# maotian123/loc_lib

Measured on AMD Instinct MI355X. Metric: scans/sec (64x1800-pt scan vs 10M-pt map) + ICP iter ms, higher is better.
Workload: dtype f64; 1 GPU; BASELINE configs[2]: 256 scans/GPU x 115200 pts (64x1800, cityblock-v1) vs one 10000000-pt map, P2PLANE ICP, reference defaults (alpha=0.1 KD-tree ANN, eps=1e-2, max 20 iters), scans sharded by rank, no collective; includes scan H2D: every step aligns a batch copied host->HBM for it (pinned double buffer, copy stream, overlapped with the previous step); 3 alignment(s) in flight; scans_per_gpu=256, map_points=10000000, pipeline_depth=3, search_mode=tree_faithful_ann, tree_depth=30, tree_bytes=239999992

## Files before the change

include/locgpu.h:

```cpp
#ifndef LOCGPU_H_
#define LOCGPU_H_

#include <stddef.h>
#include <stdint.h>

#ifdef __cplusplus
extern "C" {
#endif

#define LOCGPU_API __attribute__((visibility("default")))

typedef struct locgpu_ctx locgpu_ctx;
typedef struct locgpu_batch locgpu_batch;

typedef enum locgpu_status {
    LOCGPU_OK = 0,
    LOCGPU_ERR_INVALID = -1,
    LOCGPU_ERR_NO_DEVICE = -2,
    LOCGPU_ERR_NO_TARGET = -3,
    LOCGPU_ERR_K_TOO_LARGE = -4,
    LOCGPU_ERR_DEPTH = -5,
    LOCGPU_ERR_OOM = -6
} locgpu_status;

// ... 55 lines not shown
LOCGPU_API int locgpu_icp_build_map_planes(locgpu_ctx* ctx);
LOCGPU_API int locgpu_icp_map_planes_info(const locgpu_ctx* ctx, int64_t out[3]);
LOCGPU_API int locgpu_icp_map_planes_dump(locgpu_ctx* ctx, double* n4, uint8_t* valid, size_t cap, size_t* n_out);

LOCGPU_API int locgpu_knn(locgpu_ctx* ctx, const float* queries, size_t nq, int k, int approximate, float alpha, int search_mode,
                          int32_t* out_idx, uint32_t* visits);

LOCGPU_API int locgpu_bfnn_set_target(locgpu_ctx* ctx, const void* pts, size_t n, size_t stride_bytes);
LOCGPU_API int locgpu_bfnn_knn(locgpu_ctx* ctx, const float* queries, size_t nq, int k, int32_t* out_idx);

LOCGPU_API int locgpu_icp_hb(locgpu_ctx* ctx, const void* src, size_t n, size_t stride_bytes, const double pose[7],
                             const locgpu_icp_opts* opts, double H[36], double B[6], int64_t* effective_num, int* ok);

LOCGPU_API int locgpu_icp_align(locgpu_ctx* ctx, const void* src, size_t n, size_t stride_bytes, const double init_pose[7],
                                const locgpu_icp_opts* opts, double out_pose[7], locgpu_align_stats* stats);

typedef void* (*locgpu_out_cloud_fn)(void* user, size_t n_points);
#define LOCGPU_OUT_FIELDS_DONE ((size_t)1 << (sizeof(size_t) * 8 - 1))
LOCGPU_API int locgpu_icp_scan_match(locgpu_ctx* ctx, const void* src, size_t n, size_t stride_bytes, const double init_pose[7],
                                     const locgpu_icp_opts* opts, double out_pose[7], locgpu_align_stats* stats, void* out_cloud,
                                     size_t out_stride_bytes, locgpu_out_cloud_fn out_fn, void* out_user);
LOCGPU_API int locgpu_ndt_scan_match(locgpu_ctx* ctx, const void* src, size_t n, size_t stride_bytes, const double init_pose[7],
                                     double result_pose[7], locgpu_align_stats* stats, void* out_cloud, size_t out_stride_bytes,
                                     locgpu_out_cloud_fn out_fn, void* out_user);

LOCGPU_API int locgpu_transform_cloud(locgpu_ctx* ctx, const double pose[7], const void* src, size_t n, size_t src_stride_bytes,
                                      void* out, size_t out_stride_bytes);

LOCGPU_API int locgpu_batch_create(locgpu_ctx* ctx, const void* const* srcs, const size_t* counts, size_t stride_bytes, int n_scans,
                                   locgpu_batch** out);
LOCGPU_API void locgpu_batch_destroy(locgpu_batch* b);
LOCGPU_API int locgpu_batch_create_empty(locgpu_ctx* ctx, int n_scans, size_t max_points_per_scan, locgpu_batch** out);
LOCGPU_API int locgpu_batch_upload_async(locgpu_batch* b, const void* const* srcs, const size_t* counts, size_t stride_bytes);
LOCGPU_API int locgpu_batch_upload_wait(locgpu_batch* b);
LOCGPU_API int locgpu_icp_align_batch(locgpu_ctx* ctx, locgpu_batch* b, const double* init_poses, const locgpu_icp_opts* opts,
                                      double* out_poses, locgpu_align_stats* stats);
LOCGPU_API int locgpu_ndt_align_batch(locgpu_ctx* ctx, locgpu_batch* b, const double* init_poses, double* out_poses,
                                      locgpu_align_stats* stats);
LOCGPU_API int locgpu_icp_align_batch_begin(locgpu_ctx* ctx, locgpu_batch* b, const double* init_poses, const locgpu_icp_opts* opts);
LOCGPU_API int locgpu_ndt_align_batch_begin(locgpu_ctx* ctx, locgpu_batch* b, const double* init_poses);
LOCGPU_API int locgpu_align_batch_end(locgpu_ctx* ctx, locgpu_batch* b, double* out_poses, locgpu_align_stats* stats);
LOCGPU_API int locgpu_icp_hb_batch(locgpu_ctx* ctx, locgpu_batch* b, const double* poses, const locgpu_icp_opts* opts, double* hb);
LOCGPU_API int locgpu_gn_update(const double hb[44], int method, int min_effective_pts, double eps, double pose[7], double dx[6],
                                int* applied, int* stop);

typedef struct locgpu_loam locgpu_loam;
typedef struct locgpu_loam_opts {
    locgpu_icp_opts surf;
    locgpu_icp_opts edge;
    int32_t use_surf_points;
    int32_t use_edge_points;
    int32_t max_iteration;
    double eps;
} locgpu_loam_opts;
LOCGPU_API void locgpu_loam_opts_default(locgpu_loam_opts* o);
LOCGPU_API int locgpu_loam_create(int device_id, const locgpu_loam_opts* opts, locgpu_loam** out);
LOCGPU_API int locgpu_loam_create_on(locgpu_ctx* surf_ctx, locgpu_ctx* edge_ctx, const locgpu_loam_opts* opts, locgpu_loam** out);
LOCGPU_API void locgpu_loam_destroy(locgpu_loam* l);
LOCGPU_API const char* locgpu_loam_last_error(const locgpu_loam* l);
LOCGPU_API int locgpu_loam_set_target(locgpu_loam* l, const void* edge_pts, size_t n_edge, const void* surf_pts, size_t n_surf, size_t stride_bytes);
LOCGPU_API int locgpu_loam_hb(locgpu_loam* l, const void* edge, size_t n_edge, const void* surf, size_t n_surf, size_t stride_bytes,
                              const double pose[7], double H[36], double B[6], int64_t eff[2], int32_t ok[2]);
LOCGPU_API int locgpu_loam_scan_match(locgpu_loam* l, const void* edge, size_t n_edge, const void* surf, size_t n_surf, size_t stride_bytes,
                                      const double init_pose[7], double result_pose[7], locgpu_align_stats* stats, void* out_cloud,
                                      size_t out_stride_bytes);
LOCGPU_API int locgpu_loam_align_batch(locgpu_loam* l, int n_scans, const void* const* edge_srcs, const size_t* edge_counts,
                                       const void* const* surf_srcs, const size_t* surf_counts, size_t stride_bytes, const double* init_poses,
                                       double* out_poses, locgpu_align_stats* stats);

typedef struct locgpu_fitness {
    double score;
    int64_t inliers;
    int64_t finite_points;
} locgpu_fitness;
LOCGPU_API int locgpu_icp_fitness(locgpu_ctx* ctx, const void* src, size_t n, size_t stride_bytes, const double* poses, int n_poses,
                                  double max_range, locgpu_fitness* out);
LOCGPU_API int locgpu_icp_fitness_batch(locgpu_ctx* ctx, locgpu_batch* batch, const double* poses, double max_range, locgpu_fitness* out);
LOCGPU_API int locgpu_icp_fitness_resident(locgpu_ctx* ctx, const double pose[7], double max_range, locgpu_fitness* out);

LOCGPU_API int locgpu_batch_create_shared(locgpu_ctx* ctx, const void* src, size_t n, size_t stride_bytes, int n_entries, locgpu_batch** out);

typedef struct locgpu_init_search_opts {
    double max_range;
    double min_inlier_ratio;
} locgpu_init_search_opts;
LOCGPU_API void locgpu_init_search_opts_default(locgpu_init_search_opts* o);
LOCGPU_API int locgpu_icp_init_search(locgpu_ctx* ctx, const void* src, size_t n, size_t stride_bytes, const double* candidates, int m,
                                      const locgpu_icp_opts* opts, const locgpu_init_search_opts* sopts, double* out_poses,
                                      locgpu_fitness* out_fit, locgpu_align_stats* stats, int* best);
LOCGPU_API int locgpu_loam_fitness(locgpu_loam* l, const void* edge, size_t n_edge, const void* surf, size_t n_surf, size_t stride_bytes,
                                   const double* poses, int n_poses, double max_range, locgpu_fitness* out );
LOCGPU_API int locgpu_loam_init_search(locgpu_loam* l, const void* edge, size_t n_edge, const void* surf, size_t n_surf, size_t stride_bytes,
                                       const double* candidates, int m, const locgpu_init_search_opts* sopts, double* out_poses,
                                       locgpu_fitness* out_fit , locgpu_align_stats* stats, int* best);

LOCGPU_API int locgpu_pose_grid(const double centre[7], double xy_half, double xy_step, double yaw_half, double yaw_step, double* out,
                                size_t cap, size_t* n_out);

#define LOCGPU_COMM_ID_BYTES 128
LOCGPU_API int locgpu_comm_unique_id(void* id_out );
LOCGPU_API int locgpu_comm_init(locgpu_ctx* ctx, int rank, int world, const void* id);
LOCGPU_API int locgpu_comm_info(const locgpu_ctx* ctx, int* rank, int* world);
LOCGPU_API int locgpu_batch_create_sharded(locgpu_ctx* ctx, const void* const* srcs, const size_t* counts, size_t stride_bytes, int n_local,
                                           int first_scan, int n_total, locgpu_batch** out);
LOCGPU_API int locgpu_icp_set_target_bcast(locgpu_ctx* ctx, const void* pts, size_t n, size_t stride_bytes, int root);

typedef struct locgpu_pool locgpu_pool;
typedef struct locgpu_pool_opts {
    int32_t slots;
    int32_t prefetch;
    int32_t scans_per_job;
    int32_t chunk;
    int32_t matcher;
    uint64_t max_points;
    locgpu_icp_opts icp;
} locgpu_pool_opts;
LOCGPU_API void locgpu_pool_opts_default(locgpu_pool_opts* o);
LOCGPU_API int locgpu_pool_create(locgpu_ctx* ctx, const locgpu_pool_opts* opts, locgpu_pool** out);
LOCGPU_API void locgpu_pool_destroy(locgpu_pool* pool);
LOCGPU_API int locgpu_pool_submit(locgpu_pool* pool, const void* const* srcs, const size_t* counts, size_t stride_bytes, int n_local, int first_scan,
                                  int n_total, const double* init_poses, int64_t* ticket);
LOCGPU_API int locgpu_pool_wait(locgpu_pool* pool, int64_t ticket, double* out_poses, locgpu_align_stats* stats);
LOCGPU_API int locgpu_pool_step(locgpu_pool* pool, int block);
LOCGPU_API int locgpu_pool_done(const locgpu_pool* pool, int64_t ticket, int* done);
LOCGPU_API int locgpu_pool_info(const locgpu_pool* pool, int64_t out[8]);
LOCGPU_API int locgpu_pool_profile_read(locgpu_pool* pool, double out[2], int reset);

LOCGPU_API int locgpu_ndt_set_target(locgpu_ctx* ctx, const void* pts, size_t n, size_t stride_bytes, const locgpu_ndt_opts* opts);
LOCGPU_API int locgpu_ndt_target_info(const locgpu_ctx* ctx, int64_t out[3]);
LOCGPU_API int locgpu_ndt_dump(locgpu_ctx* ctx, int32_t* keys, double* mu, double* info, size_t cap, size_t* n_out);
LOCGPU_API int locgpu_ndt_align(locgpu_ctx* ctx, const void* src, size_t n, size_t stride_bytes, const double init_pose[7],
                                double out_pose[7], locgpu_align_stats* stats);
LOCGPU_API int locgpu_ndt_hb(locgpu_ctx* ctx, const void* src, size_t n, size_t stride_bytes, const double pose[7], double H[36], double B[6],
                             int64_t* effective_num, int* ok);
LOCGPU_API int locgpu_ndt_hb_batch(locgpu_ctx* ctx, locgpu_batch* b, const double* poses, double* hb);

LOCGPU_API int locgpu_ndt_fitness(locgpu_ctx* ctx, const void* src, size_t n, size_t stride_bytes, const double* poses, int n_poses,
                                  locgpu_fitness* out);
LOCGPU_API int locgpu_ndt_fitness_batch(locgpu_ctx* ctx, locgpu_batch* batch, const double* poses, locgpu_fitness* out);
LOCGPU_API int locgpu_ndt_fitness_resident(locgpu_ctx* ctx, const double pose[7], locgpu_fitness* out);
LOCGPU_API int locgpu_ndt_init_search(locgpu_ctx* ctx, const void* src, size_t n, size_t stride_bytes, const double* candidates, int m,
                                      const locgpu_init_search_opts* sopts, double* out_poses, locgpu_fitness* out_fit,
                                      locgpu_align_stats* stats, int* best);

LOCGPU_API int locgpu_graph_enable(locgpu_ctx* ctx, int on);

LOCGPU_API int locgpu_profile_enable(locgpu_ctx* ctx, int on);
LOCGPU_API int locgpu_profile_read(locgpu_ctx* ctx, double out[6], int reset);
LOCGPU_API int locgpu_visit_count_enable(locgpu_ctx* ctx, int on);
LOCGPU_API int locgpu_visit_count_read(locgpu_ctx* ctx, uint64_t out[4], int reset);

LOCGPU_API int locgpu_search_stats_read(locgpu_ctx* ctx, uint64_t out[4], int reset);
LOCGPU_API int locgpu_debug_batch_nn(locgpu_ctx* ctx, locgpu_batch* batch, int k, int32_t* out);
LOCGPU_API int locgpu_debug_batch_slot(const locgpu_batch* batch);

typedef struct locgpu_cloud locgpu_cloud;
typedef struct locgpu_submap locgpu_submap;
#define LOCGPU_NO_INTENSITY ((size_t)-1)

LOCGPU_API int locgpu_cloud_create(locgpu_ctx* ctx, locgpu_cloud** out);
LOCGPU_API void locgpu_cloud_destroy(locgpu_cloud* c);
LOCGPU_API int locgpu_cloud_upload(locgpu_cloud* c, const void* pts, size_t n, size_t stride_bytes, size_t intensity_offset, int is_dense);
LOCGPU_API int locgpu_cloud_info(const locgpu_cloud* c, size_t* n, int* is_dense);
LOCGPU_API int locgpu_cloud_download(const locgpu_cloud* c, void* out, size_t capacity, size_t stride_bytes, size_t intensity_offset);
LOCGPU_API int locgpu_cloud_copy(const locgpu_cloud* in, locgpu_cloud* out);

LOCGPU_API int locgpu_cloud_remove_nan(const locgpu_cloud* in, locgpu_cloud* out);
LOCGPU_API int locgpu_cloud_voxel_filter(const locgpu_cloud* in, float leaf, locgpu_cloud* out, int* passthrough);
LOCGPU_API int locgpu_cloud_crop_box(const locgpu_cloud* in, const float min_xyz[3], const float max_xyz[3], locgpu_cloud* out);
LOCGPU_API int locgpu_cloud_transform(const locgpu_cloud* in, const double pose[7], locgpu_cloud* out);
LOCGPU_API int locgpu_cloud_append(locgpu_cloud* dst, const locgpu_cloud* src);

LOCGPU_API int locgpu_icp_set_target_cloud(locgpu_ctx* ctx, const locgpu_cloud* target);
LOCGPU_API int locgpu_icp_set_target_cloud_async(locgpu_ctx* ctx, const locgpu_cloud* target);
LOCGPU_API int locgpu_ndt_set_target_cloud(locgpu_ctx* ctx, const locgpu_cloud* target, const locgpu_ndt_opts* opts);
LOCGPU_API int locgpu_icp_align_cloud(locgpu_ctx* ctx, const locgpu_cloud* src, const double init_pose[7], const locgpu_icp_opts* opts,
                                      double out_pose[7], locgpu_align_stats* stats);
LOCGPU_API int locgpu_ndt_align_cloud(locgpu_ctx* ctx, const locgpu_cloud* src, const double init_pose[7], double out_pose[7],
                                      locgpu_align_stats* stats);

LOCGPU_API int locgpu_voxel_filter(locgpu_ctx* ctx, const void* pts, size_t n, size_t stride_bytes, size_t intensity_offset, int is_dense, float leaf,
                                   void* out, size_t* out_n, int* out_is_dense);
LOCGPU_API int locgpu_crop_box(locgpu_ctx* ctx, const void* pts, size_t n, size_t stride_bytes, size_t intensity_offset, int is_dense,
                               const float min_xyz[3], const float max_xyz[3], void* out, size_t* out_n, int* out_is_dense);
LOCGPU_API int locgpu_remove_nan(locgpu_ctx* ctx, const void* pts, size_t n, size_t stride_bytes, size_t intensity_offset, int is_dense, void* out,
                                 size_t* out_n, int* out_is_dense);

LOCGPU_API int locgpu_batch_preprocess(locgpu_batch* src, float leaf, locgpu_batch* dst, int32_t* out_counts ,
                                       int32_t* out_status );
LOCGPU_API int locgpu_batch_upload_clouds(locgpu_batch* b, const locgpu_cloud* const* clouds, int n);
LOCGPU_API int locgpu_batch_download_scan(locgpu_batch* b, int scan, void* out, size_t capacity, size_t stride_bytes, size_t* n);

LOCGPU_API int locgpu_cloud_loam_extract(const locgpu_cloud* in, const uint8_t* ring, int num_scan, locgpu_cloud* edge, locgpu_cloud* surf);
LOCGPU_API int locgpu_loam_extract(locgpu_ctx* ctx, const void* pts, size_t n, size_t stride_bytes, size_t intensity_offset, int intensity_is_u8,
                                   size_t ring_offset, int num_scan, void* edge_out, size_t* n_edge, void* surf_out, size_t* n_surf,
                                   size_t out_stride_bytes, size_t out_intensity_offset);

LOCGPU_API int locgpu_batch_loam_extract(locgpu_batch* src, const uint8_t* const* rings ,
                                         int num_scan, locgpu_batch* edge, locgpu_batch* surf, int32_t* out_edge_counts,
                                         int32_t* out_surf_counts, int32_t* out_status );
LOCGPU_API int locgpu_loam_align_batches(locgpu_loam* l, locgpu_batch* edge, locgpu_batch* surf, const double* init_poses, double* out_poses,
                                         locgpu_align_stats* stats);

typedef struct locgpu_sensor locgpu_sensor;
typedef struct locgpu_sensor_model {
    int32_t n_rings, n_cols;
    float range_scale, min_range;
    int32_t az_per_ring, reserved;
    const float* cos_el;
    const float* sin_el;
    const float* cos_az;
    const float* sin_az;
} locgpu_sensor_model;
LOCGPU_API int locgpu_sensor_create(locgpu_ctx* ctx, const locgpu_sensor_model* model, locgpu_sensor** out);
LOCGPU_API void locgpu_sensor_destroy(locgpu_sensor* s);
LOCGPU_API int locgpu_batch_upload_ranges(locgpu_batch* b, const locgpu_sensor* s, const uint16_t* const* images ,
                                          int32_t* out_counts );
LOCGPU_API int locgpu_batch_download_rings(locgpu_batch* b, int scan, uint8_t* out, size_t capacity, size_t* n);
LOCGPU_API int locgpu_batch_loam_extract_resident(locgpu_batch* src, int num_scan, locgpu_batch* edge, locgpu_batch* surf,
                                                  int32_t* out_edge_counts, int32_t* out_surf_counts, int32_t* out_status );
LOCGPU_API int locgpu_cloud_upload_ranges(locgpu_cloud* c, const locgpu_sensor* s, const uint16_t* image, uint8_t* ring_out ,
                                          size_t* n);

LOCGPU_API int locgpu_range_ingest_times(locgpu_ctx* ctx, double out_ms[2]);

LOCGPU_API int locgpu_submap_create(locgpu_ctx* ctx, int num_kfs, float leaf, locgpu_submap** out);
LOCGPU_API void locgpu_submap_destroy(locgpu_submap* m);
LOCGPU_API int locgpu_submap_add_keyframe(locgpu_submap* m, const locgpu_cloud* scan, const double pose[7]);
LOCGPU_API int locgpu_submap_cloud(locgpu_submap* m, locgpu_cloud** map);
LOCGPU_API int locgpu_submap_last_keyframe(locgpu_submap* m, locgpu_cloud** kf);
LOCGPU_API int locgpu_submap_info(const locgpu_submap* m, int* n_keyframes, size_t* map_points);

LOCGPU_API int locgpu_loam_set_target_cloud(locgpu_loam* l, const locgpu_cloud* edge_map, const locgpu_cloud* surf_map);
LOCGPU_API int locgpu_loam_set_target_cloud_async(locgpu_loam* l, const locgpu_cloud* edge_map, const locgpu_cloud* surf_map);
LOCGPU_API int locgpu_loam_scan_match_cloud(locgpu_loam* l, const locgpu_cloud* edge, const locgpu_cloud* surf, const double init_pose[7],
                                            double result_pose[7], locgpu_align_stats* stats, locgpu_cloud* out);
LOCGPU_API int locgpu_loam_fitness_resident(locgpu_loam* l, const double pose[7], double max_range, locgpu_fitness out[2]);
LOCGPU_API int locgpu_loam_fitness_cloud(locgpu_loam* l, const locgpu_cloud* edge, const locgpu_cloud* surf, const double* poses, int n_poses,
                                         double max_range, locgpu_fitness* out );
LOCGPU_API int locgpu_loam_init_search_cloud(locgpu_loam* l, const locgpu_cloud* edge, const locgpu_cloud* surf, const double* candidates, int m,
                                             const locgpu_init_search_opts* sopts, double* out_poses, locgpu_fitness* out_fit ,
                                             locgpu_align_stats* stats, int* best);

typedef struct locgpu_loam_submap locgpu_loam_submap;
LOCGPU_API int locgpu_loam_submap_create(locgpu_ctx* ctx, int num_kfs, float leaf, locgpu_loam_submap** out);
LOCGPU_API void locgpu_loam_submap_destroy(locgpu_loam_submap* m);
LOCGPU_API int locgpu_loam_submap_add_keyframe(locgpu_loam_submap* m, const locgpu_cloud* edge, const locgpu_cloud* surf, const double pose[7]);
LOCGPU_API int locgpu_loam_submap_clouds(locgpu_loam_submap* m, locgpu_cloud** edge_map, locgpu_cloud** surf_map);
LOCGPU_API int locgpu_loam_submap_info(const locgpu_loam_submap* m, int* n_keyframes, size_t* edge_points, size_t* surf_points);

LOCGPU_API int locgpu_clouds_merge(locgpu_ctx* ctx, const locgpu_cloud* const* clouds, const double* poses , int n, float leaf,
                                   locgpu_cloud* out, int* passthrough );
LOCGPU_API int locgpu_batch_merge(locgpu_batch* b, const double* poses , const uint8_t* use , float leaf,
                                  locgpu_cloud* out, int* passthrough );
LOCGPU_API int locgpu_batch_export_cloud(locgpu_batch* b, int scan, locgpu_cloud* cloud);

#ifdef __cplusplus
}
#endif
#endif
```

loc_lib_amd/api.py:

```python
import ctypes
import os
import subprocess

import numpy as np

_HERE = os.path.dirname(os.path.abspath(__file__))
LIB_PATH = os.environ.get("LOCGPU_LIB") or os.path.join(_HERE, "liblocgpu.so")
CSRC = os.path.join(_HERE, "csrc")

P2P, P2LINE, P2PLANE = 0, 1, 2
P2PLANE_MAP = 5
SEARCH_TREE_FAITHFUL, SEARCH_GRID_EXACT = 0, 1
CENTER, NEARBY6 = 0, 1
DIRECT_NDT, INCREMENTAL_NDT = 1, 2

ABI_SYMBOLS = [
    "locgpu_icp_opts_default", "locgpu_ndt_opts_default", "locgpu_create", "locgpu_destroy", "locgpu_last_error",
    "locgpu_device_count", "locgpu_icp_set_target", "locgpu_icp_set_target_async", "locgpu_icp_target_info", "locgpu_knn", "locgpu_icp_hb", "locgpu_icp_align",
    "locgpu_transform_cloud", "locgpu_batch_create", "locgpu_batch_destroy", "locgpu_icp_align_batch", "locgpu_ndt_align_batch",
    "locgpu_icp_hb_batch", "locgpu_gn_update", "locgpu_ndt_set_target", "locgpu_ndt_target_info", "locgpu_ndt_dump",
    "locgpu_ndt_align", "locgpu_profile_enable", "locgpu_profile_read", "locgpu_visit_count_enable", "locgpu_visit_count_read",
    "locgpu_search_stats_read", "locgpu_debug_batch_nn", "locgpu_debug_batch_slot", "locgpu_graph_enable",
    "locgpu_cloud_create", "locgpu_cloud_destroy", "locgpu_cloud_upload", "locgpu_cloud_info", "locgpu_cloud_download", "locgpu_cloud_copy",
    "locgpu_cloud_remove_nan", "locgpu_cloud_voxel_filter", "locgpu_cloud_crop_box", "locgpu_cloud_transform", "locgpu_cloud_append",
    "locgpu_icp_set_target_cloud", "locgpu_icp_set_target_cloud_async", "locgpu_ndt_set_target_cloud", "locgpu_icp_align_cloud", "locgpu_ndt_align_cloud",
    "locgpu_voxel_filter", "locgpu_crop_box", "locgpu_remove_nan",
    "locgpu_submap_create", "locgpu_submap_destroy", "locgpu_submap_add_keyframe", "locgpu_submap_cloud", "locgpu_submap_last_keyframe",
    "locgpu_submap_info", "locgpu_cloud_loam_extract", "locgpu_loam_extract",
    "locgpu_batch_create_empty", "locgpu_batch_upload_async", "locgpu_batch_upload_wait",
    "locgpu_bfnn_set_target", "locgpu_bfnn_knn",
    "locgpu_icp_align_batch_begin", "locgpu_ndt_align_batch_begin", "locgpu_align_batch_end",
    "locgpu_comm_unique_id", "locgpu_comm_init", "locgpu_comm_info", "locgpu_batch_create_sharded", "locgpu_icp_set_target_bcast",
    "locgpu_pool_opts_default", "locgpu_pool_create", "locgpu_pool_destroy", "locgpu_pool_submit", "locgpu_pool_wait", "locgpu_pool_info",
    "locgpu_pool_profile_read", "locgpu_pool_step", "locgpu_pool_done",
    "locgpu_icp_scan_match", "locgpu_ndt_scan_match",
    "locgpu_icp_fitness", "locgpu_icp_fitness_batch", "locgpu_icp_fitness_resident", "locgpu_batch_create_shared",
    "locgpu_init_search_opts_default", "locgpu_icp_init_search", "locgpu_pose_grid",
    "locgpu_ndt_fitness", "locgpu_ndt_fitness_batch", "locgpu_ndt_fitness_resident", "locgpu_ndt_init_search", "locgpu_ndt_hb", "locgpu_ndt_hb_batch",
    "locgpu_icp_build_map_planes", "locgpu_icp_map_planes_info", "locgpu_icp_map_planes_dump",
    "locgpu_loam_opts_default", "locgpu_loam_create", "locgpu_loam_destroy", "locgpu_loam_last_error", "locgpu_loam_set_target",
    "locgpu_loam_hb", "locgpu_loam_scan_match", "locgpu_loam_align_batch",
    "locgpu_loam_set_target_cloud", "locgpu_loam_set_target_cloud_async", "locgpu_loam_scan_match_cloud", "locgpu_loam_fitness_resident",
    "locgpu_loam_submap_create", "locgpu_loam_submap_destroy", "locgpu_loam_submap_add_keyframe", "locgpu_loam_submap_clouds", "locgpu_loam_submap_info",
    "locgpu_loam_create_on", "locgpu_loam_fitness", "locgpu_loam_fitness_cloud", "locgpu_loam_init_search", "locgpu_loam_init_search_cloud",
    "locgpu_batch_preprocess", "locgpu_batch_upload_clouds", "locgpu_batch_download_scan",
    "locgpu_batch_loam_extract", "locgpu_loam_align_batches",
    "locgpu_clouds_merge", "locgpu_batch_merge", "locgpu_batch_export_cloud",
    "locgpu_sensor_create", "locgpu_sensor_destroy", "locgpu_batch_upload_ranges", "locgpu_batch_download_rings",
    "locgpu_batch_loam_extract_resident", "locgpu_cloud_upload_ranges", "locgpu_range_ingest_times",
]
COMM_ID_BYTES = 128
NO_INTENSITY = ctypes.c_size_t(-1).value


class LocGpuError(RuntimeError):
    def __init__(self, code, msg):
        super().__init__("locgpu error %d: %s" % (code, msg))
        self.code = code


class IcpOpts(ctypes.Structure):
    _fields_ = [("method", ctypes.c_int32), ("max_iteration", ctypes.c_int32), ("max_nn_distance", ctypes.c_double),
                ("max_plane_distance", ctypes.c_double), ("max_line_distance", ctypes.c_double), ("min_effective_pts", ctypes.c_int32),
                ("eps", ctypes.c_double), ("approximate", ctypes.c_int32), ("ann_alpha", ctypes.c_float), ("search_mode", ctypes.c_int32)]


class NdtOpts(ctypes.Structure):
    _fields_ = [("max_iteration", ctypes.c_int32), ("voxel_size", ctypes.c_double), ("min_effective_pts", ctypes.c_int32),
                ("min_pts_in_voxel", ctypes.c_int32), ("eps", ctypes.c_double), ("res_outlier_th", ctypes.c_double),
                ("nearby_type", ctypes.c_int32), ("method", ctypes.c_int32), ("capacity", ctypes.c_int64)]


class LoamOpts(ctypes.Structure):
    _fields_ = [("surf", IcpOpts), ("edge", IcpOpts), ("use_surf_points", ctypes.c_int32), ("use_edge_points", ctypes.c_int32),
                ("max_iteration", ctypes.c_int32), ("eps", ctypes.c_double)]


class PoolOpts(ctypes.Structure):
    _fields_ = [("slots", ctypes.c_int32), ("prefetch", ctypes.c_int32), ("scans_per_job", ctypes.c_int32), ("chunk", ctypes.c_int32), ("matcher", ctypes.c_int32),
                ("max_points", ctypes.c_uint64), ("icp", IcpOpts)]


class Fitness(ctypes.Structure):
    _fields_ = [("score", ctypes.c_double), ("inliers", ctypes.c_int64), ("finite_points", ctypes.c_int64)]


class InitSearchOpts(ctypes.Structure):
    _fields_ = [("max_range", ctypes.c_double), ("min_inlier_ratio", ctypes.c_double)]


class SensorModelC(ctypes.Structure):
    _fields_ = [("n_rings", ctypes.c_int32), ("n_cols", ctypes.c_int32), ("range_scale", ctypes.c_float), ("min_range", ctypes.c_float),
                ("az_per_ring", ctypes.c_int32), ("reserved", ctypes.c_int32), ("cos_el", ctypes.c_void_p), ("sin_el", ctypes.c_void_p),
                ("cos_az", ctypes.c_void_p), ("sin_az", ctypes.c_void_p)]


class AlignStats(ctypes.Structure):
    _fields_ = [("iterations", ctypes.c_int32), ("converged", ctypes.c_int32), ("status", ctypes.c_int32), ("reserved", ctypes.c_int32),
                ("last_effective_num", ctypes.c_int64), ("last_dx_norm", ctypes.c_double)]


def build(force=False):
    args = ["make", "-C", CSRC, "-j4"]
    if force:
        args.append("-B")
    subprocess.check_call(args, stdout=subprocess.DEVNULL)
    return LIB_PATH


_lib = None


def lib():
    global _lib
    if _lib is None:
        if not os.path.exists(LIB_PATH):
            raise LocGpuError(-2, "liblocgpu.so is not built (run `python -c 'import __graft_entry__ as g; g.build()'`); no CPU fallback exists")
        L = ctypes.CDLL(LIB_PATH)
        vp, sz, i32, dbl, f32 = ctypes.c_void_p, ctypes.c_size_t, ctypes.c_int, ctypes.c_double, ctypes.c_float
        sig = {
            "locgpu_icp_opts_default": (None, [vp]), "locgpu_ndt_opts_default": (None, [vp]),
            "locgpu_create": (i32, [i32, vp]), "locgpu_destroy": (None, [vp]), "locgpu_last_error": (ctypes.c_char_p, [vp]),
            "locgpu_device_count": (i32, []),
            "locgpu_icp_set_target": (i32, [vp, vp, sz, sz]), "locgpu_icp_set_target_async": (i32, [vp, vp, sz, sz]), "locgpu_icp_target_info": (i32, [vp, vp]),
            "locgpu_knn": (i32, [vp, vp, sz, i32, i32, f32, i32, vp, vp]),
            "locgpu_icp_hb": (i32, [vp, vp, sz, sz, vp, vp, vp, vp, vp, vp]),
            "locgpu_icp_align": (i32, [vp, vp, sz, sz, vp, vp, vp, vp]),
            "locgpu_transform_cloud": (i32, [vp, vp, vp, sz, sz, vp, sz]),
            "locgpu_batch_create": (i32, [vp, vp, vp, sz, i32, vp]), "locgpu_batch_destroy": (None, [vp]),
            "locgpu_icp_align_batch": (i32, [vp, vp, vp, vp, vp, vp]), "locgpu_ndt_align_batch": (i32, [vp, vp, vp, vp, vp]),
            "locgpu_icp_align_batch_begin": (i32, [vp, vp, vp, vp]), "locgpu_ndt_align_batch_begin": (i32, [vp, vp, vp]),
            "locgpu_align_batch_end": (i32, [vp, vp, vp, vp]),
            "locgpu_icp_hb_batch": (i32, [vp, vp, vp, vp, vp]),
            "locgpu_gn_update": (i32, [vp, i32, i32, dbl, vp, vp, vp, vp]),
            "locgpu_ndt_set_target": (i32, [vp, vp, sz, sz, vp]), "locgpu_ndt_target_info": (i32, [vp, vp]),
            "locgpu_ndt_dump": (i32, [vp, vp, vp, vp, sz, vp]), "locgpu_ndt_align": (i32, [vp, vp, sz, sz, vp, vp, vp]),
            "locgpu_profile_enable": (i32, [vp, i32]), "locgpu_profile_read": (i32, [vp, vp, i32]),
            "locgpu_visit_count_enable": (i32, [vp, i32]), "locgpu_visit_count_read": (i32, [vp, vp, i32]),
            "locgpu_search_stats_read": (i32, [vp, vp, i32]), "locgpu_debug_batch_nn": (i32, [vp, vp, i32, vp]), "locgpu_debug_batch_slot": (i32, [vp]), "locgpu_graph_enable": (i32, [vp, i32]),
            "locgpu_cloud_create": (i32, [vp, vp]), "locgpu_cloud_destroy": (None, [vp]),
            "locgpu_cloud_upload": (i32, [vp, vp, sz, sz, sz, i32]), "locgpu_cloud_info": (i32, [vp, vp, vp]),
            "locgpu_cloud_download": (i32, [vp, vp, sz, sz, sz]), "locgpu_cloud_copy": (i32, [vp, vp]),
            "locgpu_cloud_remove_nan": (i32, [vp, vp]), "locgpu_cloud_voxel_filter": (i32, [vp, f32, vp, vp]),
            "locgpu_cloud_crop_box": (i32, [vp, vp, vp, vp]), "locgpu_cloud_transform": (i32, [vp, vp, vp]),
            "locgpu_cloud_append": (i32, [vp, vp]),
            "locgpu_icp_set_target_cloud": (i32, [vp, vp]), "locgpu_icp_set_target_cloud_async": (i32, [vp, vp]), "locgpu_ndt_set_target_cloud": (i32, [vp, vp, vp]),
            "locgpu_icp_align_cloud": (i32, [vp, vp, vp, vp, vp, vp]), "locgpu_ndt_align_cloud": (i32, [vp, vp, vp, vp, vp]),
            "locgpu_voxel_filter": (i32, [vp, vp, sz, sz, sz, i32, f32, vp, vp, vp]),
            "locgpu_crop_box": (i32, [vp, vp, sz, sz, sz, i32, vp, vp, vp, vp, vp]),
            "locgpu_remove_nan": (i32, [vp, vp, sz, sz, sz, i32, vp, vp, vp]),
            "locgpu_submap_create": (i32, [vp, i32, f32, vp]), "locgpu_submap_destroy": (None, [vp]),
            "locgpu_submap_add_keyframe": (i32, [vp, vp, vp]), "locgpu_submap_cloud": (i32, [vp, vp]),
            "locgpu_submap_last_keyframe": (i32, [vp, vp]), "locgpu_submap_info": (i32, [vp, vp, vp]),
            "locgpu_cloud_loam_extract": (i32, [vp, vp, i32, vp, vp]),
            "locgpu_loam_extract": (i32, [vp, vp, sz, sz, sz, i32, sz, i32, vp, vp, vp, vp, sz, sz]),
            "locgpu_batch_create_empty": (i32, [vp, i32, sz, vp]), "locgpu_batch_upload_async": (i32, [vp, vp, vp, sz]),
            "locgpu_batch_upload_wait": (i32, [vp]),
            "locgpu_comm_unique_id": (i32, [vp]), "locgpu_comm_init": (i32, [vp, i32, i32, vp]), "locgpu_comm_info": (i32, [vp, vp, vp]),
            "locgpu_batch_create_sharded": (i32, [vp, vp, vp, sz, i32, i32, i32, vp]),
            "locgpu_icp_set_target_bcast": (i32, [vp, vp, sz, sz, i32]),
            "locgpu_bfnn_set_target": (i32, [vp, vp, sz, sz]), "locgpu_bfnn_knn": (i32, [vp, vp, sz, i32, vp]),
            "locgpu_pool_opts_default": (None, [vp]), "locgpu_pool_create": (i32, [vp, vp, vp]), "locgpu_pool_destroy": (None, [vp]),
            "locgpu_pool_submit": (i32, [vp, vp, vp, sz, i32, i32, i32, vp, vp]), "locgpu_pool_wait": (i32, [vp, ctypes.c_int64, vp, vp]),
            "locgpu_pool_info": (i32, [vp, vp]), "locgpu_pool_profile_read": (i32, [vp, vp, i32]),
            "locgpu_pool_step": (i32, [vp, i32]), "locgpu_pool_done": (i32, [vp, ctypes.c_int64, vp]),
            "locgpu_icp_scan_match": (i32, [vp, vp, sz, sz, vp, vp, vp, vp, vp, sz, vp, vp]),
            "locgpu_ndt_scan_match": (i32, [vp, vp, sz, sz, vp, vp, vp, vp, sz, vp, vp]),
            "locgpu_icp_fitness": (i32, [vp, vp, sz, sz, vp, i32, dbl, vp]), "locgpu_icp_fitness_batch": (i32, [vp, vp, vp, dbl, vp]),
            "locgpu_icp_fitness_resident": (i32, [vp, vp, dbl, vp]), "locgpu_batch_create_shared": (i32, [vp, vp, sz, sz, i32, vp]),
            "locgpu_init_search_opts_default": (None, [vp]),
            "locgpu_icp_init_search": (i32, [vp, vp, sz, sz, vp, i32, vp, vp, vp, vp, vp, vp]),
            "locgpu_pose_grid": (i32, [vp, dbl, dbl, dbl, dbl, vp, sz, vp]),
            "locgpu_ndt_fitness": (i32, [vp, vp, sz, sz, vp, i32, vp]), "locgpu_ndt_fitness_batch": (i32, [vp, vp, vp, vp]),
            "locgpu_ndt_fitness_resident": (i32, [vp, vp, vp]),
            "locgpu_ndt_hb": (i32, [vp, vp, sz, sz, vp, vp, vp, vp, vp]), "locgpu_ndt_hb_batch": (i32, [vp, vp, vp, vp]),
            "locgpu_ndt_init_search": (i32, [vp, vp, sz, sz, vp, i32, vp, vp, vp, vp, vp]),
            "locgpu_icp_build_map_planes": (i32, [vp]), "locgpu_icp_map_planes_info": (i32, [vp, vp]),
            "locgpu_icp_map_planes_dump": (i32, [vp, vp, vp, sz, vp]),
            "locgpu_loam_opts_default": (None, [vp]), "locgpu_loam_create": (i32, [i32, vp, vp]), "locgpu_loam_destroy": (None, [vp]),
            "locgpu_loam_last_error": (ctypes.c_char_p, [vp]), "locgpu_loam_set_target": (i32, [vp, vp, sz, vp, sz, sz]),
            "locgpu_loam_hb": (i32, [vp, vp, sz, vp, sz, sz, vp, vp, vp, vp, vp]),
            "locgpu_loam_scan_match": (i32, [vp, vp, sz, vp, sz, sz, vp, vp, vp, vp, sz]),
            "locgpu_loam_align_batch": (i32, [vp, i32, vp, vp, vp, vp, sz, vp, vp, vp]),
            "locgpu_loam_set_target_cloud": (i32, [vp, vp, vp]), "locgpu_loam_set_target_cloud_async": (i32, [vp, vp, vp]),
            "locgpu_loam_scan_match_cloud": (i32, [vp, vp, vp, vp, vp, vp, vp]), "locgpu_loam_fitness_resident": (i32, [vp, vp, dbl, vp]),
            "locgpu_loam_submap_create": (i32, [vp, i32, f32, vp]), "locgpu_loam_submap_destroy": (None, [vp]),
            "locgpu_loam_submap_add_keyframe": (i32, [vp, vp, vp, vp]), "locgpu_loam_submap_clouds": (i32, [vp, vp, vp]),
            "locgpu_loam_submap_info": (i32, [vp, vp, vp, vp]),
            "locgpu_loam_create_on": (i32, [vp, vp, vp, vp]),
            "locgpu_loam_fitness": (i32, [vp, vp, sz, vp, sz, sz, vp, i32, dbl, vp]),
            "locgpu_loam_fitness_cloud": (i32, [vp, vp, vp, vp, i32, dbl, vp]),
            "locgpu_loam_init_search": (i32, [vp, vp, sz, vp, sz, sz, vp, i32, vp, vp, vp, vp, vp]),
            "locgpu_loam_init_search_cloud": (i32, [vp, vp, vp, vp, i32, vp, vp, vp, vp, vp]),
            "locgpu_batch_preprocess": (i32, [vp, f32, vp, vp, vp]), "locgpu_batch_upload_clouds": (i32, [vp, vp, i32]),
            "locgpu_batch_download_scan": (i32, [vp, i32, vp, sz, sz, vp]),
            "locgpu_batch_loam_extract": (i32, [vp, vp, i32, vp, vp, vp, vp, vp]), "locgpu_loam_align_batches": (i32, [vp, vp, vp, vp, vp, vp]),
            "locgpu_clouds_merge": (i32, [vp, vp, vp, i32, f32, vp, vp]), "locgpu_batch_merge": (i32, [vp, vp, vp, f32, vp, vp]),
            "locgpu_batch_export_cloud": (i32, [vp, i32, vp]),
            "locgpu_sensor_create": (i32, [vp, vp, vp]), "locgpu_sensor_destroy": (None, [vp]),
            "locgpu_batch_upload_ranges": (i32, [vp, vp, vp, vp]), "locgpu_batch_download_rings": (i32, [vp, i32, vp, sz, vp]),
            "locgpu_batch_loam_extract_resident": (i32, [vp, i32, vp, vp, vp, vp, vp]),
            "locgpu_cloud_upload_ranges": (i32, [vp, vp, vp, vp, vp]), "locgpu_range_ingest_times": (i32, [vp, vp]),
        }
        for name, (res, args) in sig.items():
            fn = getattr(L, name)
            fn.restype = res
            fn.argtypes = args
        _lib = L
    return _lib


def device_count():
    return int(lib().locgpu_device_count())


def comm_unique_id():
    buf = (ctypes.c_char * COMM_ID_BYTES)()
    rc = lib().locgpu_comm_unique_id(buf)
    if rc != 0:
        raise LocGpuError(rc, "locgpu_comm_unique_id failed")
    return bytes(buf)


def _cloud(a):
    a = np.ascontiguousarray(a, dtype=np.float32)
    if a.ndim != 2 or a.shape[1] < 3:
        raise ValueError("cloud must be [n, >=3] float32")
    return a


def _pose(p):
    p = np.ascontiguousarray(p, dtype=np.float64)
    if p.shape[-1] != 7:
        raise ValueError("pose must have 7 doubles (quaternion xyzw + translation)")
    return p


def icp_opts(method=P2P, **kw):
    o = IcpOpts()
    lib().locgpu_icp_opts_default(ctypes.byref(o))
    o.method = method
    for k, v in kw.items():
        if not hasattr(o, k):
            raise TypeError("unknown ICP option %r" % k)
        setattr(o, k, v)
    return o


def ndt_opts(**kw):
    o = NdtOpts()
    lib().locgpu_ndt_opts_default(ctypes.byref(o))
    for k, v in kw.items():
        if not hasattr(o, k):
            raise TypeError("unknown NDT option %r" % k)
        setattr(o, k, v)
    return o


def init_search_opts(**kw):
    o = InitSearchOpts()
    lib().locgpu_init_search_opts_default(ctypes.byref(o))
    for k, v in kw.items():
        if not hasattr(o, k):
            raise TypeError("unknown initial-pose search option %r" % k)
        setattr(o, k, v)
    return o


def loam_opts(**kw):
    o = LoamOpts()
    lib().locgpu_loam_opts_default(ctypes.byref(o))
    for k, v in kw.items():
        if not hasattr(o, k):
            raise TypeError("unknown LOAM option %r" % k)
        setattr(o, k, v)
    return o


def pose_grid(centre, xy_half, xy_step, yaw_half, yaw_step, cap=None):
    c = _pose(centre)
    n = ctypes.c_size_t(0)
    rc = lib().locgpu_pose_grid(c.ctypes.data, xy_half, xy_step, yaw_half, yaw_step, None, 0, ctypes.byref(n))
    if rc != 0:
        raise LocGpuError(rc, "locgpu_pose_grid: bad arguments")
    k = n.value if cap is None else min(int(cap), n.value)
    out = np.zeros((k, 7))
    rc = lib().locgpu_pose_grid(c.ctypes.data, xy_half, xy_step, yaw_half, yaw_step, out.ctypes.data if k else None, k, ctypes.byref(n))
    if rc != 0:
        raise LocGpuError(rc, "locgpu_pose_grid: bad arguments")
    return out, int(n.value)


# ... 224 lines not shown
        return out, [_stats_dict(s) for s in st]

    def icp_hb_batch(self, batch, poses, opts):
        batch.upload_wait()
        p = _pose(poses).reshape(batch.n_scans, 7)
        hb = np.zeros((batch.n_scans, 44))
        self._check(lib().locgpu_icp_hb_batch(self._h, batch._h, p.ctypes.data, ctypes.byref(opts), hb.ctypes.data))
        return hb

    def icp_fitness(self, src, poses, max_range=1.0, raw=False):
        s = _cloud(src)
        p = _pose(poses)
        one = p.ndim == 1
        p = p.reshape(-1, 7)
        out = (Fitness * p.shape[0])()
        self._check(lib().locgpu_icp_fitness(self._h, s.ctypes.data, s.shape[0], s.strides[0], p.ctypes.data, p.shape[0], max_range, out))
        if raw:
            return out
        return _fitness_dict(out[0]) if one else [_fitness_dict(f) for f in out]

    def icp_fitness_batch(self, batch, poses, max_range=1.0, raw=False):
        batch.upload_wait()
        p = _pose(poses).reshape(batch.n_scans, 7)
        out = (Fitness * batch.n_scans)()
        self._check(lib().locgpu_icp_fitness_batch(self._h, batch._h, p.ctypes.data, max_range, out))
        return out if raw else [_fitness_dict(f) for f in out]

    def icp_fitness_resident(self, pose, max_range=1.0):
        out = Fitness()
        self._check(lib().locgpu_icp_fitness_resident(self._h, _pose(pose).ctypes.data, max_range, ctypes.byref(out)))
        return _fitness_dict(out)

    def batch_shared(self, scan, n_entries):
        return Batch(self, None, n_scans=n_entries, shared=scan)

    def icp_init_search(self, src, candidates, opts, sopts=None, raw=False):
        s = _cloud(src)
        c = _pose(candidates).reshape(-1, 7)
        m = c.shape[0]
        out = np.zeros((m, 7))
        fit = (Fitness * max(m, 1))()
        st = (AlignStats * max(m, 1))()
        best = ctypes.c_int(-2)
        self._check(lib().locgpu_icp_init_search(self._h, s.ctypes.data, s.shape[0], s.strides[0], c.ctypes.data, m, ctypes.byref(opts),
                                                 ctypes.byref(sopts) if sopts is not None else None, out.ctypes.data, fit, st, ctypes.byref(best)))
        return out, (fit if raw else [_fitness_dict(f) for f in fit]), [_stats_dict(x) for x in st], int(best.value)

    def ndt_set_target(self, cloud, opts=None):
        c = _cloud(cloud)
        self._check(lib().locgpu_ndt_set_target(self._h, c.ctypes.data, c.shape[0], c.strides[0], ctypes.byref(opts) if opts else None))

    def ndt_target_info(self):
        out = np.zeros(3, dtype=np.int64)
        self._check(lib().locgpu_ndt_target_info(self._h, out.ctypes.data))
        return dict(num_voxels=int(out[0]), capacity=int(out[1]), bytes=int(out[2]))

    def ndt_dump(self):
        n = self.ndt_target_info()["num_voxels"]
        keys = np.zeros((max(n, 1), 3), dtype=np.int32)
        mu = np.zeros((max(n, 1), 3))
        info = np.zeros((max(n, 1), 9))
        n_out = ctypes.c_size_t(0)
        self._check(lib().locgpu_ndt_dump(self._h, keys.ctypes.data, mu.ctypes.data, info.ctypes.data, n, ctypes.byref(n_out)))
        return keys[:n], mu[:n], info[:n].reshape(n, 3, 3)

    def ndt_align(self, src, init_pose):
        s = _cloud(src)
        out = np.zeros(7)
        st = AlignStats()
        self._check(lib().locgpu_ndt_align(self._h, s.ctypes.data, s.shape[0], s.strides[0], _pose(init_pose).ctypes.data, out.ctypes.data,
                                           ctypes.byref(st)))
        return out, _stats_dict(st)

    def ndt_hb(self, src, pose):
        s = _cloud(src)
        H, B = np.zeros(36), np.zeros(6)
        eff, ok = ctypes.c_int64(0), ctypes.c_int(0)
        self._check(lib().locgpu_ndt_hb(self._h, s.ctypes.data, s.shape[0], s.strides[0], _pose(pose).ctypes.data, H.ctypes.data, B.ctypes.data,
                                        ctypes.byref(eff), ctypes.byref(ok)))
        return bool(ok.value), H.reshape(6, 6), B, int(eff.value)

    def ndt_hb_batch(self, batch, poses):
        batch.upload_wait()
        p = _pose(poses).reshape(batch.n_scans, 7)
        hb = np.zeros((batch.n_scans, 44))
        self._check(lib().locgpu_ndt_hb_batch(self._h, batch._h, p.ctypes.data, hb.ctypes.data))
        return hb

    def ndt_fitness(self, src, poses, raw=False):
        s = _cloud(src)
        p = _pose(poses)
        one = p.ndim == 1
        p = p.reshape(-1, 7)
        out = (Fitness * max(p.shape[0], 1))()
        self._check(lib().locgpu_ndt_fitness(self._h, s.ctypes.data, s.shape[0], s.strides[0], p.ctypes.data, p.shape[0], out))
        if raw:
            return out
        return _fitness_dict(out[0]) if one else [_fitness_dict(f) for f in out]

    def ndt_fitness_batch(self, batch, poses, raw=False):
        batch.upload_wait()
        p = _pose(poses).reshape(batch.n_scans, 7)
        out = (Fitness * batch.n_scans)()
        self._check(lib().locgpu_ndt_fitness_batch(self._h, batch._h, p.ctypes.data, out))
        return out if raw else [_fitness_dict(f) for f in out]

    def ndt_fitness_resident(self, pose):
        out = Fitness()
        self._check(lib().locgpu_ndt_fitness_resident(self._h, _pose(pose).ctypes.data, ctypes.byref(out)))
        return _fitness_dict(out)

    def ndt_init_search(self, src, candidates, sopts=None, raw=False):
        s = _cloud(src)
        c = _pose(candidates).reshape(-1, 7)
        m = c.shape[0]
        out = np.zeros((m, 7))
        fit = (Fitness * max(m, 1))()
        st = (AlignStats * max(m, 1))()
        best = ctypes.c_int(-2)
        self._check(lib().locgpu_ndt_init_search(self._h, s.ctypes.data, s.shape[0], s.strides[0], c.ctypes.data, m,
                                                 ctypes.byref(sopts) if sopts is not None else None, out.ctypes.data, fit, st, ctypes.byref(best)))
        return out, (fit if raw else [_fitness_dict(f) for f in fit]), [_stats_dict(x) for x in st], int(best.value)

    def graph_enable(self, on=True):
        self._check(lib().locgpu_graph_enable(self._h, int(on)))

    def profile_enable(self, on=True):
        self._check(lib().locgpu_profile_enable(self._h, int(on)))

    def profile_read(self, reset=True):
        out = np.zeros(6)
        self._check(lib().locgpu_profile_read(self._h, out.ctypes.data, int(reset)))
        return dict(search_ms=out[0], accum_ms=out[1], solve_ms=out[2], search_n=int(out[3]), accum_n=int(out[4]), solve_n=int(out[5]))

    def range_ingest_times(self):
        out = np.zeros(2)
        self._check(lib().locgpu_range_ingest_times(self._h, out.ctypes.data))
        return float(out[0]), float(out[1])

    def visit_count_enable(self, on=True):
        self._check(lib().locgpu_visit_count_enable(self._h, int(on)))

    def visit_count_read(self, reset=True):
        out = np.zeros(4, dtype=np.uint64)
        self._check(lib().locgpu_visit_count_read(self._h, out.ctypes.data, int(reset)))
        return dict(nodes=int(out[0]), leaves=int(out[1]), queries=int(out[2]), distinct_slots=int(out[3]))


    def debug_batch_nn(self, batch, k=5):
        out = np.empty((batch.n_local, batch.max_points, k), dtype=np.int32)
        self._check(lib().locgpu_debug_batch_nn(self._h, batch._h, int(k), out.ctypes.data))
        return out

    def search_stats_read(self, reset=True):
        out = np.zeros(4, dtype=np.uint64)
        self._check(lib().locgpu_search_stats_read(self._h, out.ctypes.data, int(reset)))
        return dict(searched=int(out[0]), redone=int(out[1]), walked=int(out[2]), replayed=int(out[3]))


def _xyzi(a):
    a = np.ascontiguousarray(a, dtype=np.float32)
    if a.ndim != 2 or a.shape[1] != 4:
        raise ValueError("cloud must be [n, 4] float32 (x, y, z, intensity)")
    return a


class Cloud:

    def __init__(self, ctx, points=None, is_dense=True, _borrowed=None):
        self.ctx = ctx
        self._owned = _borrowed is None
        if _borrowed is not None:
            self._h = _borrowed
        else:
            self._h = ctypes.c_void_p()
            ctx._check(lib().locgpu_cloud_create(ctx._h, ctypes.byref(self._h)))
            if points is not None:
                self.upload(points, is_dense)

    def upload(self, points, is_dense=True):
        a = _xyzi(points)
        self.ctx._check(lib().locgpu_cloud_upload(self._h, a.ctypes.data, a.shape[0], 16, 12, int(is_dense)))
        return self

    @property
    def info(self):
        n, d = ctypes.c_size_t(0), ctypes.c_int(0)
        self.ctx._check(lib().locgpu_cloud_info(self._h, ctypes.byref(n), ctypes.byref(d)))
        return int(n.value), bool(d.value)

    def __len__(self):
        return self.info[0]

    @property
    def is_dense(self):
        return self.info[1]

    def download(self):
        n = len(self)
        out = np.zeros((n, 4), np.float32)
        self.ctx._check(lib().locgpu_cloud_download(self._h, out.ctypes.data, n, 16, 12))
        return out

    def _out(self, out):
        return out if out is not None else Cloud(self.ctx)

    def copy(self, out=None):
        out = self._out(out)
        self.ctx._check(lib().locgpu_cloud_copy(self._h, out._h))
        return out

    def remove_nan(self, out=None):
        out = self._out(out)
        self.ctx._check(lib().locgpu_cloud_remove_nan(self._h, out._h))
        return out

    def voxel_filter(self, leaf, out=None, with_passthrough=False):
        out = self._out(out)
        pt = ctypes.c_int(0)
        self.ctx._check(lib().locgpu_cloud_voxel_filter(self._h, float(leaf), out._h, ctypes.byref(pt)))
        return (out, bool(pt.value)) if with_passthrough else out

    def crop_box(self, mn, mx, out=None):
        out = self._out(out)
        mn, mx = np.ascontiguousarray(mn, np.float32), np.ascontiguousarray(mx, np.float32)
        self.ctx._check(lib().locgpu_cloud_crop_box(self._h, mn.ctypes.data, mx.ctypes.data, out._h))
        return out

    def transform(self, pose, out=None):
        out = self._out(out)
        self.ctx._check(lib().locgpu_cloud_transform(self._h, _pose(pose).ctypes.data, out._h))
        return out

    def append(self, other):
        self.ctx._check(lib().locgpu_cloud_append(self._h, other._h))
        return self

    def upload_ranges(self, sensor, image, with_rings=True):
        img = sensor.model.image(image)
        rings = np.zeros(sensor.model.cells, np.uint8) if with_rings else None
        n = ctypes.c_size_t(0)
        self.ctx._check(lib().locgpu_cloud_upload_ranges(self._h, sensor._h, img.ctypes.data, rings.ctypes.data if with_rings else None, ctypes.byref(n)))
        return np.ascontiguousarray(rings[:int(n.value)]) if with_rings else None

    def loam_extract(self, ring, num_scan=16):
        ring = np.ascontiguousarray(ring, dtype=np.uint8)
        if len(ring) != len(self):
            raise ValueError("one ring byte per point")
        edge, surf = Cloud(self.ctx), Cloud(self.ctx)
        self.ctx._check(lib().locgpu_cloud_loam_extract(self._h, ring.ctypes.data, int(num_scan), edge._h, surf._h))
        return edge, surf

    def close(self):
        if self._owned and getattr(self, "_h", None) and getattr(self.ctx, "_h", None):
            lib().locgpu_cloud_destroy(self._h)
        self._h = None

    def __del__(self):
        self.close()


class SensorModel:

    def __init__(self, n_rings, n_cols, range_scale, min_range, cos_el, sin_el, cos_az, sin_az):
        self.n_rings, self.n_cols = int(n_rings), int(n_cols)
        self.range_scale, self.min_range = np.float32(range_scale), np.float32(min_range)
        self.cos_el, self.sin_el, self.cos_az, self.sin_az = (np.ascontiguousarray(t, dtype=np.float32) for t in (cos_el, sin_el, cos_az, sin_az))
        self.az_per_ring = int(self.cos_az.ndim == 2)
        want_az = (self.n_rings, self.n_cols) if self.az_per_ring else (self.n_cols,)
        if self.cos_el.shape != (self.n_rings,) or self.sin_el.shape != (self.n_rings,) or self.cos_az.shape != want_az or self.sin_az.shape != want_az:
            raise ValueError("sensor tables do not match n_rings / n_cols")

    @property
    def cells(self):
        return self.n_rings * self.n_cols

    def c_struct(self):
        return SensorModelC(self.n_rings, self.n_cols, float(self.range_scale), float(self.min_range), self.az_per_ring, 0, self.cos_el.ctypes.data,
                            self.sin_el.ctypes.data, self.cos_az.ctypes.data, self.sin_az.ctypes.data)

    def image(self, a):
        a = np.ascontiguousarray(a, dtype=np.uint16)
        if a.size != self.cells:
            raise ValueError("a range image of this sensor has %d x %d cells" % (self.n_rings, self.n_cols))
        return a


class Sensor:

    def __init__(self, ctx, model):
        self.ctx, self.model = ctx, model
        self._h = ctypes.c_void_p()
        m = model.c_struct()
        ctx._check(lib().locgpu_sensor_create(ctx._h, ctypes.byref(m), ctypes.byref(self._h)))

    def close(self):
        if getattr(self, "_h", None) and getattr(self.ctx, "_h", None):
            lib().locgpu_sensor_destroy(self._h)
        self._h = None

    def __del__(self):
        self.close()


class Submap:

# ... 469 lines not shown
```

loc_lib_amd/csrc/context.hpp:

```cpp
#pragma once
#include <hip/hip_runtime.h>

#include <string>
#include <vector>

#include "../../include/locgpu.h"
#include "batch_upload.hpp"
#include "device_buffer.hpp"
#include "device_math.hpp"
#include "grid_kernels.hpp"
#include "icp_kernels.hpp"

#include "host_worker.hpp"

struct NdtTable;
namespace locgpu {
struct IncNdtState;
struct FilterScratch;
struct LoamScratch;
struct BatchFilterScratch;
struct BatchLoamScratch;
struct MergeScratch;
struct RangeIngestScratch;
}
struct locgpu_sensor;

namespace locgpu {
struct PendingTarget;
struct AlignSpec {
    GnParams prm{};
    float alpha = 1.0f;
    bool grid = false;
    bool ndt() const { return method_is_ndt(prm.method); }
    int k() const { return method_k(prm.method); }
    bool operator==(const AlignSpec& o) const { return prm == o.prm && alpha == o.alpha && grid == o.grid; }
};
constexpr int kNdtOptDirect = 1, kNdtOptIncremental = 2;
constexpr int kNearbyCenter = 0, kNearby6 = 1;
constexpr int ndt_n_nearby(int nearby_type) { return nearby_type == kNearbyCenter ? 1 : 7; }
struct StageEvents {
    std::vector<Event> ev;
    size_t used = 0;
    int mode = 0;
    void mark(hipStream_t s, bool search_edge = false);
    void collect(locgpu_ctx* ctx, bool ndt);
};
}

struct locgpu_ctx {
    int device = 0;
    hipStream_t stream = nullptr;
    static constexpr int kSlots = 3;
    hipStream_t slot_stream[kSlots] = {};
    int next_slot = 0;
    int slot_load[kSlots] = {};
    hipStream_t copy_stream = nullptr;
    locgpu::Event foreign_ev;
    hipStream_t comm_stream = nullptr;
    locgpu::Uploader* up = nullptr;
    locgpu::PendingTarget* target_scratch = nullptr;
    locgpu::PendingTarget* pending_target = nullptr;
    std::string err;

    locgpu::DevBuf<uint2> d_tree;
    size_t tree_slots = 0, num_leaves = 0, num_nodes = 0, num_points = 0;
    int depth = 0;
    bool tree_bounded = true;
    unsigned long long target_epoch = 0;

    locgpu::DevBuf<uint32_t> d_leaf_slots;

    locgpu::DevBuf<double> d_planes;
    size_t planes_rows = 0;
    bool planes_ready = false;
    long long planes_valid = 0;
    locgpu::DevBuf<unsigned long long> d_planes_count;
    locgpu_batch* planes_ws = nullptr;

    locgpu::GridView grid;
    locgpu::GridBuffers grid_buf;

    locgpu::DevBuf<float4> d_bfnn;
    size_t bfnn_n = 0;

    NdtTable* ndt = nullptr;
    locgpu::IncNdtState* inc = nullptr;
    locgpu_ndt_opts ndt_opts;

    locgpu::FilterScratch* filt = nullptr;
    locgpu::LoamScratch* loam = nullptr;
    locgpu::BatchFilterScratch* bfilt = nullptr;
    locgpu::BatchLoamScratch* bloam = nullptr;
    locgpu::MergeScratch* merge = nullptr;
    locgpu::RangeIngestScratch* ringest = nullptr;
    std::vector<locgpu_sensor*> sensors;

    locgpu_batch* single = nullptr;
    size_t single_cap = 0;
    locgpu_batch* search = nullptr;
    locgpu::HostWorker* worker = nullptr;

    void* comm = nullptr;
    int comm_rank = 0, comm_world = 1;

    int profile = 0;
    double prof_ms[3] = {0, 0, 0};
    long long prof_n[3] = {0, 0, 0};
    bool use_graph = false;
    bool count_visits = false;
    locgpu::DevBuf<unsigned long long> d_visits;
    locgpu::DevBuf<uint32_t> d_touched;
    size_t touched_words = 0;
    locgpu::DevBuf<unsigned long long> d_search_stats;
};

struct locgpu_batch {
    locgpu_ctx* ctx = nullptr;
    int slot = 0;
    hipStream_t stream = nullptr;
    bool pinned = false;
    bool leased = false;
    locgpu::Event chunk_ev;
    int n_scans = 0, max_n = 0, blocks_per_scan = 0;
    int n_total = 0, first = 0;
    bool sharded = false;
    locgpu::DevBuf<double> d_acc;
    size_t pitch = 0;
    locgpu::DevBuf<float4> d_src;
    locgpu::DevBuf<int> d_counts;
    locgpu::DevBuf<unsigned char> d_rings;
    bool rings_valid = false;
    locgpu::DevBuf<locgpu::PoseState> d_state;
    locgpu::DevBuf<uint32_t> d_nn;
    bool shared_src = false;
    locgpu::DevBuf<int> d_src_of;
    int cap_scans = 0, split_scans = 0;
    size_t cap_points = 0;
    const float4* d_src_ext = nullptr;
    bool counters_clean = false;
    int last_iterations = -1;
    locgpu::DevBuf<double> d_partials;
    locgpu::DevBuf<double> d_hb;
    locgpu::DevBuf<uint32_t> d_redo_list;
    locgpu::DevBuf<unsigned int> d_redo_count;
    locgpu::DevBuf<uint32_t> d_redo_list2;
    locgpu::DevBuf<uint32_t> d_grid_qkey;
    locgpu::DevBuf<uint2> d_grid_sorted;
    locgpu::DevBuf<uint32_t> d_grid_tile_count;
    locgpu::DevBuf<unsigned char> d_grid_scan_temp;
    hipGraphExec_t graph_exec = nullptr;
    hipGraphExec_t graph_exec_next = nullptr;
    locgpu::AlignSpec graph_spec;
    const void* graph_target = nullptr;
    unsigned long long graph_epoch = 0;
    locgpu::PinnedBuf<float4> h_src;
    locgpu::Event xyz_ev[8];
    locgpu::PinnedBuf<locgpu::PoseState> h_state;
    locgpu::PinnedBuf<unsigned long long> h_post;
    static constexpr int kPostWord = 16;
    unsigned int post_call = 0;
    bool paced_tail = false;
    locgpu::Event tail_ev;
    locgpu::PinnedBuf<double> h_hb;
    locgpu::PinnedBuf<int> h_active;
    locgpu::DevBuf<int> d_active;
    std::vector<int> counts;
    locgpu::BatchUploadState upl;
    locgpu::StageEvents stage_ev;
    locgpu::Event ev_ready, ev_reduced;
    struct Pending {
        bool active = false;
        locgpu::AlignSpec spec;
        bool graph = false;
        bool paced = false;
        int launched = 0;
        std::vector<double> init_poses;
    } pending;
};

namespace locgpu {

int fail(locgpu_ctx* ctx, int code, const std::string& msg);
bool hip_ok(locgpu_ctx* ctx, hipError_t e, const char* what);

void ndt_free(locgpu_ctx* ctx);
int alloc_batch(locgpu_ctx* ctx, int n_scans, size_t max_n, locgpu_batch** out, int first = 0, int n_total = -1, bool shared_src = false);
void free_batch(locgpu_batch* b);
int check_icp(locgpu_ctx* ctx, const locgpu_icp_opts* o, AlignSpec& spec);
int check_ndt(locgpu_ctx* ctx, AlignSpec& spec);
int target_join(locgpu_ctx* ctx, bool install = true);
void free_target_scratch(locgpu_ctx* ctx);
int icp_set_target_from_cloud(locgpu_ctx* ctx, const locgpu_cloud* target, bool async);
int ensure_grid(locgpu_ctx* ctx);
void free_grid(locgpu_ctx* ctx);
bool comm_all_reduce_f64(locgpu_ctx* ctx, double* buf, size_t count, hipStream_t s);
bool comm_broadcast(locgpu_ctx* ctx, void* buf, size_t bytes, int root, hipStream_t s);
bool comm_all_reduce_min_int(locgpu_ctx* ctx, int* buf, hipStream_t s);
void comm_destroy(locgpu_ctx* ctx);

}

#define LOCGPU_HIP(ctx, expr)                                                    \
    do {                                                                         \
        if (!locgpu::hip_ok((ctx), (expr), #expr)) return LOCGPU_ERR_NO_DEVICE;  \
    } while (0)
```

loc_lib_amd/csrc/gn_driver.hip:

```cpp
#include <algorithm>
#include <chrono>
#include <cmath>
#include <cstdlib>
#include <cstring>
#include <string>
#include <thread>

#include "batch_upload.hpp"
#include "env.hpp"
#include "gn_driver.hpp"
#include "ndt_inc.hpp"
#include "ndt_kernels.hpp"
#include "stream_lease.hpp"

namespace locgpu {

namespace {
inline int next_chunk(const locgpu_batch* b) { return b->n_total == 1 ? 2 : kNextChunk; }
inline int first_chunk_len(const locgpu_batch* b) {
    if (b->n_total != 1 || b->sharded || b->last_iterations < 0) return kFirstChunk;
    return std::min(kLongFirstChunk, std::max(3, b->last_iterations + 1));
}

}

SearchArgs make_search_args(const locgpu_ctx* ctx, const locgpu_batch* b, const float4* src, const PoseState* st, int k, float alpha_eff, bool skip_nonfinite) {
    SearchArgs sa{ctx->d_tree, ctx->tree_slots * sizeof(uint64_t), ctx->depth, src, b->d_counts, st, b->d_nn, b->pitch, b->max_n, b->n_scans, k, alpha_eff,
                  skip_nonfinite ? 1 : 0, nullptr, b->d_redo_list, b->d_redo_count, b->d_redo_list2, b->d_redo_count + 1, ctx->d_search_stats};
    if (!ctx->tree_bounded) sa.redo_list = nullptr;
    return sa;
}

void init_state(PoseState& ps, const double pose[7]) {
    std::memset(&ps, 0, sizeof(ps));
    for (int i = 0; i < 4; ++i) ps.q[i] = pose[i];
    for (int i = 0; i < 3; ++i) ps.t[i] = pose[4 + i];
    quat_to_R(ps.q, ps.R);
}

static void init_states(locgpu_batch* b, const double* poses) {
    for (int s = 0; s < b->n_total; ++s) init_state(b->h_state[s], poses + 7 * (size_t)s);
}

void write_scan_result(const PoseState& ps, const double* init, double* out_pose, locgpu_align_stats* stats) {
    if (ps.status == 1) {
        for (int j = 0; j < 7; ++j) out_pose[j] = init[j];
    } else {
        for (int j = 0; j < 4; ++j) out_pose[j] = ps.q[j];
        for (int j = 0; j < 3; ++j) out_pose[4 + j] = ps.t[j];
    }
    if (!stats) return;
    stats->iterations = ps.iterations; stats->converged = ps.converged; stats->status = ps.status; stats->reserved = 0;
    stats->last_effective_num = ps.last_eff; stats->last_dx_norm = ps.last_dx_norm;
}

bool shard_decoupled(const locgpu_ctx* ctx, bool scan_sharded) {
    static const int env = env_int("LOCGPU_SHARD_DECOUPLED", -1);
    return ctx->comm && scan_sharded && (env >= 0 ? env != 0 : ctx->comm_world > 1);
}

void StageEvents::mark(hipStream_t s, bool search_edge) {
    if (!mode || (mode == 2 && !search_edge)) return;
    if (ev.size() <= used) {
        Event e;
        if (e.ensure(hipEventDefault) != hipSuccess) return;
        ev.push_back(std::move(e));
    }
    (void)hipEventRecord(ev[used++], s);
}

void StageEvents::collect(locgpu_ctx* ctx, bool ndt) {
    const size_t per = mode == 2 ? 2 : 4;
    for (size_t i = 0; i + per - 1 < used; i += per)
        for (size_t j = 0; j + 1 < per; ++j) {
            if (ndt && j == 0) continue;
            float ms = 0.f;
            if (hipEventElapsedTime(&ms, ev[i + j], ev[i + j + 1]) == hipSuccess) { ctx->prof_ms[j] += ms; ctx->prof_n[j] += 1; }
        }
    used = 0;
}

int launch_local_stage(locgpu_ctx* ctx, locgpu_batch* b, const LocalStage& w, hipStream_t s) {
    StageEvents& ev = b->stage_ev;
    int n_partial_blocks = b->blocks_per_scan;
    ev.mark(s, true);
    if (b->n_scans == 0 || (w.active && w.n_active == 0)) {
        ev.mark(s, true);
    } else if (!w.spec.ndt()) {
        const GnParams& prm = w.spec.prm;
        SearchArgs sa = make_search_args(ctx, b, w.src, w.state, w.spec.k(), w.spec.alpha, skips_nonfinite(prm.method));
        const bool grid_mode = w.spec.grid && ctx->tree_bounded;
        if (grid_mode && !w.grid) { fail(ctx, LOCGPU_ERR_INVALID, "grid search: work list missing (ensure_grid_lists was not called)"); return -1; }
        sa.visit_totals = w.visits;
        sa.active = w.active; sa.n_active = w.n_active;
        sa.src_of = w.src_of;
        if (sa.visit_totals && !w.capturing) {
            const size_t words = (ctx->tree_slots + 2 + 31) / 32;
            if (words > ctx->touched_words) {
                ctx->touched_words = 0;
                if (ctx->d_touched.alloc(words) == hipSuccess && hipMemsetAsync(ctx->d_touched, 0, words * sizeof(uint32_t), s) == hipSuccess)
                    ctx->touched_words = words;
            }
            sa.touched = ctx->touched_words ? ctx->d_touched.get() : nullptr;
        }
        const bool ok_search = (grid_mode && !sa.visit_totals) ? launch_icp_search_grid(ctx->grid, sa, *w.grid, s) : launch_icp_search(sa, s);
        if (!ok_search) { fail(ctx, LOCGPU_ERR_DEPTH, std::string(w.who) + ": unsupported k/depth"); return -1; }
        if (sa.touched) launch_count_touched(sa.touched, (ctx->tree_slots + 2 + 31) / 32, sa.visit_totals, s);
        ev.mark(s, true);
        AccumArgs aa{ctx->d_tree, w.src, b->d_counts, w.state, b->d_nn, b->pitch, b->max_n, b->n_scans, icp_gate(prm), b->d_partials};
        aa.planes = ctx->d_planes;
        aa.active = w.active; aa.n_active = w.n_active;
        aa.src_of = w.src_of;
        aa.split_scans = w.split_scans;
        n_partial_blocks = launch_icp_accum(prm.method, aa, s);
    } else {
        ev.mark(s, true);
        if (w.spec.prm.method == kMethodNdtInc)
            launch_inc_accum(ctx->inc, ctx->ndt_opts.res_outlier_th, ndt_n_nearby(ctx->ndt_opts.nearby_type), w.src, b->d_counts, w.state, b->max_n, b->n_scans, b->d_partials, s,
                             w.active, w.n_active, w.src_of);
        else
            n_partial_blocks = launch_ndt_accum(ctx->ndt, w.src, b->d_counts, w.state, b->max_n, b->n_scans, b->d_partials, s, w.active, w.n_active, w.split_scans, w.src_of);
    }
    ev.mark(s);
    return n_partial_blocks;
}

struct IterLauncher {
    locgpu_ctx* ctx;
    locgpu_batch* b;
    const AlignSpec& spec;
    bool capturing = false;
    int slot = 0;
    bool replicated_on_comm_stream = false;
    const int* active = nullptr;
    int n_active = 0;
    const GnPost* post = nullptr;
    bool launch(int do_update);
};

bool IterLauncher::launch(int do_update) {
    hipStream_t s = b->stream;
    const GnParams& prm = spec.prm;
    const bool ndt = spec.ndt();
    StageEvents& ev = b->stage_ev;
    ev.mode = capturing ? 0 : ctx->profile;
    const GridSearchScratch gsc{b->d_grid_qkey, b->d_grid_sorted, b->d_grid_tile_count, b->d_grid_scan_temp};
    const LocalStage w{batch_src(b), b->d_state + b->first, active, n_active, b->d_src_of, b->sharded ? b->n_total : b->split_scans, spec,
                       ctx->count_visits ? ctx->d_visits : nullptr, b->d_grid_qkey ? &gsc : nullptr, capturing, "search"};
    const int n_partial_blocks = launch_local_stage(ctx, b, w, s);
    if (n_partial_blocks < 0) return false;
    if (b->sharded) {
        double* acc = b->d_acc + (size_t)(slot % kFirstChunk) * b->n_total * kAccW;
        slot++;
        launch_sum_partials(b->d_partials, n_partial_blocks, b->d_state, b->first, b->n_scans, b->n_total, acc, s);
        if (do_update && shard_decoupled(ctx, b->n_scans != b->n_total)) {
            hipStream_t cs = ctx->comm_stream;
            if (b->n_scans > 0)
                launch_gn_solve(acc + (size_t)b->first * kAccW, 1, b->d_state + b->first, b->n_scans, prm, do_update, b->d_hb + (size_t)b->first * 44,
                                ndt ? nullptr : b->d_redo_count, s);
            if (!hip_ok(ctx, hipEventRecord(b->ev_ready, s), "sharded: hipEventRecord") || !hip_ok(ctx, hipStreamWaitEvent(cs, b->ev_ready, 0), "sharded: hipStreamWaitEvent")) return false;
            if (!comm_all_reduce_f64(ctx, acc, (size_t)b->n_total * kAccW, cs)) return false;
            const int after = b->first + b->n_scans;
            if (b->first > 0) launch_gn_solve(acc, 1, b->d_state, b->first, prm, do_update, b->d_hb, nullptr, cs);
            if (after < b->n_total)
                launch_gn_solve(acc + (size_t)after * kAccW, 1, b->d_state + after, b->n_total - after, prm, do_update, b->d_hb + (size_t)after * 44, nullptr, cs);
            replicated_on_comm_stream = true;
            ev.mark(s);
            return hip_ok(ctx, hipGetLastError(), "kernel launch");
        }
        if (ctx->comm) {
            static const int force = env_int("LOCGPU_COMM_DIRECT", -1);
            const bool direct = force >= 0 ? force != 0 : ctx->comm_world == 1;
            hipStream_t cs = direct ? s : ctx->comm_stream;
            if (!direct && (!hip_ok(ctx, hipEventRecord(b->ev_ready, s), "sharded: hipEventRecord") || !hip_ok(ctx, hipStreamWaitEvent(cs, b->ev_ready, 0), "sharded: hipStreamWaitEvent"))) return false;
            if (!comm_all_reduce_f64(ctx, acc, (size_t)b->n_total * kAccW, cs)) return false;
            if (!direct && (!hip_ok(ctx, hipEventRecord(b->ev_reduced, cs), "sharded: hipEventRecord") || !hip_ok(ctx, hipStreamWaitEvent(s, b->ev_reduced, 0), "sharded: hipStreamWaitEvent"))) return false;
        }
        launch_gn_solve(acc, 1, b->d_state, b->n_total, prm, do_update, b->d_hb, ndt ? nullptr : b->d_redo_count, s);
    } else {
        launch_gn_solve(b->d_partials, n_partial_blocks, b->d_state, b->n_scans, prm, do_update, b->d_hb, ndt ? nullptr : b->d_redo_count, s, nullptr, post);
    }
    ev.mark(s);
    return hip_ok(ctx, hipGetLastError(), "kernel launch");
}

static int batch_ready(locgpu_ctx* ctx, locgpu_batch* b) {
    const int rc = upload_join_batch(b);
    if (rc != LOCGPU_OK) return rc;
    LOCGPU_HIP(ctx, upload_order_after(b, b->stream));
    return LOCGPU_OK;
}

int ensure_grid_lists(locgpu_ctx* ctx, locgpu_batch* b, const AlignSpec& spec) {
    if (!spec.grid) return LOCGPU_OK;
    if (!b->d_grid_qkey) {
        LOCGPU_HIP(ctx, b->d_grid_qkey.alloc(b->pitch));
        LOCGPU_HIP(ctx, b->d_grid_sorted.alloc(b->pitch));
    }
    const size_t tocc = ctx->grid.n_tocc, scan = std::max<size_t>(ctx->grid.scan_temp_bytes, 1);
    if (b->d_grid_tile_count.cap() < tocc + 1) {
        LOCGPU_HIP(ctx, hipStreamSynchronize(b->stream));
        LOCGPU_HIP(ctx, b->d_grid_tile_count.alloc(tocc + 1));
    }
    if (b->d_grid_scan_temp.cap() < scan) {
        LOCGPU_HIP(ctx, hipStreamSynchronize(b->stream));
        LOCGPU_HIP(ctx, b->d_grid_scan_temp.alloc(scan));
    }
    return LOCGPU_OK;
}

static int capture_chunk(locgpu_ctx* ctx, locgpu_batch* b, const AlignSpec& spec, int iters, bool with_h2d, hipGraphExec_t* out) {
    hipStream_t s = b->stream;
    hipGraph_t graph = nullptr;
    LOCGPU_HIP(ctx, hipStreamBeginCapture(s, hipStreamCaptureModeThreadLocal));
    bool ok = !with_h2d || hip_ok(ctx, hipMemcpyAsync(b->d_state, b->h_state, b->n_total * sizeof(PoseState), hipMemcpyHostToDevice, s), "capture H2D");
    IterLauncher it{ctx, b, spec};
    it.capturing = true;
    for (int i = 0; ok && i < iters; ++i) ok = it.launch(1);
    ok = ok && hip_ok(ctx, hipMemcpyAsync(b->h_state, b->d_state, b->n_total * sizeof(PoseState), hipMemcpyDeviceToHost, s), "capture D2H");
    const hipError_t e = hipStreamEndCapture(s, &graph);
    if (!ok || !hip_ok(ctx, e, "hipStreamEndCapture")) { if (graph) (void)hipGraphDestroy(graph); return LOCGPU_ERR_NO_DEVICE; }
    const bool inst = hip_ok(ctx, hipGraphInstantiate(out, graph, nullptr, nullptr, 0), "hipGraphInstantiate");
    (void)hipGraphDestroy(graph);
    if (!inst) { *out = nullptr; return LOCGPU_ERR_NO_DEVICE; }
    return LOCGPU_OK;
}

static int ensure_graphs(locgpu_ctx* ctx, locgpu_batch* b, const AlignSpec& spec) {
    const void* target = !spec.ndt() ? (const void*)ctx->d_tree : (spec.prm.method == kMethodNdtInc ? inc_ndt_table_ptr(ctx->inc) : (const void*)ctx->ndt->d_rec);
    if (b->graph_exec && b->graph_spec == spec && b->graph_target == target && b->graph_epoch == ctx->target_epoch) return LOCGPU_OK;
    const int first = std::min(kFirstChunk, spec.prm.max_iteration);
    if (b->graph_exec) { (void)hipGraphExecDestroy(b->graph_exec); b->graph_exec = nullptr; }
    if (b->graph_exec_next) { (void)hipGraphExecDestroy(b->graph_exec_next); b->graph_exec_next = nullptr; }
    int rc = capture_chunk(ctx, b, spec, first, true, &b->graph_exec);
    if (rc == LOCGPU_OK && spec.prm.max_iteration > first) rc = capture_chunk(ctx, b, spec, next_chunk(b), false, &b->graph_exec_next);
    if (rc != LOCGPU_OK) return rc;
    b->graph_spec = spec; b->graph_target = target;
    b->graph_epoch = ctx->target_epoch;
    return LOCGPU_OK;
}

static int enqueue_chunk(locgpu_ctx* ctx, locgpu_batch* b, bool first_chunk) {
    locgpu_batch::Pending& P = b->pending;
    const GnParams& prm = P.spec.prm;
    hipStream_t s = b->stream;
    if (P.graph) {
        LOCGPU_HIP(ctx, hipGraphLaunch(first_chunk ? b->graph_exec : b->graph_exec_next, s));
        P.launched += first_chunk ? std::min(kFirstChunk, prm.max_iteration) : next_chunk(b);
        LOCGPU_HIP(ctx, hipEventRecord(b->chunk_ev, s));
        return LOCGPU_OK;
    }
    if (first_chunk) LOCGPU_HIP(ctx, hipMemcpyAsync(b->d_state, b->h_state, b->n_total * sizeof(PoseState), hipMemcpyHostToDevice, s));
    IterLauncher it{ctx, b, P.spec};
    if (!first_chunk && !P.spec.ndt() && b->n_scans > 1) {
        int na = 0;
        for (int i = 0; i < b->n_scans; ++i)
            if (!b->h_state[b->first + i].done) b->h_active[na++] = i;
        if (na > 0 && na < b->n_scans) {
            LOCGPU_HIP(ctx, hipMemcpyAsync(b->d_active, b->h_active, (size_t)na * sizeof(int), hipMemcpyHostToDevice, s));
            it.active = b->d_active;
            it.n_active = na;
        }
    }
    const int todo = std::min(first_chunk ? first_chunk_len(b) : next_chunk(b), prm.max_iteration - P.launched);
    for (int c = 0; c < todo; ++c)
        if (!it.launch(1)) return LOCGPU_ERR_NO_DEVICE;
// ... 315 lines not shown
```

loc_lib_amd/csrc/icp_fit.hip:

```cpp
#include "env.hpp"
#include "icp_kernels.hpp"
#include "launch.hpp"

#include <cstdlib>

namespace locgpu {

template <int ROWS>
__device__ __forceinline__ void add_rows(double (&acc)[28], const double (&J)[ROWS][6], const double (&e)[ROWS]) {
#pragma clang fp contract(fast)
    int o = 0;
#pragma unroll
    for (int i = 0; i < 6; ++i)
#pragma unroll
        for (int j = i; j < 6; ++j) {
            double s = J[0][i] * J[0][j];
#pragma unroll
            for (int r = 1; r < ROWS; ++r) s += J[r][i] * J[r][j];
            acc[o++] += s;
        }
#pragma unroll
    for (int i = 0; i < 6; ++i) {
        double s = -J[0][i] * e[0];
#pragma unroll
        for (int r = 1; r < ROWS; ++r) s += -J[r][i] * e[r];
        acc[21 + i] += s;
    }
}

constexpr int kAccPad = kBlock + 2;
struct RowAccum {
    int ent, slice, ra, rb;
    double sum;
    bool used;
    __device__ __forceinline__ void init() {
        index(threadIdx.x);
        sum = 0.0;
        used = false;
    }
    __device__ __forceinline__ void index(int tid) {
        ent = tid & 31;
        slice = tid >> 5;
        ra = 7; rb = 7;
        int o = 0;
#pragma unroll
        for (int i = 0; i < 6; ++i)
#pragma unroll
            for (int j = i; j < 6; ++j) {
                if (o == ent) { ra = i; rb = j; }
                ++o;
            }
        if (ent >= 21 && ent < 27) { ra = ent - 21; rb = 6; }
    }
    template <int ROWS>
    __device__ __forceinline__ void add(double (&s_row)[8][kAccPad], const double (&J)[ROWS][6], const double (&neg_e)[ROWS], double fitted) {
#pragma clang fp contract(fast)
        const int tid = threadIdx.x;
#pragma unroll
        for (int r = 0; r < ROWS; ++r) {
            if (used) __syncthreads();
            used = true;
#pragma unroll
            for (int c = 0; c < 6; ++c) s_row[c][tid] = J[r][c];
            s_row[6][tid] = neg_e[r];
            s_row[7][tid] = r == 0 ? fitted : 0.0;
            __syncthreads();
            if (ent < 28) {
#pragma unroll 8
                for (int k = 0; k < 32; ++k) {
                    const int col = k * (kBlock / 32) + slice;
                    sum += s_row[ra][col] * s_row[rb][col];
                }
            }
        }
    }
    __device__ __forceinline__ void store(double (&s_slice)[kBlock / 32][32], double* __restrict__ dst) {
        s_slice[slice][ent] = sum;
        __syncthreads();
        if (threadIdx.x < 28) {
            double t = s_slice[0][threadIdx.x];
#pragma unroll
            for (int w = 1; w < kBlock / 32; ++w) t += s_slice[w][threadIdx.x];
            dst[threadIdx.x] = t;
        }
    }
};

__device__ __forceinline__ void R_hat(const double* R, const D3& q, double (&Rh)[3][3]) {
#pragma unroll
    for (int r = 0; r < 3; ++r) {
        Rh[r][0] = R[3 * r + 1] * q.z - R[3 * r + 2] * q.y;
        Rh[r][1] = R[3 * r + 2] * q.x - R[3 * r + 0] * q.z;
        Rh[r][2] = R[3 * r + 0] * q.y - R[3 * r + 1] * q.x;
    }
}

__device__ __forceinline__ void plane_row(const D3& n3, const double* R, const D3& q, double (&J)[6]) {
    double nR[3];
#pragma unroll
    for (int c = 0; c < 3; ++c) nR[c] = -n3.x * R[c] + (-n3.y * R[3 + c] + -n3.z * R[6 + c]);
    J[0] = nR[1] * q.z - nR[2] * q.y;
    J[1] = nR[2] * q.x - nR[0] * q.z;
    J[2] = nR[0] * q.y - nR[1] * q.x;
    J[3] = n3.x; J[4] = n3.y; J[5] = n3.z;
}

__device__ __forceinline__ void sort5(uint32_t (&s)[5]) {
    auto cx = [&](int a, int b) {
        const uint32_t lo = min(s[a], s[b]), hi = max(s[a], s[b]);
        s[a] = lo; s[b] = hi;
    };
    cx(0, 1); cx(3, 4); cx(2, 4); cx(2, 3); cx(1, 4); cx(0, 3); cx(0, 2); cx(1, 3); cx(1, 2);
}

template <int FIT>
__device__ __forceinline__ bool fit_plane(const uint2* __restrict__ tree, const uint32_t (&slot)[5], double (&n4)[4]) {
    D3 nb[5];
#pragma unroll
    for (int j = 0; j < 5; ++j) nb[j] = leaf_point(tree, slot[j]);
    if constexpr (FIT == 1) {
        if (!plane_null_vector_secular(nb, n4)) plane_null_vector(nb, n4);
    } else {
        plane_null_vector(nb, n4);
    }
    const D3 n3{n4[0], n4[1], n4[2]};
    bool fit = true;
#pragma unroll
    for (int j = 0; j < 5; ++j) {
        const double err = dot3(n3, nb[j]) + n4[3];
        if (err * err > 1e-2) fit = false;
    }
    return fit;
}

__device__ __forceinline__ void plane_point_row(const double (&n4)[4], const float4& p, const PoseState& ps, double max_plane_distance,
                                                double (&J)[6], double& neg_e) {
    const D3 n3{n4[0], n4[1], n4[2]};
    const D3 q{(double)p.x, (double)p.y, (double)p.z};
    const D3 qs = se3_apply(ps.q, ps.t, q);
    const double dis = dot3(n3, qs) + n4[3];
    if (!(fabs(dis) > max_plane_distance)) {
        plane_row(n3, ps.R, q, J);
        neg_e = -dis;
    }
}

template <int FIT>
__device__ __forceinline__ void plane_accum_per_point(const uint2* __restrict__ tree, const float4* __restrict__ src,
                                                                 const int* __restrict__ counts, const PoseState* __restrict__ st,
                                                                 const uint32_t* __restrict__ nn, size_t nn_pitch, int max_n,
                                                                 double max_plane_distance, double* __restrict__ partials, int kPlanePts,
                                                                 const int* __restrict__ active, const int* __restrict__ src_of) {
    __shared__ double s_row[8][kAccPad];
    __shared__ double s_slice[kBlock / 32][32];
    const int scan = active ? active[blockIdx.y] : (int)blockIdx.y;
    if (st[scan].done) return;
    RowAccum ra;
    ra.init();
    const int tid = threadIdx.x;
#pragma unroll 1
    for (int pp = 0; pp < kPlanePts; ++pp) {
        const int i = (blockIdx.x * kPlanePts + pp) * kBlock + tid;
        double J[1][6] = {{0.0, 0.0, 0.0, 0.0, 0.0, 0.0}};
        double neg_e[1] = {0.0};
        double fitted = 0.0;
        if (i < counts[scan]) {
            const size_t gi = (size_t)scan * max_n + i;
            uint32_t slot[5];
#pragma unroll
            for (int j = 0; j < 5; ++j) slot[j] = __builtin_nontemporal_load(&nn[(size_t)j * nn_pitch + gi]);
            const float4 p = src[src_index(src_of, scan, max_n, i)];
            if (slot[4] != kInvalidSlot) {
                sort5(slot);
                double n4[4];
                if (fit_plane<FIT>(tree, slot, n4)) {
                    fitted = 1.0;
                    plane_point_row(n4, p, st[scan], max_plane_distance, J[0], neg_e[0]);
                }
            }
        }
        ra.add<1>(s_row, J, neg_e, fitted);
    }
    ra.store(s_slice, partials + ((size_t)scan * gridDim.x + blockIdx.x) * kAccW);
}

constexpr int kDedupPP = 4;
constexpr int kDedupPts = kDedupPP * kBlock;
constexpr uint16_t kLeadFits = 0x8000;
static_assert(8 * kAccPad <= 4 * kDedupPts && kDedupPts <= kLeadFits, "s_row inside the plane table; a leader's point in 15 bits");
template <int FIT>
__device__ __forceinline__ void plane_accum_per_run(const uint2* __restrict__ tree, const float4* __restrict__ src,
                                                                 const int* __restrict__ counts, const PoseState* __restrict__ st,
                                                                 const uint32_t* __restrict__ nn, size_t nn_pitch, int max_n,
                                                                 double max_plane_distance, double* __restrict__ partials, int kPlanePts,
                                                                 const int* __restrict__ active, const int* __restrict__ src_of) {
    __shared__ double s_plane[kDedupPts][4];
    __shared__ double s_slice[kBlock / 32][32];
    __shared__ uint16_t s_lead[kDedupPts];
    __shared__ uint16_t s_rank[kDedupPP][kBlock];
    __shared__ int s_wcnt[kDedupPP][kBlock / 64];
    double (&s_row)[8][kAccPad] = *reinterpret_cast<double (*)[8][kAccPad]>(&s_plane[0][0]);
    const int scan = active ? active[blockIdx.y] : (int)blockIdx.y;
    if (st[scan].done) return;
    const int lane = threadIdx.x & 63;
    const int wave = __builtin_amdgcn_readfirstlane(threadIdx.x >> 6);
    const int n = counts[scan];
    const size_t region = (size_t)scan * max_n;
    const int first = blockIdx.x * kPlanePts * kBlock;
    RowAccum ra;
    ra.init();
    int tid = threadIdx.x;
    asm volatile("" : "+v"(tid));
    int rank[kDedupPP];
    bool leader[kDedupPP];
#pragma unroll
    for (int h = 0; h < kDedupPP; ++h) {
        const int i = first + h * kBlock + tid;
        uint32_t slot[5];
        bool has = false;
        if (h < kPlanePts && i < n) {
#pragma unroll
            for (int j = 0; j < 5; ++j) slot[j] = nn[(size_t)j * nn_pitch + region + i];
            has = slot[4] != kInvalidSlot;
        }
        if (has) {
            sort5(slot);
        } else {
#pragma unroll
            for (int j = 0; j < 5; ++j) slot[j] = kInvalidSlot;
        }
        bool differs = lane == 0;
#pragma unroll
        for (int j = 0; j < 5; ++j) differs |= (uint32_t)__shfl_up((int)slot[j], 1, 64) != slot[j];
        leader[h] = has && differs;
        const unsigned long long mask = __ballot(leader[h]);
        const int below = (int)__builtin_amdgcn_mbcnt_hi((uint32_t)(mask >> 32), __builtin_amdgcn_mbcnt_lo((uint32_t)mask, 0u));
        rank[h] = has ? below + (leader[h] ? 1 : 0) : 0;
        if (lane == 0) s_wcnt[h][wave] = __popcll(mask);
    }
    __syncthreads();
    int n_lead = 0, before[kDedupPP];
#pragma unroll
    for (int h = 0; h < kDedupPP; ++h) {
        before[h] = n_lead;
#pragma unroll
        for (int w = 0; w < kBlock / 64; ++w) {
            const int c = s_wcnt[h][w];
            before[h] += w < wave ? c : 0;
            n_lead += c;
        }
    }
    n_lead = __builtin_amdgcn_readfirstlane(n_lead);
#pragma unroll
    for (int h = 0; h < kDedupPP; ++h) {
        if (rank[h] > 0) rank[h] += before[h];
        if (leader[h]) s_lead[rank[h] - 1] = (uint16_t)(h * kBlock + tid);
        s_rank[h][tid] = (uint16_t)rank[h];
    }
    __syncthreads();
#pragma unroll 1
    for (int base = 0; base < n_lead; base += kBlock) {
        if (base + wave * 64 < n_lead) {
            const int j = base + tid;
            if (j < n_lead) {
                const uint16_t pt = s_lead[j];
                const size_t gi = region + first + pt;
                uint32_t slot[5];
#pragma unroll
                for (int k = 0; k < 5; ++k) slot[k] = __builtin_nontemporal_load(&nn[(size_t)k * nn_pitch + gi]);
                sort5(slot);
                double n4[4];
                if (fit_plane<FIT>(tree, slot, n4)) s_lead[j] = pt | kLeadFits;
#pragma unroll
                for (int c = 0; c < 4; ++c) s_plane[j][c] = n4[c];
            }
        }
    }
    __syncthreads();
    tid = threadIdx.x;
    asm volatile("" : "+v"(tid));
    ra.index(tid);
    double n4[kDedupPP][4];
    float4 p[kDedupPP];
    bool fits[kDedupPP];
#pragma unroll
    for (int h = 0; h < kDedupPP; ++h) {
        rank[h] = s_rank[h][tid];
        fits[h] = false;
        if (rank[h] > 0) {
            fits[h] = (s_lead[rank[h] - 1] & kLeadFits) != 0;
#pragma unroll
            for (int c = 0; c < 4; ++c) n4[h][c] = s_plane[rank[h] - 1][c];
            p[h] = src[src_index(src_of, scan, max_n, first + h * kBlock + tid)];
        }
    }
    __syncthreads();
#pragma unroll
    for (int h = 0; h < kDedupPP; ++h) {
        if (h < kPlanePts) {
            double J[1][6] = {{0.0, 0.0, 0.0, 0.0, 0.0, 0.0}};
            double neg_e[1] = {0.0};
            double fitted = 0.0;
            if (fits[h]) {
                fitted = 1.0;
                plane_point_row(n4[h], p[h], st[scan], max_plane_distance, J[0], neg_e[0]);
            }
            ra.add<1>(s_row, J, neg_e, fitted);
        }
    }
    ra.store(s_slice, partials + ((size_t)scan * gridDim.x + blockIdx.x) * kAccW);
}

template <int FIT, bool DEDUP>
__global__ __launch_bounds__(kBlock) __attribute__((amdgpu_waves_per_eu(4, 4))) void icp_plane_accum_kernel(const uint2* __restrict__ tree, const float4* __restrict__ src,
                                                                 const int* __restrict__ counts, const PoseState* __restrict__ st,
                                                                 const uint32_t* __restrict__ nn, size_t nn_pitch, int max_n,
                                                                 double max_plane_distance, double* __restrict__ partials, int kPlanePts,
                                                                 const int* __restrict__ active, const int* __restrict__ src_of) {
    if constexpr (DEDUP)
        plane_accum_per_run<FIT>(tree, src, counts, st, nn, nn_pitch, max_n, max_plane_distance, partials, kPlanePts, active, src_of);
    else
        plane_accum_per_point<FIT>(tree, src, counts, st, nn, nn_pitch, max_n, max_plane_distance, partials, kPlanePts, active, src_of);
}

__global__ __launch_bounds__(kBlock) void icp_point_accum_kernel(const uint2* __restrict__ tree, const float4* __restrict__ src,
                                                                 const int* __restrict__ counts, const PoseState* __restrict__ st,
                                                                 const uint32_t* __restrict__ nn, size_t nn_pitch, int max_n,
                                                                 double max_nn_distance, double* __restrict__ partials, int pts,
                                                                 const int* __restrict__ active, const int* __restrict__ src_of) {
    const int scan = active ? active[blockIdx.y] : (int)blockIdx.y;
    if (st[scan].done) return;
    double acc[28];
#pragma unroll
    for (int v = 0; v < 28; ++v) acc[v] = 0.0;
#pragma unroll 1
    for (int pp = 0; pp < pts; ++pp) {
    const int i = (blockIdx.x * pts + pp) * kBlock + threadIdx.x;
    if (i < counts[scan]) {
        const size_t gi = (size_t)scan * max_n + i;
        const uint32_t s0 = nn[gi];
        if (s0 != kInvalidSlot) {
            const float4 p = src[src_index(src_of, scan, max_n, i)];
            const D3 q{(double)p.x, (double)p.y, (double)p.z};
            const D3 qs = se3_apply(st[scan].q, st[scan].t, q);
            const D3 e3 = leaf_point(tree, s0) - qs;
            const double dis2 = dot3(e3, e3);
            if (!(dis2 > max_nn_distance)) {
                acc[27] += 1.0;
                double Rh[3][3];
                R_hat(st[scan].R, q, Rh);
                double J[3][6];
#pragma unroll
                for (int r = 0; r < 3; ++r)
#pragma unroll
                    for (int c = 0; c < 3; ++c) { J[r][c] = Rh[r][c] / 16; J[r][3 + c] = (r == c) ? -1.0 : 0.0; }
                const double e[3] = {e3.x, e3.y, e3.z};
                add_rows<3>(acc, J, e);
            }
        }
    }
    }
    block_reduce_store<28, kAccW>(acc, partials + ((size_t)scan * gridDim.x + blockIdx.x) * kAccW);
}

__global__ __launch_bounds__(kBlock) void icp_mapplane_accum_kernel(const double4* __restrict__ planes, const float4* __restrict__ src,
                                                                    const int* __restrict__ counts, const PoseState* __restrict__ st,
                                                                    const uint32_t* __restrict__ nn, int max_n, double max_plane_distance,
                                                                    double* __restrict__ partials, int pts, const int* __restrict__ active,
                                                                    const int* __restrict__ src_of) {
    const int scan = active ? active[blockIdx.y] : (int)blockIdx.y;
    if (st[scan].done) return;
    double acc[28];
#pragma unroll
    for (int v = 0; v < 28; ++v) acc[v] = 0.0;
    const int n = counts[scan];
    const size_t region = src_index(src_of, scan, max_n, 0);
#pragma unroll 1
    for (int pp = 0; pp < pts; ++pp) {
        const int i = (blockIdx.x * pts + pp) * kBlock + threadIdx.x;
        if (i < n) {
            const uint32_t s0 = __builtin_nontemporal_load(&nn[(size_t)scan * max_n + i]);
            const float4 p = src[region + i];
            if (s0 != kInvalidSlot) {
                const double4 n4 = planes[s0 >> 1];
                if (n4.x == n4.x) {
                    acc[27] += 1.0;
                    const D3 n3{n4.x, n4.y, n4.z};
                    const D3 q{(double)p.x, (double)p.y, (double)p.z};
                    const D3 qs = se3_apply(st[scan].q, st[scan].t, q);
                    const double dis = dot3(n3, qs) + n4.w;
                    if (!(fabs(dis) > max_plane_distance)) {
                        double J[1][6];
                        plane_row(n3, st[scan].R, q, J[0]);
                        const double e[1] = {dis};
                        add_rows<1>(acc, J, e);
                    }
                }
            }
        }
    }
    block_reduce_store<28, kAccW>(acc, partials + ((size_t)scan * gridDim.x + blockIdx.x) * kAccW);
}

__global__ __launch_bounds__(kBlock) __attribute__((amdgpu_waves_per_eu(5, 5))) void icp_line_accum_kernel(const uint2* __restrict__ tree, const float4* __restrict__ src,
                                                                const int* __restrict__ counts, const PoseState* __restrict__ st,
                                                                const uint32_t* __restrict__ nn, size_t nn_pitch, int max_n,
                                                                double max_line_distance, double* __restrict__ partials, int pts,
                                                                const int* __restrict__ active, const int* __restrict__ src_of) {
    __shared__ double s_row[8][kAccPad];
    __shared__ double s_slice[kBlock / 32][32];
    const int scan = active ? active[blockIdx.y] : (int)blockIdx.y;
    if (st[scan].done) return;
    RowAccum ra;
    ra.init();
#pragma unroll 1
    for (int pp = 0; pp < pts; ++pp) {
    const int i = (blockIdx.x * pts + pp) * kBlock + threadIdx.x;
    double J[3][6], neg_e[3] = {0.0, 0.0, 0.0};
    double fitted = 0.0;
#pragma unroll
    for (int r = 0; r < 3; ++r)
#pragma unroll
        for (int c = 0; c < 6; ++c) J[r][c] = 0.0;
    if (i < counts[scan]) {
        const size_t gi = (size_t)scan * max_n + i;
        uint32_t slot[5];
#pragma unroll
        for (int j = 0; j < 5; ++j) slot[j] = nn[(size_t)j * nn_pitch + gi];
        const float4 p = src[src_index(src_of, scan, max_n, i)];
        if (slot[4] != kInvalidSlot) {
            const D3 q{(double)p.x, (double)p.y, (double)p.z};
            const D3 qs = se3_apply(st[scan].q, st[scan].t, q);
            D3 nb[5];
#pragma unroll
            for (int j = 0; j < 5; ++j) nb[j] = leaf_point(tree, slot[j]);
            D3 sum{0.0, 0.0, 0.0};
#pragma unroll
            for (int j = 0; j < 5; ++j) sum = sum + nb[j];
            const D3 p0{sum.x / 5.0, sum.y / 5.0, sum.z / 5.0};
            D3 dl[5];
#pragma unroll
            for (int j = 0; j < 5; ++j) dl[j] = nb[j] - p0;
            const D3 d = line_direction(dl);
            bool fit = true;
#pragma unroll
            for (int j = 0; j < 5; ++j) {
                const D3 c = cross3(d, nb[j] - p0);
                if (dot3(c, c) > max_line_distance) fit = false;
            }
            if (fit) {
                fitted = 1.0;
                const D3 e3 = cross3(d, qs - p0);
                if (!(sqrt(dot3(e3, e3)) > max_line_distance)) {
                    const double hd[3][3] = {{0.0, -d.z, d.y}, {d.z, 0.0, -d.x}, {-d.y, d.x, 0.0}};
                    const double hq[3][3] = {{0.0, -q.z, q.y}, {q.z, 0.0, -q.x}, {-q.y, q.x, 0.0}};
                    const double* R = st[scan].R;
                    double hR[3][3], A[3][3];
#pragma unroll
                    for (int r = 0; r < 3; ++r)
#pragma unroll
                        for (int c = 0; c < 3; ++c) {
                            double s = hd[r][0] * R[c];
                            s += hd[r][1] * R[3 + c];
                            s += hd[r][2] * R[6 + c];
                            hR[r][c] = s;
                        }
#pragma unroll
                    for (int r = 0; r < 3; ++r)
#pragma unroll
                        for (int c = 0; c < 3; ++c) {
                            double s = hR[r][0] * hq[0][c];
                            s += hR[r][1] * hq[1][c];
// ... 82 lines not shown
    ps.iterations += 1;
    if (ok) {
        if (prm.method == LOCGPU_P2P)
            for (int i = 0; i < 6; ++i) dx[i] = dx[i] / 16;
        se3_apply_update(ps.q, ps.t, dx);
        quat_to_R(ps.q, ps.R);
        const double nrm = sqrt((dx[0] * dx[0] + (dx[2] * dx[2] + dx[4] * dx[4])) + (dx[1] * dx[1] + (dx[3] * dx[3] + dx[5] * dx[5])));
        ps.last_dx_norm = nrm;
        if (nrm < prm.eps) { ps.converged = 1; ps.done = 1; }
    }
    if (ps.iterations >= prm.max_iteration) ps.done = 1;
}

__global__ __launch_bounds__(kBlock) void gn_solve_kernel(const double* __restrict__ partials, int blocks_per_scan, PoseState* __restrict__ st,
                                                          GnParams prm, int do_update, double* __restrict__ hb_out, unsigned int* __restrict__ list_counts,
                                                          const int* __restrict__ scans, GnPost post) {
    __shared__ double s_sum[kBlock / kAccW][kAccW];
    const int scan = scans ? scans[blockIdx.x] : (int)blockIdx.x;
    if (list_counts && blockIdx.x == 0 && threadIdx.x < 4) list_counts[threadIdx.x] = 0u;
    if (st[scan].done) return;
    const double col_total = reduce_partials(partials + (size_t)scan * blocks_per_scan * kAccW, blocks_per_scan, true, s_sum);
    if (threadIdx.x < kAccW) s_sum[0][threadIdx.x] = col_total;
    __syncthreads();
    if (threadIdx.x != 0) return;
    double tot[28];
    for (int v = 0; v < 28; ++v) tot[v] = s_sum[0][v];
    PoseState& ps = st[scan];
    gn_update(tot, ps, prm, do_update, hb_out ? hb_out + 44 * (size_t)scan : nullptr);
    if (post.word) {
        const unsigned long long tag = ((unsigned long long)post.call << 32) | ((unsigned long long)(unsigned int)ps.iterations << 1) | (ps.done ? 1ull : 0ull);
        if (ps.done) {
            GnPostRecord r;
            for (int i = 0; i < 4; ++i) r.w[i] = __double_as_longlong(ps.q[i]);
            for (int i = 0; i < 3; ++i) r.w[4 + i] = __double_as_longlong(ps.t[i]);
            r.w[7] = __double_as_longlong(ps.last_dx_norm);
            r.w[8] = (unsigned long long)ps.last_eff;
            r.w[9] = ((unsigned long long)(unsigned int)ps.converged << 32) | (unsigned int)ps.status;
            typedef unsigned long long u64x2 __attribute__((ext_vector_type(2)));
            volatile u64x2* to = reinterpret_cast<volatile u64x2*>(post.record);
            for (int i = 0; i < GnPostRecord::kWords / 2; ++i) to[i] = u64x2{r.w[2 * i], r.w[2 * i + 1]};
            *reinterpret_cast<volatile u64x2*>(post.word) = u64x2{tag, gn_post_sum(tag, r)};
        } else {
            __hip_atomic_store(post.word, tag, __ATOMIC_RELAXED, __HIP_MEMORY_SCOPE_SYSTEM);
        }
    }
}

__global__ __launch_bounds__(kBlock) void loam_solve_kernel(LoamSolveArgs a) {
    __shared__ double s_sum[kBlock / kAccW][kAccW];
    __shared__ double s_tot[2][kAccW];
    const int scan = a.scans ? a.scans[blockIdx.x] : (int)blockIdx.x;
    if (blockIdx.x == 0 && threadIdx.x < 4) {
        if (a.list_counts[0]) a.list_counts[0][threadIdx.x] = 0u;
        if (a.list_counts[1]) a.list_counts[1][threadIdx.x] = 0u;
    }
    if (a.st[scan].done) return;
#pragma unroll
    for (int c = 0; c < 2; ++c) {
        double t = 0.0;
        if (a.partials[c]) t = reduce_partials(a.partials[c] + (size_t)scan * a.blocks_per_scan[c] * kAccW, a.blocks_per_scan[c], true, s_sum);
        if (threadIdx.x < kAccW) s_tot[c][threadIdx.x] = t;
    }
    __syncthreads();
    if (threadIdx.x != 0) return;
    PoseState& ps = a.st[scan];
    double H[36], B[6], dx[6];
    long long eff[2] = {0, 0};
    bool ok[2] = {true, true};
#pragma unroll
    for (int c = 0; c < 2; ++c) {
        if (!a.partials[c]) continue;
        int o = 0;
        for (int i = 0; i < 6; ++i)
            for (int j = i; j < 6; ++j) { H[6 * i + j] = s_tot[c][o]; H[6 * j + i] = s_tot[c][o]; ++o; }
        for (int i = 0; i < 6; ++i) B[i] = s_tot[c][21 + i];
        eff[c] = (long long)s_tot[c][27];
        const double det_c = lu6_det_solve_reg(H, B, dx);
        ok[c] = (eff[c] >= a.min_effective_pts[c]) && !(det_c == 0.0);
    }
    {
        int o = 0;
        for (int i = 0; i < 6; ++i)
            for (int j = i; j < 6; ++j) { const double v = s_tot[0][o] + s_tot[1][o]; H[6 * i + j] = v; H[6 * j + i] = v; ++o; }
        for (int i = 0; i < 6; ++i) { B[i] = s_tot[0][21 + i] + s_tot[1][21 + i]; dx[i] = 0.0; }
    }
    if (a.hb_out) {
        double* hb = a.hb_out + (size_t)kLoamHbW * scan;
        for (int i = 0; i < 36; ++i) hb[i] = H[i];
        for (int i = 0; i < 6; ++i) hb[36 + i] = B[i];
        hb[42] = (double)eff[0]; hb[43] = (double)eff[1];
        hb[44] = ok[0] ? 1.0 : 0.0; hb[45] = ok[1] ? 1.0 : 0.0;
    }
    ps.last_eff = eff[0] + eff[1];
    if (!a.do_update) return;
    ps.iterations += 1;
    if (!ok[0] || !ok[1]) {
        ps.status = !ok[0] ? 3 : 4;
        ps.done = 1;
        return;
    }
    const double det = lu6_det_solve_reg(H, B, dx);
    if (!(det == 0.0)) {
        se3_apply_update(ps.q, ps.t, dx);
        quat_to_R(ps.q, ps.R);
        const double nrm = sqrt((dx[0] * dx[0] + (dx[2] * dx[2] + dx[4] * dx[4])) + (dx[1] * dx[1] + (dx[3] * dx[3] + dx[5] * dx[5])));
        ps.last_dx_norm = nrm;
        if (nrm < a.eps) { ps.converged = 1; ps.done = 1; }
    }
    if (ps.iterations >= a.max_iteration) ps.done = 1;
}

__global__ __launch_bounds__(kBlock) void sum_partials_kernel(const double* __restrict__ partials, int blocks_per_scan, const PoseState* __restrict__ st_all,
                                                              int first, int n_local, double* __restrict__ acc, const unsigned char* __restrict__ owned) {
    __shared__ double s_sum[kBlock / kAccW][kAccW];
    const int g = blockIdx.x;
    const int scan = g - first;
    const bool mine = scan >= 0 && scan < n_local && !st_all[g].done && (!owned || owned[g]);
    const double t = reduce_partials(partials + (size_t)(mine ? scan : 0) * blocks_per_scan * kAccW, blocks_per_scan, mine, s_sum);
    if (threadIdx.x < kAccW) acc[(size_t)g * kAccW + threadIdx.x] = threadIdx.x < 28 ? t : 0.0;
}

__global__ __launch_bounds__(kBlock) void transform_cloud_kernel(const float4* __restrict__ src, size_t n, M12f m, float* __restrict__ dst_xyz) {
    const size_t i = (size_t)blockIdx.x * kBlock + threadIdx.x;
    if (i >= n) return;
    const float4 p = src[i];
    const float* m12 = m.v;
    dst_xyz[3 * i + 0] = ((m12[0] * p.x + m12[1] * p.y) + m12[2] * p.z) + m12[3];
    dst_xyz[3 * i + 1] = ((m12[4] * p.x + m12[5] * p.y) + m12[6] * p.z) + m12[7];
    dst_xyz[3 * i + 2] = ((m12[8] * p.x + m12[9] * p.y) + m12[10] * p.z) + m12[11];
}

int plane_fit_mode() {
    static const int mode = [] { const char* e = getenv("LOCGPU_PLANE_FIT"); return e && *e ? atoi(e) : 1; }();
    return mode;
}
static bool plane_dedup() {
    static const bool on = env_int("LOCGPU_PLANE_DEDUP", 1) != 0;
    return on;
}

int icp_accum_split(int method, int max_n, int n_scans) {
    static_assert(kDedupPP >= 4, "the plane table of plane_accum_per_run has room for the largest plane rung below");
    const long total_blocks = (long)((max_n + kBlock - 1) / kBlock) * n_scans;
    return total_blocks >= 8192 ? (method == LOCGPU_P2PLANE ? 4 : 8) : (total_blocks >= 4096 ? 4 : (total_blocks >= 2048 ? 2 : 1));
}

int launch_icp_accum(int method, const AccumArgs& a, hipStream_t s) {
    const int blocks = (a.max_n + kBlock - 1) / kBlock;
    int pts = icp_accum_split(method, a.max_n, a.n_scans);
    if (a.split_scans > 0) pts = icp_accum_split(method, a.max_n, a.split_scans);
    const dim3 grid((blocks + pts - 1) / pts, a.active ? a.n_active : a.n_scans);
    if (method == LOCGPU_P2PLANE) {
        const bool secular = plane_fit_mode() == 1;
        auto kernel = plane_dedup() && pts <= kDedupPP ? (secular ? icp_plane_accum_kernel<1, true> : icp_plane_accum_kernel<0, true>)
                                    : (secular ? icp_plane_accum_kernel<1, false> : icp_plane_accum_kernel<0, false>);
        hipLaunchKernelGGL(kernel, grid, dim3(kBlock), 0, s, a.tree, a.src, a.counts, a.st, a.nn, a.nn_pitch, a.max_n, a.gate, a.partials, pts, a.active, a.src_of);
    } else if (method == LOCGPU_P2PLANE_MAP)
        hipLaunchKernelGGL(icp_mapplane_accum_kernel, grid, dim3(kBlock), 0, s, reinterpret_cast<const double4*>(a.planes), a.src, a.counts, a.st, a.nn, a.max_n, a.gate, a.partials, pts, a.active, a.src_of);
    else if (method == LOCGPU_P2LINE)
        hipLaunchKernelGGL(icp_line_accum_kernel, grid, dim3(kBlock), 0, s, a.tree, a.src, a.counts, a.st, a.nn, a.nn_pitch, a.max_n, a.gate, a.partials, pts, a.active, a.src_of);
    else
        hipLaunchKernelGGL(icp_point_accum_kernel, grid, dim3(kBlock), 0, s, a.tree, a.src, a.counts, a.st, a.nn, a.nn_pitch, a.max_n, a.gate, a.partials, pts, a.active, a.src_of);
    return (int)grid.x;
}

void launch_gn_solve(const double* partials, int blocks_per_scan, PoseState* st, int n_scans, const GnParams& prm, int do_update, double* hb_out,
                     unsigned int* list_counts, hipStream_t s, const int* scans, const GnPost* post) {
    hipLaunchKernelGGL(gn_solve_kernel, dim3(n_scans), dim3(kBlock), 0, s, partials, blocks_per_scan, st, prm, do_update, hb_out, list_counts, scans, post ? *post : GnPost{});
}

void launch_loam_solve(const LoamSolveArgs& a, int n_scans, hipStream_t s) {
    hipLaunchKernelGGL(loam_solve_kernel, dim3(n_scans), dim3(kBlock), 0, s, a);
}

void launch_sum_partials(const double* partials, int blocks_per_scan, const PoseState* st_all, int first, int n_local, int n_total, double* acc,
                         hipStream_t s, const unsigned char* owned) {
    hipLaunchKernelGGL(sum_partials_kernel, dim3(n_total), dim3(kBlock), 0, s, partials, blocks_per_scan, st_all, first, n_local, acc, owned);
}

void launch_transform_cloud(const float4* src, size_t n, const M12f& m12, float* dst_xyz, hipStream_t s) {
    hipLaunchKernelGGL(transform_cloud_kernel, dim3((unsigned)((n + kBlock - 1) / kBlock)), dim3(kBlock), 0, s, src, n, m12, dst_xyz);
}

}
```

loc_lib_amd/csrc/icp_kernels.hpp:

```cpp
#pragma once
#include <hip/hip_runtime.h>
#include <stdint.h>

#include "../../include/locgpu.h"
#include "device_math.hpp"

namespace locgpu {

constexpr int kBlock = 256;
constexpr int kAccW = 32;
constexpr uint32_t kInvalidSlot = 0xFFFFFFFFu;
constexpr int kSearchStatSlots = 16 + 2 * 64;

struct GnParams {
    int method;
    int max_iteration;
    int min_effective_pts;
    double eps;
    double max_nn_distance, max_plane_distance, max_line_distance;
    bool operator==(const GnParams& o) const {
        return method == o.method && max_iteration == o.max_iteration && min_effective_pts == o.min_effective_pts && eps == o.eps &&
               max_nn_distance == o.max_nn_distance && max_plane_distance == o.max_plane_distance && max_line_distance == o.max_line_distance;
    }
};
constexpr int kMethodNdtDirect = 3, kMethodNdtInc = 4;
constexpr bool method_is_ndt(int method) { return method == kMethodNdtDirect || method == kMethodNdtInc; }
static_assert(!method_is_ndt(LOCGPU_P2P) && !method_is_ndt(LOCGPU_P2LINE) && !method_is_ndt(LOCGPU_P2PLANE) && !method_is_ndt(LOCGPU_P2PLANE_MAP),
              "an NDT method value collides with a locgpu_icp_method");
constexpr int method_k(int method) { return method_is_ndt(method) ? 0 : ((method == LOCGPU_P2P || method == LOCGPU_P2PLANE_MAP) ? 1 : 5); }

__device__ __forceinline__ float as_f32(uint32_t u) { return __uint_as_float(u); }

__device__ __forceinline__ size_t src_index(const int* __restrict__ src_of, int scan, int max_n, int i) {
    return (size_t)(src_of ? src_of[scan] : scan) * max_n + i;
}

template <int NV, int W>
__device__ __forceinline__ void block_reduce_store(double (&acc)[NV], double* __restrict__ dst) {
    static_assert(NV <= W, "a value per LDS column");
    __shared__ double s_part[kBlock / 64][W];
    const int lane = threadIdx.x & 63, wave = threadIdx.x >> 6;
#pragma unroll
    for (int v = 0; v < NV; ++v) {
        const double s = wave_sum(acc[v]);
        if (lane == 0) s_part[wave][v] = s;
    }
    __syncthreads();
    if (threadIdx.x < NV) {
        double s = s_part[0][threadIdx.x];
#pragma unroll
        for (int w = 1; w < kBlock / 64; ++w) s += s_part[w][threadIdx.x];
        dst[threadIdx.x] = s;
    }
}

__device__ __forceinline__ void wave_append(uint32_t* __restrict__ list, unsigned int* __restrict__ count, bool pred, uint32_t value) {
    const unsigned long long mask = __ballot(pred);
    if (!mask) return;
    const int lane = (int)__lane_id();
    const int leader = __ffsll((long long)mask) - 1;
    unsigned int base = 0;
    if (lane == leader) base = atomicAdd(count, (unsigned int)__popcll(mask));
    base = (unsigned int)__shfl((int)base, leader, 64);
    if (pred) list[base + (unsigned int)__popcll(mask & ((1ull << lane) - 1ull))] = value;
}

template <int KMAX>
struct KnnHeap {
    float d[KMAX + 1];
    uint32_t id[KMAX + 1];
    int n;

    __device__ __forceinline__ float getd(int i) const {
        float r = d[0];
#pragma unroll
        for (int j = 1; j <= KMAX; ++j) {
            const float t = d[j];
            r = (i == j) ? t : r;
        }
        return r;
    }
    __device__ __forceinline__ uint32_t geti(int i) const {
        uint32_t r = id[0];
#pragma unroll
        for (int j = 1; j <= KMAX; ++j) {
            const uint32_t t = id[j];
            r = (i == j) ? t : r;
        }
        return r;
    }
    __device__ __forceinline__ void set(int i, float v, uint32_t w) {
#pragma unroll
        for (int j = 0; j <= KMAX; ++j) {
            const float od = d[j];
            const uint32_t oi = id[j];
            d[j] = (i == j) ? v : od;
            id[j] = (i == j) ? w : oi;
        }
    }
    __device__ __forceinline__ float top() const { return d[0]; }

    __device__ __forceinline__ void sift_up(int hole, float val, uint32_t w) {
        while (hole > 0) {
            const int parent = (hole - 1) / 2;
            const float pd = getd(parent);
            if (!(pd < val)) break;
            set(hole, pd, geti(parent));
            hole = parent;
        }
        set(hole, val, w);
    }
    __device__ __forceinline__ void push(float val, uint32_t w) {
        const int hole = n;
        n++;
        sift_up(hole, val, w);
    }
    __device__ __forceinline__ void pop() {
        const float value = getd(n - 1);
        const uint32_t vid = geti(n - 1);
        const int len = n - 1;
        int hole = 0, second = 0;
        while (second < (len - 1) / 2) {
            second = 2 * (second + 1);
            if (getd(second) < getd(second - 1)) second--;
            set(hole, getd(second), geti(second));
            hole = second;
        }
        if ((len & 1) == 0 && second == (len - 2) / 2) {
            second = 2 * (second + 1);
            set(hole, getd(second - 1), geti(second - 1));
            hole = second - 1;
        }
        sift_up(hole, value, vid);
        n--;
    }
};

template <>
struct KnnHeap<1> {
    float d[1];
    uint32_t id[1];
    int n;
    __device__ __forceinline__ float top() const { return d[0]; }
    __device__ __forceinline__ uint32_t geti(int) const { return id[0]; }
    __device__ __forceinline__ void push(float val, uint32_t w) {
        if (n == 0 || val < d[0]) { d[0] = val; id[0] = w; }
        n++;
    }
    __device__ __forceinline__ void pop() { n--; }
};

template <int KMAX, int D, bool COUNT>
__device__ __forceinline__ void tree_knn(const uint2* __restrict__ tree, float qx, float qy, float qz, int k, float alpha_eff,
                                         uint32_t (*s_far)[kBlock], float (*s_d2)[kBlock], int tid, KnnHeap<KMAX>& heap,
                                         uint32_t& nvis, uint32_t& lvis) {
    heap.n = 0;
    int sp = 0;
    uint32_t cur = 0;
    for (;;) {
        for (;;) {
            uint4 w;
            __builtin_memcpy(&w, tree + cur, 16);
            if (COUNT) nvis++;
            const uint32_t meta = w.y;
            const uint32_t tag = meta >> 30;
            if (tag == 3u) {
                if (COUNT) lvis++;
                const float dx = qx - as_f32(w.x), dy = qy - as_f32(w.z), dz = qz - as_f32(w.w);
                const float dis2 = dx * dx + (dy * dy + dz * dz);
                if (heap.n < k) {
                    heap.push(dis2, cur);
                } else if (dis2 < heap.top()) {
                    heap.push(dis2, cur);
                    heap.pop();
                }
                break;
            }
            const float th = as_f32(w.x);
            const float qa = tag == 0u ? qx : (tag == 1u ? qy : qz);
            const float dd = qa - th;
            const float d2 = dd * dd;
            const uint32_t right = meta & 0x3FFFFFFFu;
            const bool go_left = qa < th;
            const uint32_t far_slot = go_left ? right : cur + 1u;
            if (heap.n < k || d2 < heap.top() * alpha_eff) {
                s_far[sp][tid] = far_slot;
                s_d2[sp][tid] = d2;
                sp = sp + 1 < D ? sp + 1 : D - 1;
            }
            cur = go_left ? cur + 1u : right;
        }
        bool found = false;
        while (sp > 0) {
            sp--;
            const float d2 = s_d2[sp][tid];
            if (heap.n < k || d2 < heap.top() * alpha_eff) {
                cur = s_far[sp][tid];
                found = true;
                break;
            }
        }
        if (!found) break;
    }
}

template <int KMAX, int D, bool COUNT, int BLK = kBlock>
// ... 81 lines not shown
```

loc_lib_amd/csrc/icp_search.hip:

```cpp
#include "env.hpp"
#include "icp_kernels.hpp"
#include "launch.hpp"
#include "search_walk.hpp"

#include <algorithm>
#include <iterator>
#include <type_traits>
#include <utility>

namespace locgpu {

template <int KMAX, int D, bool COUNT>
__global__ __launch_bounds__(kBlock) void icp_search_kernel(const uint2* __restrict__ tree, const float4* __restrict__ src,
                                                            const int* __restrict__ counts, const PoseState* __restrict__ st,
                                                            uint32_t* __restrict__ nn, size_t nn_pitch, int max_n, int k, float alpha_eff,
                                                            int skip_nonfinite, unsigned long long* __restrict__ visit_totals, uint32_t* __restrict__ touched,
                                                            const int* __restrict__ active, const int* __restrict__ src_of) {
    __shared__ uint32_t s_far[D][kBlock];
    __shared__ float s_d2[D][kBlock];
    const int scan = active ? active[blockIdx.y] : (int)blockIdx.y;
    if (st[scan].done) return;
    const int tid = threadIdx.x;
    const int i = blockIdx.x * kBlock + tid;
    if (i >= counts[scan]) return;
    const size_t gi = (size_t)scan * max_n + i;
    const float4 p = src[src_index(src_of, scan, max_n, i)];
    uint32_t out[KMAX];
    int cnt = 0;
    uint32_t nvis = 0, lvis = 0;
    const bool finite = !skip_nonfinite || (isfinite(p.x) && isfinite(p.y) && isfinite(p.z));
    if (finite) {
        const D3 qs = se3_apply(st[scan].q, st[scan].t, D3{(double)p.x, (double)p.y, (double)p.z});
        KnnHeap<KMAX> heap;
        tree_knn_flat<KMAX, D, COUNT>(tree, (float)qs.x, (float)qs.y, (float)qs.z, k, alpha_eff, s_far, s_d2, tid, heap, nvis, lvis, touched);
        heap_to_sorted<KMAX>(heap, out, cnt);
    } else {
#pragma unroll
        for (int j = 0; j < KMAX; ++j) out[j] = kInvalidSlot;
    }
#pragma unroll
    for (int j = 0; j < KMAX; ++j)
        if (j < k) nn[(size_t)j * nn_pitch + gi] = out[j];
    if (COUNT) {
        atomicAdd(&visit_totals[0], (unsigned long long)nvis);
        atomicAdd(&visit_totals[1], (unsigned long long)lvis);
        atomicAdd(&visit_totals[2], 1ull);
    }
}

typedef float f32x4_nt __attribute__((ext_vector_type(4)));
__device__ __forceinline__ float4 load_once(const float4* __restrict__ p) {
    const f32x4_nt v = __builtin_nontemporal_load(reinterpret_cast<const f32x4_nt*>(p));
    return float4{v.x, v.y, v.z, v.w};
}

template <class T>
__device__ __forceinline__ float4 list_point(const float4* __restrict__ src, const int* __restrict__ src_of, int max_n, T gi, int& scan) {
    scan = (int)(gi / (T)max_n);
    return src_of ? src[(size_t)src_of[scan] * max_n + (gi - (T)scan * (T)max_n)] : src[gi];
}

template <int K, int ROWB, bool STAMP = false, int WIN = 0>
__device__ __forceinline__ void walk_query(__amdgpu_buffer_rsrc_t rsrc, const uint2* __restrict__ tree, Walk<K>& w, bool valid, float alpha_eff, int T, uint32_t dummy,
                                           uint32_t col_addr, int cap) {
#pragma unroll
    for (int j = 0; j < K; ++j) { w.d[j] = __builtin_inff(); w.id[j] = kInvalidSlot; }
    w.slow = 0;
    const bool sane = fabsf(w.qx) < 1e18f && fabsf(w.qy) < 1e18f && fabsf(w.qz) < 1e18f;
    if (valid && sane) {
        walk_descend<K, ROWB, WIN>(rsrc, tree, w, T, col_addr);
    } else {
        w.cur = dummy; w.avail = 0; w.c3n = 0; w.slow = valid ? 1u : 0u;
    }
#ifndef LOCGPU_K1_C
#define LOCGPU_K1_C 2
#endif
    walk_rounds_capped<K, ROWB, LOCGPU_K1_C, STAMP>(rsrc, w, alpha_eff, dummy, col_addr, cap);
#pragma unroll
    for (int j = 0; j + 1 < K; ++j) w.slow |= w.d[j] == w.d[j + 1] ? 1u : 0u;
}

template <int K>
__device__ __forceinline__ bool walk_exact_in_wave(const uint2* __restrict__ tree, bool slow, float qx, float qy, float qz, float alpha_eff, uint2* lds,
                                                   uint32_t* __restrict__ nn, size_t nn_pitch, size_t gi, unsigned long long* __restrict__ search_stats) {
    const unsigned long long slow_mask = __ballot(slow);
    if (slow_mask == 0ull || __popcll(slow_mask) > 2) return slow_mask == 0ull;
    if (slow) {
        uint32_t(*s_far)[2] = reinterpret_cast<uint32_t(*)[2]>(lds);
        float(*s_d2)[2] = reinterpret_cast<float(*)[2]>(reinterpret_cast<char*>(lds) + 64 * 2 * sizeof(uint32_t));
        const int col = __popcll(slow_mask & ((1ull << (threadIdx.x & 63)) - 1ull));
        KnnHeap<K> heap;
        uint32_t nvis = 0, lvis = 0, out[K];
        int cnt;
        tree_knn_flat<K, 64, false, 2>(tree, qx, qy, qz, K, alpha_eff, s_far, s_d2, col, heap, nvis, lvis);
        heap_to_sorted<K>(heap, out, cnt);
#pragma unroll
        for (int j = 0; j < K; ++j) nn[(size_t)j * nn_pitch + gi] = out[j];
        if (search_stats) atomicAdd(&search_stats[1], 1ull);
    }
    return true;
}

template <int K, int DF, int LANES = 64, bool STAMP = false, int WIN = 0>
__global__ __launch_bounds__(64) void icp_search_walk_kernel(const uint2* __restrict__ tree, const float4* __restrict__ src,
                                                             const int* __restrict__ counts, const PoseState* __restrict__ st,
                                                             uint32_t* __restrict__ nn, size_t nn_pitch, int max_n, float alpha_eff, int T,
                                                             unsigned int tree_bytes, uint32_t dummy, int skip_nonfinite, uint32_t* __restrict__ redo_list,
                                                             unsigned int* __restrict__ redo_count, uint32_t* __restrict__ deep_list,
                                                             unsigned int* __restrict__ deep_count, unsigned long long* __restrict__ search_stats,
                                                             const int* __restrict__ active, const int* __restrict__ src_of) {
    extern __shared__ uint2 s_dyn[];
    constexpr int ROWB = LANES * 8;
    static_assert(DF * ROWB >= 64 * 2 * 8, "exact stack columns do not fit");
    if ((uint32_t)(size_t)s_dyn != 0u) __builtin_trap();
    const int scan = active ? active[blockIdx.y] : (int)blockIdx.y;
    const int tid = threadIdx.x;
    if (st[scan].done) return;
    const int i = blockIdx.x * LANES + tid;
    if (tid >= LANES || i >= counts[scan]) return;
    const size_t gi = (size_t)scan * max_n + i;
    const float4 p = load_once(&src[src_index(src_of, scan, max_n, i)]);
    const bool finite = !skip_nonfinite || (isfinite(p.x) && isfinite(p.y) && isfinite(p.z));
    if (search_stats && finite) atomicAdd(&search_stats[0], 1ull);
    const D3 qs = se3_apply(st[scan].q, st[scan].t, D3{(double)p.x, (double)p.y, (double)p.z});
    const __amdgpu_buffer_rsrc_t rsrc = __builtin_amdgcn_make_buffer_rsrc((void*)tree, 0, (int)tree_bytes, 0x00020000);
    Walk<K> w;
    w.qx = (float)qs.x; w.qy = (float)qs.y; w.qz = (float)qs.z;
    static_assert(WIN <= DF - 2, "the window lies in the rows above the two candidate rows");
    walk_query<K, ROWB, STAMP, WIN>(rsrc, tree, w, finite, alpha_eff, T, dummy, (uint32_t)(size_t)(&s_dyn[tid]), DF);
    if (STAMP && search_stats) {
        atomicAdd(&search_stats[4], (unsigned long long)w.rounds);
        if ((tid & 63) == 0) { atomicAdd(&search_stats[9], (unsigned long long)w.wave_rounds); atomicAdd(&search_stats[12], 1ull); }
        atomicAdd(&search_stats[13], (unsigned long long)w.wave_rounds);
        redo_list[nn_pitch + gi] = w.rounds;
    }
    const bool deep = w.c3n == 1u;
    const bool slow = !deep && w.slow != 0u;
    if (!deep && !slow) {
#pragma unroll
        for (int j = 0; j < K; ++j) __builtin_nontemporal_store(w.id[j], &nn[(size_t)j * nn_pitch + gi]);
    }
    wave_append(deep_list, deep_count, deep, (uint32_t)gi);
    if (LANES == 16) {
        bool pending = slow;
        for (;;) {
            const unsigned long long m = __ballot(pending);
            if (m == 0ull) break;
            const bool mine = pending && __popcll(m & ((1ull << (threadIdx.x & 63)) - 1ull)) < 2;
            (void)walk_exact_in_wave<K>(tree, mine, w.qx, w.qy, w.qz, alpha_eff, s_dyn, nn, nn_pitch, gi, search_stats);
            pending = pending && !mine;
        }
    } else if (!walk_exact_in_wave<K>(tree, slow, w.qx, w.qy, w.qz, alpha_eff, s_dyn, nn, nn_pitch, gi, search_stats)) {
        wave_append(redo_list, redo_count, slow, (uint32_t)gi);
    }
}

template <int K, int D, int LANES = 64>
__global__ __launch_bounds__(64) void icp_search_walk_list_kernel(const uint2* __restrict__ tree, const float4* __restrict__ src,
                                                                  const PoseState* __restrict__ st, uint32_t* __restrict__ nn, size_t nn_pitch, int max_n,
                                                                  float alpha_eff, unsigned int tree_bytes, uint32_t dummy, const uint32_t* __restrict__ list,
                                                                  const unsigned int* __restrict__ n_list, uint32_t* __restrict__ redo_list,
                                                                  unsigned int* __restrict__ redo_count, unsigned long long* __restrict__ search_stats,
                                                                  const int* __restrict__ src_of) {
    extern __shared__ uint2 s_dyn[];
    constexpr int ROWB = LANES * 8;
    static_assert((D + 2) * ROWB >= 64 * 2 * 8, "exact stack columns do not fit");
    if ((uint32_t)(size_t)s_dyn != 0u) __builtin_trap();
    const unsigned int n = *n_list;
    const int tid = threadIdx.x;
    if (blockIdx.x == 0 && tid == 0 && search_stats) atomicAdd(&search_stats[2], (unsigned long long)n);
    if (tid >= LANES) return;
    const __amdgpu_buffer_rsrc_t rsrc = __builtin_amdgcn_make_buffer_rsrc((void*)tree, 0, (int)tree_bytes, 0x00020000);
    const unsigned int per_wave = min((unsigned int)LANES, max(1u, (n + gridDim.x - 1) / gridDim.x));
    for (unsigned int r0 = blockIdx.x * per_wave; r0 < n; r0 += gridDim.x * per_wave) {
        const unsigned int r = r0 + (unsigned int)tid;
        const bool valid = (unsigned int)tid < per_wave && r < n;
        const uint32_t gi = valid ? list[r] : 0u;
        Walk<K> w;
        w.qx = w.qy = w.qz = 0.f;
        if (valid) {
            int scan;
            const float4 p = list_point(src, src_of, max_n, gi, scan);
            const D3 qs = se3_apply(st[scan].q, st[scan].t, D3{(double)p.x, (double)p.y, (double)p.z});
            w.qx = (float)qs.x; w.qy = (float)qs.y; w.qz = (float)qs.z;
        }
        walk_query<K, ROWB>(rsrc, tree, w, valid, alpha_eff, 0, dummy, (uint32_t)(size_t)(&s_dyn[tid]), 0x7fffffff);
        const bool slow = valid && w.slow != 0u;
        if (valid && !slow) {
#pragma unroll
            for (int j = 0; j < K; ++j) nn[(size_t)j * nn_pitch + gi] = w.id[j];
        }
        if (!walk_exact_in_wave<K>(tree, slow, w.qx, w.qy, w.qz, alpha_eff, s_dyn, nn, nn_pitch, gi, search_stats))
            wave_append(redo_list, redo_count, slow, gi);
    }
}

constexpr int kRedoWaves = 2048;
constexpr int kDeepLanes = 64, kDeepWaves = 2048;
template <int KMAX, int D>
__global__ __launch_bounds__(64) void icp_search_redo_kernel(const uint2* __restrict__ tree, const float4* __restrict__ src,
                                                             const PoseState* __restrict__ st, uint32_t* __restrict__ nn, size_t nn_pitch,
                                                             int max_n, int k, float alpha_eff, const uint32_t* __restrict__ redo_list,
                                                             const unsigned int* __restrict__ redo_count, unsigned long long* __restrict__ search_stats,
                                                             const int* __restrict__ src_of) {
    __shared__ uint32_t s_far[D][64];
    __shared__ float s_d2[D][64];
    const unsigned int n = *redo_count;
    const int tid = threadIdx.x;
    if (blockIdx.x == 0 && tid == 0 && search_stats) atomicAdd(&search_stats[1], (unsigned long long)n);
    const unsigned int per_wave = min(64u, (n + gridDim.x - 1) / gridDim.x);
    if ((unsigned)tid >= per_wave) return;
    for (unsigned int r = blockIdx.x * per_wave + tid; r < n; r += gridDim.x * per_wave) {
        const size_t gi = redo_list[r];
        int scan;
        const float4 p = list_point(src, src_of, max_n, gi, scan);
        const D3 qs = se3_apply(st[scan].q, st[scan].t, D3{(double)p.x, (double)p.y, (double)p.z});
        KnnHeap<KMAX> heap;
        uint32_t nvis = 0, lvis = 0, out[KMAX];
        int cnt;
        tree_knn_flat<KMAX, D, false, 64>(tree, (float)qs.x, (float)qs.y, (float)qs.z, k, alpha_eff, s_far, s_d2, tid, heap, nvis, lvis);
        heap_to_sorted<KMAX>(heap, out, cnt);
#pragma unroll
        for (int j = 0; j < KMAX; ++j)
            if (j < k) nn[(size_t)j * nn_pitch + gi] = out[j];
    }
}

template <int KMAX, int D>
__global__ __launch_bounds__(kBlock) void knn_query_kernel(const uint2* __restrict__ tree, const float* __restrict__ queries, size_t nq,
                                                           int k, float alpha_eff, int32_t* __restrict__ out_idx,
                                                           uint32_t* __restrict__ visits) {
    __shared__ uint32_t s_far[D][kBlock];
    __shared__ float s_d2[D][kBlock];
    const int tid = threadIdx.x;
    const size_t i = (size_t)blockIdx.x * kBlock + tid;
    if (i >= nq) return;
    KnnHeap<KMAX> heap;
    uint32_t nvis = 0, lvis = 0;
    tree_knn<KMAX, D, true>(tree, queries[3 * i], queries[3 * i + 1], queries[3 * i + 2], k, alpha_eff, s_far, s_d2, tid, heap, nvis, lvis);
    uint32_t out[KMAX];
    int cnt;
    heap_to_sorted<KMAX>(heap, out, cnt);
#pragma unroll
    for (int j = 0; j < KMAX; ++j)
        if (j < k) out_idx[i * k + j] = (out[j] == kInvalidSlot) ? -1 : (int32_t)(tree[out[j]].y & 0x3FFFFFFFu);
    if (visits) { visits[2 * i] = nvis; visits[2 * i + 1] = lvis; }
}

__global__ __launch_bounds__(kBlock) void count_touched_kernel(uint32_t* __restrict__ touched, size_t n_words, unsigned long long* __restrict__ totals) {
    unsigned long long c = 0;
    for (size_t i = (size_t)blockIdx.x * kBlock + threadIdx.x; i < n_words; i += (size_t)gridDim.x * kBlock) {
        c += (unsigned long long)__popc(touched[i]);
        touched[i] = 0u;
    }
    for (int off = 32; off > 0; off >>= 1) c += __shfl_xor(c, off, 64);
    if ((threadIdx.x & 63) == 0 && c) atomicAdd(&totals[3], c);
}

__global__ __launch_bounds__(kBlock) void nn_to_index_kernel(const uint2* __restrict__ tree, uint32_t tree_slots, const uint32_t* __restrict__ nn, size_t nn_pitch,
                                                             const int* __restrict__ counts, int max_n, size_t n_queries, int k, int32_t* __restrict__ out) {
    const size_t gi = (size_t)blockIdx.x * kBlock + threadIdx.x;
    if (gi >= n_queries) return;
    const bool live = (int)(gi % (size_t)max_n) < counts[gi / (size_t)max_n];
    for (int j = 0; j < k; ++j) {
        const uint32_t slot = live ? nn[(size_t)j * nn_pitch + gi] : kInvalidSlot;
        out[gi * k + j] = (slot == kInvalidSlot || slot >= tree_slots) ? -1 : (int32_t)(tree[slot].y & 0x3FFFFFFFu);
    }
}


template <class F>
static bool with_depth(int depth, F&& f) {
    if (depth <= 32) f(std::integral_constant<int, 32>{});
    else if (depth <= 40) f(std::integral_constant<int, 40>{});
    else if (depth <= 64) f(std::integral_constant<int, 64>{});
    else return false;
    return true;
}
template <bool UP_TO, class F>
static bool with_k(int k, F&& f) {
    if (k == 1) return f(std::integral_constant<int, 1>{});
    if (UP_TO ? k <= 5 : k == 5) return f(std::integral_constant<int, 5>{});
    if constexpr (UP_TO)
        if (k <= 8) return f(std::integral_constant<int, 8>{});
    return false;
}

bool stamp_build() {
    static const bool on = env_int("LOCGPU_STAMP", 0) != 0;
    return on;
}

void launch_nn_to_index(const uint2* tree, size_t tree_slots, const uint32_t* nn, size_t nn_pitch, const int* counts, int max_n, size_t n_queries, int k,
                        int32_t* out, hipStream_t s) {
    if (n_queries == 0 || max_n <= 0) return;
    hipLaunchKernelGGL(nn_to_index_kernel, dim3((unsigned)((n_queries + kBlock - 1) / kBlock)), dim3(kBlock), 0, s, tree, (uint32_t)tree_slots, nn, nn_pitch, counts, max_n,
                       n_queries, k, out);
}

void launch_count_touched(uint32_t* touched, size_t n_words, unsigned long long* totals, hipStream_t s) {
    hipLaunchKernelGGL(count_touched_kernel, dim3(1024), dim3(kBlock), 0, s, touched, n_words, totals);
}

template <int KMAX, int D, bool COUNT>
static void launch_exact(const SearchArgs& a, hipStream_t s) {
    dim3 grid((a.max_n + kBlock - 1) / kBlock, a.active ? a.n_active : a.n_scans);
    hipLaunchKernelGGL((icp_search_kernel<KMAX, D, COUNT>), grid, dim3(kBlock), 0, s, a.tree, a.src, a.counts, a.st, a.nn, a.nn_pitch, a.max_n,
                       a.k, a.alpha_eff, a.skip_nonfinite, a.visit_totals, COUNT ? a.touched : nullptr, a.active, a.src_of);
}

struct WalkShape { int df, win; };
constexpr WalkShape kWalkShapes[] = {{10, 8}, {12, 0}, {15, 0}, {24, 0}};
template <class F, size_t... I>
static bool all_walk_shapes(F&& f, std::index_sequence<I...>) {
    return (f(std::integral_constant<int, kWalkShapes[I].df>{}, std::integral_constant<int, kWalkShapes[I].win>{}) && ...);
}
template <class F>
static bool all_walk_shapes(F&& f) { return all_walk_shapes(f, std::make_index_sequence<std::size(kWalkShapes)>{}); }

static int fast_stack_depth() {
    static const int v = [] {
        const int e = env_int("LOCGPU_FAST_STACK", kWalkShapes[0].df);
        for (const WalkShape& w : kWalkShapes)
            if (w.df == e) return e;
        return kWalkShapes[0].df;
    }();
    return v;
}
constexpr int kWindowStored = 13;

template <auto Kernel>
static bool no_static_lds() {
    hipFuncAttributes attr{};
    return hipFuncGetAttributes(&attr, reinterpret_cast<const void*>(Kernel)) == hipSuccess && attr.sharedSizeBytes == 0;
}
template <int K>
static bool walk_kernels_ok() {
    bool ok = all_walk_shapes([](auto DF, auto WIN) {
        return no_static_lds<icp_search_walk_kernel<K, DF(), 64, false, WIN()>>() && no_static_lds<icp_search_walk_kernel<K, DF(), 64, true, WIN()>>();
    });
    for (int depth : {32, 40, 64})
        with_depth(depth, [&](auto D) { ok = ok && no_static_lds<icp_search_walk_kernel<K, D() + 2, 16>>() && no_static_lds<icp_search_walk_list_kernel<K, D(), kDeepLanes>>(); });
    return ok;
}
bool search_kernels_lds_ok() {
    static const bool ok = walk_kernels_ok<1>() && walk_kernels_ok<5>();
    return ok;
}

template <int K, int D>
static void launch_redo(const SearchArgs& a, hipStream_t s) {
    hipLaunchKernelGGL((icp_search_redo_kernel<K, D>), dim3(kRedoWaves), dim3(64), 0, s, a.tree, a.src, a.st, a.nn, a.nn_pitch, a.max_n, a.k,
                       a.alpha_eff, a.redo_list, a.redo_count, a.search_stats, a.src_of);
}
template <int K, int D>
static void launch_walk_list(const SearchArgs& a, const uint32_t* list, const unsigned int* n_list, hipStream_t s) {
    hipLaunchKernelGGL((icp_search_walk_list_kernel<K, D, kDeepLanes>), dim3(kDeepWaves), dim3(64), (D + 2) * kDeepLanes * 8, s, a.tree, a.src, a.st, a.nn, a.nn_pitch, a.max_n,
                       a.alpha_eff, (unsigned int)a.tree_bytes + 16u, (uint32_t)(a.tree_bytes / 8), list, n_list, a.redo_list, a.redo_count, a.search_stats, a.src_of);
}

template <int K, int D, int DF, int WIN>
static void launch_walk(const SearchArgs& a, hipStream_t s) {
    const bool stamp = stamp_build();
    const uint32_t dummy = (uint32_t)(a.tree_bytes / 8);
    const unsigned int rsrc_bytes = (unsigned int)a.tree_bytes + 16u;
    const int n_launch = a.active ? a.n_active : a.n_scans;
    if (!stamp && (size_t)((a.max_n + 63) / 64) * n_launch <= 2048) {
        dim3 g1((a.max_n + 15) / 16, n_launch);
        hipLaunchKernelGGL((icp_search_walk_kernel<K, D + 2, 16>), g1, dim3(64), (D + 2) * 16 * 8, s, a.tree, a.src, a.counts, a.st, a.nn, a.nn_pitch, a.max_n,
                           a.alpha_eff, 0, rsrc_bytes, dummy, a.skip_nonfinite, a.redo_list, a.redo_count, a.redo_list2, a.redo_count2, a.search_stats, a.active, a.src_of);
        return;
    }
    const int stored = WIN ? kWindowStored : DF - 2;
    const int Tw = a.depth > stored ? a.depth - stored : 0;
    dim3 g2((a.max_n + 63) / 64, n_launch);
    static const bool lds_knob = env_flag("LOCGPU_K1_LDS_BYTES");
    unsigned lds_bytes = DF * 64 * 8;
    if (lds_knob) lds_bytes = (unsigned)std::max(env_int("LOCGPU_K1_LDS_BYTES", 0), DF * 64 * 8);
    if (stamp)
        hipLaunchKernelGGL((icp_search_walk_kernel<K, DF, 64, true, WIN>), g2, dim3(64), DF * 64 * 8, s, a.tree, a.src, a.counts, a.st, a.nn, a.nn_pitch, a.max_n,
                           a.alpha_eff, Tw, rsrc_bytes, dummy, a.skip_nonfinite, a.redo_list, a.redo_count, a.redo_list2, a.redo_count2, a.search_stats, a.active, a.src_of);
    else
        hipLaunchKernelGGL((icp_search_walk_kernel<K, DF, 64, false, WIN>), g2, dim3(64), lds_bytes, s, a.tree, a.src, a.counts, a.st, a.nn, a.nn_pitch, a.max_n,
                           a.alpha_eff, Tw, rsrc_bytes, dummy, a.skip_nonfinite, a.redo_list, a.redo_count, a.redo_list2, a.redo_count2, a.search_stats, a.active, a.src_of);
    launch_walk_list<K, D>(a, a.redo_list2, a.redo_count2, s);
    launch_redo<K, D>(a, s);
}

bool launch_icp_search(const SearchArgs& a, hipStream_t s) {
    const bool exact_only = a.visit_totals != nullptr || !a.redo_list || !a.redo_list2;
    return with_k<false>(a.k, [&](auto Kc) {
        return with_depth(a.depth, [&](auto Dc) {
            constexpr int K = decltype(Kc)::value, D = decltype(Dc)::value;
            if (exact_only) return a.visit_totals ? launch_exact<K, D, true>(a, s) : launch_exact<K, D, false>(a, s);
            all_walk_shapes([&](auto DF, auto WIN) {
                if (DF() != fast_stack_depth()) return true;
                launch_walk<K, D, DF(), WIN()>(a, s);
                return false;
            });
        });
    });
}

bool launch_icp_search_redo(const SearchArgs& a, hipStream_t s) {
    return with_k<false>(a.k, [&](auto Kc) {
        return with_depth(a.depth, [&](auto Dc) { launch_redo<decltype(Kc)::value, decltype(Dc)::value>(a, s); });
    });
}

bool launch_icp_search_list(const SearchArgs& a, const uint32_t* list, const unsigned int* n_list, hipStream_t s) {
    return with_k<false>(a.k, [&](auto Kc) {
        return with_depth(a.depth, [&](auto Dc) {
            constexpr int K = decltype(Kc)::value, D = decltype(Dc)::value;
            launch_walk_list<K, D>(a, list, n_list, s);
            launch_redo<K, D>(a, s);
        });
    });
}

bool launch_knn_query(const uint2* tree, int depth, const float* q, size_t nq, int k, float alpha_eff, int32_t* out, uint32_t* visits,
                      hipStream_t s) {
    return with_k<true>(k, [&](auto Kc) {
        return with_depth(depth, [&](auto Dc) {
            hipLaunchKernelGGL((knn_query_kernel<decltype(Kc)::value, decltype(Dc)::value>), dim3((unsigned)((nq + kBlock - 1) / kBlock)), dim3(kBlock), 0, s, tree, q, nq, k,
                               alpha_eff, out, visits);
        });
    });
}

}
```

loc_lib_amd/csrc/launch.hpp:

```cpp
#pragma once
#include "gn_post.hpp"
#include <hip/hip_runtime.h>
#include <stdint.h>

#include "device_math.hpp"

namespace locgpu {

struct GnParams;

struct SearchArgs {
    const uint2* tree;
    size_t tree_bytes;
    int depth;
    const float4* src;
    const int* counts;
    const PoseState* st;
    uint32_t* nn;
    size_t nn_pitch;
    int max_n, n_scans, k;
    float alpha_eff;
    int skip_nonfinite;
    unsigned long long* visit_totals;
    uint32_t* redo_list;
    unsigned int* redo_count;
    uint32_t* redo_list2;
    unsigned int* redo_count2;
    unsigned long long* search_stats;
    const int* active = nullptr;
    int n_active = 0;
    const int* src_of = nullptr;
    uint32_t* touched = nullptr;
};

struct AccumArgs {
    const uint2* tree;
    const float4* src;
    const int* counts;
    const PoseState* st;
    const uint32_t* nn;
    size_t nn_pitch;
    int max_n, n_scans;
    double gate;
    double* partials;
    const int* active = nullptr;
    int n_active = 0;
    const int* src_of = nullptr;
    int split_scans = 0;
    const double* planes = nullptr;
};

bool launch_icp_search(const SearchArgs& a, hipStream_t s);
bool launch_icp_search_redo(const SearchArgs& a, hipStream_t s);
bool launch_icp_search_list(const SearchArgs& a, const uint32_t* list, const unsigned int* n_list, hipStream_t s);
bool launch_knn_query(const uint2* tree, int depth, const float* q, size_t nq, int k, float alpha_eff, int32_t* out, uint32_t* visits,
                      hipStream_t s);
int launch_icp_accum(int method, const AccumArgs& a, hipStream_t s);
void launch_gn_solve(const double* partials, int blocks_per_scan, PoseState* st, int n_scans, const GnParams& prm, int do_update, double* hb_out,
                     unsigned int* list_counts, hipStream_t s, const int* scans = nullptr, const GnPost* post = nullptr);
constexpr int kLoamHbW = 46;
struct LoamSolveArgs {
    const double* partials[2];
    int blocks_per_scan[2];
    int min_effective_pts[2];
    unsigned int* list_counts[2];
    int max_iteration;
    double eps;
    PoseState* st;
    int do_update;
    double* hb_out;
    const int* scans;
};
void launch_loam_solve(const LoamSolveArgs& a, int n_scans, hipStream_t s);
int icp_accum_split(int method, int max_n, int n_scans);
void launch_sum_partials(const double* partials, int blocks_per_scan, const PoseState* st_all, int first, int n_local, int n_total, double* acc,
                         hipStream_t s, const unsigned char* owned = nullptr);
constexpr int kFitW = 4;
struct FitnessArgs {
    const uint2* tree;
    const float4* src;
    const int* counts;
    const PoseState* st;
    const uint32_t* nn;
    int max_n, n_scans;
    float gate2;
    double* partials;
    double* out;
    unsigned int* list_counts;
    const int* src_of = nullptr;
};
int icp_fitness_rows(int max_n);
void launch_icp_fitness(const FitnessArgs& a, hipStream_t s);
int launch_icp_fitness_accum(const FitnessArgs& a, hipStream_t s);
void launch_loam_fitness_sum(const double* const partials[2], const int rows[2], int n_cands, double* out, unsigned int* const list_counts[2], hipStream_t s);
void launch_fitness_sum(const double* partials, int rows, int n_scans, double* out, unsigned int* list_counts, hipStream_t s);
struct M12f { float v[12]; };
void launch_transform_cloud(const float4* src, size_t n, const M12f& m12, float* dst_xyz, hipStream_t s);
void launch_loam_join_transform(const float4* edge, size_t n_edge, const float4* surf, size_t n_surf, const M12f& m12, float4* out, hipStream_t s);
void launch_map_plane_queries(const uint2* tree, const uint32_t* leaf_slots, size_t first, int n, float4* src, int* counts, hipStream_t s);
void launch_map_plane_fit(const uint2* tree, const uint32_t* leaf_slots, size_t first, int n, const uint32_t* nn, size_t nn_pitch, double* planes,
                          unsigned long long* n_valid, hipStream_t s);
void launch_map_plane_dump(const uint2* tree, const uint32_t* leaf_slots, size_t n_leaves, const double* planes, size_t n_points, double* out_n4,
                           unsigned char* out_valid, hipStream_t s);
bool search_kernels_lds_ok();
bool stamp_build();
void launch_count_touched(uint32_t* touched, size_t n_words, unsigned long long* totals, hipStream_t s);
void launch_nn_to_index(const uint2* tree, size_t tree_slots, const uint32_t* nn, size_t nn_pitch, const int* counts, int max_n, size_t n_queries, int k,
                        int32_t* out, hipStream_t s);

}
```

loc_lib_amd/csrc/locgpu_api.hip:

```cpp
#include <algorithm>
#include <atomic>
#include <cmath>
#include <cstdio>
#include <cstdlib>
#include <cstring>
#include <string>
#include <vector>

#include "batch_upload.hpp"
#include "cloud_filters.hpp"
#include "context.hpp"
#include "gn_driver.hpp"
#include "launch.hpp"
#include "ndt_inc.hpp"
#include "ndt_kernels.hpp"
#include "search_chunks.hpp"

using namespace locgpu;

namespace {
std::string g_create_err;
}

namespace locgpu {
// ... 59 lines not shown

int locgpu_create(int device_id, locgpu_ctx** out) {
    if (!out) return fail(nullptr, LOCGPU_ERR_INVALID, "locgpu_create: out is NULL");
    *out = nullptr;
    int n = 0;
    hipError_t e = hipGetDeviceCount(&n);
    if (e != hipSuccess || n <= 0)
        return fail(nullptr, LOCGPU_ERR_NO_DEVICE, std::string("no HIP device available (there is no CPU fallback): ") + hipGetErrorString(e));
    if (device_id < 0 || device_id >= n) return fail(nullptr, LOCGPU_ERR_INVALID, "locgpu_create: device_id out of range");
    auto* ctx = new locgpu_ctx();
    ctx->device = device_id;
    locgpu_ndt_opts_default(&ctx->ndt_opts);
    bool ok = hip_ok(nullptr, hipSetDevice(device_id), "hipSetDevice");
    for (int i = 0; ok && i < locgpu_ctx::kSlots; ++i) ok = hip_ok(nullptr, hipStreamCreateWithFlags(&ctx->slot_stream[i], hipStreamNonBlocking), "hipStreamCreate");
    ok = ok && hip_ok(nullptr, hipStreamCreateWithFlags(&ctx->copy_stream, hipStreamNonBlocking), "hipStreamCreate");
    ok = ok && hip_ok(nullptr, hipStreamCreateWithFlags(&ctx->comm_stream, hipStreamNonBlocking), "hipStreamCreate");
    if (!ok) {
        for (hipStream_t st : ctx->slot_stream) if (st) (void)hipStreamDestroy(st);
        if (ctx->copy_stream) (void)hipStreamDestroy(ctx->copy_stream);
        if (ctx->comm_stream) (void)hipStreamDestroy(ctx->comm_stream);
        delete ctx;
        return LOCGPU_ERR_NO_DEVICE;
    }
    ctx->stream = ctx->slot_stream[0];
    if (!search_kernels_lds_ok()) {
        locgpu_destroy(ctx);
        return fail(nullptr, LOCGPU_ERR_INVALID, "locgpu_create: a search kernel of this build owns static LDS — its traversal stack would not start at LDS address 0 (search_walk.hpp)");
    }
    *out = ctx;
    return LOCGPU_OK;
}

void locgpu_destroy(locgpu_ctx* ctx) {
    if (!ctx) return;
    (void)hipSetDevice(ctx->device);
    (void)target_join(ctx, false);
    free_target_scratch(ctx);
    for (hipStream_t st : ctx->slot_stream) if (st) (void)hipStreamSynchronize(st);
    if (ctx->comm_stream) (void)hipStreamSynchronize(ctx->comm_stream);
    delete ctx->worker;
    free_batch(ctx->single);
    free_batch(ctx->search);
    free_batch(ctx->planes_ws);
    upload_free_ctx(ctx);
    comm_destroy(ctx);
    if (ctx->comm_stream) (void)hipStreamDestroy(ctx->comm_stream);
    if (ctx->copy_stream) (void)hipStreamDestroy(ctx->copy_stream);
    free_grid(ctx);
    ndt_free(ctx);
    filters_free(ctx);
    loam_free(ctx);
    range_ingest_free(ctx);
    for (hipStream_t st : ctx->slot_stream) if (st) (void)hipStreamDestroy(st);
    delete ctx;
}

const char* locgpu_last_error(const locgpu_ctx* ctx) { return ctx ? ctx->err.c_str() : g_create_err.c_str(); }

int locgpu_knn(locgpu_ctx* ctx, const float* queries, size_t nq, int k, int approximate, float alpha, int search_mode, int32_t* out_idx,
               uint32_t* visits) {
    if (!ctx) return LOCGPU_ERR_INVALID;
    { const int jrc = target_join(ctx); if (jrc != LOCGPU_OK) return jrc; }
    if (!ctx->d_tree) return fail(ctx, LOCGPU_ERR_NO_TARGET, "knn: no target set");
    if (!queries || !out_idx || k < 1 || k > 8) return fail(ctx, LOCGPU_ERR_INVALID, "knn: bad arguments (1 <= k <= 8)");
    if (search_mode != LOCGPU_SEARCH_TREE_FAITHFUL && search_mode != LOCGPU_SEARCH_GRID_EXACT) return fail(ctx, LOCGPU_ERR_INVALID, "knn: unknown search mode");
    if ((size_t)k > ctx->num_leaves) return fail(ctx, LOCGPU_ERR_K_TOO_LARGE, "knn: k larger than the number of tree leaves");
    if (nq == 0) return LOCGPU_OK;
    LOCGPU_HIP(ctx, hipSetDevice(ctx->device));
    const bool grid = search_mode == LOCGPU_SEARCH_GRID_EXACT;
    if (grid) {
        if (k != 1 && k != 5) return fail(ctx, LOCGPU_ERR_INVALID, "knn: grid search supports k = 1 or 5");
        const int grc = ensure_grid(ctx);
        if (grc != LOCGPU_OK) return grc;
    }
    DevBuf<float> d_q;
    DevBuf<int32_t> d_out;
    DevBuf<uint32_t> d_vis;
    DevBuf<unsigned int> d_flag;
    int rc = LOCGPU_OK;
    if (!hip_ok(ctx, d_q.alloc(nq * 3), "hipMalloc") || !hip_ok(ctx, d_out.alloc(nq * k), "hipMalloc") || !hip_ok(ctx, d_flag.alloc(1), "hipMalloc") ||
        (visits && !hip_ok(ctx, d_vis.alloc(nq * 2), "hipMalloc")))
        return LOCGPU_ERR_OOM;
    hipStream_t s = ctx->stream;
    if (!hip_ok(ctx, hipMemcpyAsync(d_q, queries, nq * 12, hipMemcpyHostToDevice, s), "H2D")) rc = LOCGPU_ERR_NO_DEVICE;
    if (rc == LOCGPU_OK && grid) {
        unsigned int flagged = 0;
        (void)hipMemsetAsync(d_flag, 0, 4, s);
        if (!launch_knn_grid_query(ctx->grid, ctx->d_tree, d_q, nq, k, d_out, d_flag, s)) rc = fail(ctx, LOCGPU_ERR_INVALID, "knn: unsupported k");
        if (rc == LOCGPU_OK && (!hip_ok(ctx, hipMemcpyAsync(out_idx, d_out, nq * k * 4, hipMemcpyDeviceToHost, s), "D2H") ||
                                !hip_ok(ctx, hipMemcpyAsync(&flagged, d_flag, 4, hipMemcpyDeviceToHost, s), "D2H") ||
                                !hip_ok(ctx, hipStreamSynchronize(s), "sync")))
            rc = LOCGPU_ERR_NO_DEVICE;
        if (rc == LOCGPU_OK && visits) std::memset(visits, 0, nq * 8);
        if (rc == LOCGPU_OK && flagged) {
            std::vector<int32_t> tmp(nq * k);
            if (!launch_knn_query(ctx->d_tree, ctx->depth, d_q, nq, k, 1.0f, d_out, nullptr, s)) rc = fail(ctx, LOCGPU_ERR_DEPTH, "knn: unsupported k/depth");
            if (rc == LOCGPU_OK && (!hip_ok(ctx, hipMemcpyAsync(tmp.data(), d_out, nq * k * 4, hipMemcpyDeviceToHost, s), "D2H") ||
                                    !hip_ok(ctx, hipStreamSynchronize(s), "sync")))
                rc = LOCGPU_ERR_NO_DEVICE;
            if (rc == LOCGPU_OK)
                for (size_t i = 0; i < nq; ++i)
                    if (out_idx[i * k] == -2)
                        for (int j = 0; j < k; ++j) out_idx[i * k + j] = tmp[i * k + j];
        }
        return rc;
    }
    if (rc == LOCGPU_OK && !launch_knn_query(ctx->d_tree, ctx->depth, d_q, nq, k, approximate ? alpha : 1.0f, d_out, d_vis, s))
        rc = fail(ctx, LOCGPU_ERR_DEPTH, "knn: unsupported k/depth");
    if (rc == LOCGPU_OK && !hip_ok(ctx, hipGetLastError(), "knn launch")) rc = LOCGPU_ERR_NO_DEVICE;
    if (rc == LOCGPU_OK && !hip_ok(ctx, hipMemcpyAsync(out_idx, d_out, nq * k * 4, hipMemcpyDeviceToHost, s), "D2H")) rc = LOCGPU_ERR_NO_DEVICE;
    if (rc == LOCGPU_OK && visits && !hip_ok(ctx, hipMemcpyAsync(visits, d_vis, nq * 8, hipMemcpyDeviceToHost, s), "D2H")) rc = LOCGPU_ERR_NO_DEVICE;
    if (!hip_ok(ctx, hipStreamSynchronize(s), "sync") && rc == LOCGPU_OK) rc = LOCGPU_ERR_NO_DEVICE;
    return rc;
}

}

int locgpu::alloc_batch(locgpu_ctx* ctx, int n_scans, size_t max_n, locgpu_batch** out, int first, int n_total, bool shared_src) {
    if (!ctx || !out) return LOCGPU_ERR_INVALID;
    *out = nullptr;
    const bool sharded = n_total >= 0;
    if (!sharded) n_total = n_scans;
    if (shared_src && (sharded || n_scans < 1)) return fail(ctx, LOCGPU_ERR_INVALID, "batch_create: a shared-source batch cannot be sharded or empty");
    if (n_scans < 0 || (n_scans == 0 && !sharded) || first < 0 || first + n_scans > n_total) return fail(ctx, LOCGPU_ERR_INVALID, "batch_create: bad arguments");
    if (n_total > 65535) return fail(ctx, LOCGPU_ERR_INVALID, "batch_create: at most 65535 scans per batch");
    if (n_scans > 65535) return fail(ctx, LOCGPU_ERR_INVALID, "batch_create: at most 65535 scans per batch");
    LOCGPU_HIP(ctx, hipSetDevice(ctx->device));
    if (n_scans == 0) max_n = 1;
    if (max_n == 0 || max_n > 0x7FFFFF00u || (size_t)n_scans * max_n > 0xFFFFFFF0ull)
        return fail(ctx, LOCGPU_ERR_INVALID, "batch_create: scans are empty or the batch exceeds 2^32 points");
    auto* b = new locgpu_batch();
    b->ctx = ctx;
    b->slot = ctx->next_slot;
    ctx->next_slot = (ctx->next_slot + 1) % locgpu_ctx::kSlots;
    b->stream = ctx->slot_stream[b->slot];
    b->n_scans = n_scans;
    b->n_total = n_total;
    b->first = first;
    b->sharded = sharded;
    b->max_n = (int)max_n;
    b->blocks_per_scan = (int)((max_n + kBlock - 1) / kBlock);
    b->pitch = (size_t)n_scans * max_n;
    b->counts.assign(n_scans, 0);
    b->shared_src = shared_src;
    b->cap_scans = n_scans;
    b->cap_points = max_n;
    bool ok = hip_ok(ctx, b->d_src.alloc(std::max<size_t>(shared_src ? max_n : b->pitch, 1)), "hipMalloc src") &&
              (!shared_src || (hip_ok(ctx, b->d_src_of.alloc((size_t)n_scans), "hipMalloc src_of") &&
                               fill_now(ctx, b->d_src_of, (size_t)n_scans * sizeof(int), "hipMemset src_of"))) &&
              hip_ok(ctx, b->d_counts.alloc(std::max(n_scans, 1)), "hipMalloc counts") &&
              hip_ok(ctx, b->d_state.alloc(n_total), "hipMalloc state") &&
              (!sharded || hip_ok(ctx, b->d_acc.alloc((size_t)kFirstChunk * n_total * kAccW), "hipMalloc acc")) &&
              hip_ok(ctx, b->d_nn.alloc(5 * std::max<size_t>(b->pitch, 1)), "hipMalloc nn") &&
              hip_ok(ctx, b->d_partials.alloc((size_t)std::max(n_scans, 1) * b->blocks_per_scan * kAccW), "hipMalloc partials") &&
              hip_ok(ctx, b->d_hb.alloc((size_t)n_total * 44), "hipMalloc hb") &&
              hip_ok(ctx, b->d_redo_list.alloc((stamp_build() ? 2 : 1) * std::max<size_t>(b->pitch, 1)), "hipMalloc redo") &&
              hip_ok(ctx, b->d_redo_list2.alloc(std::max<size_t>(b->pitch, 1)), "hipMalloc redo2") &&
              hip_ok(ctx, b->d_redo_count.alloc(4), "hipMalloc redo") &&
              hip_ok(ctx, b->h_state.alloc(n_total), "hipHostMalloc state") &&
              hip_ok(ctx, b->h_hb.alloc((size_t)n_total * 44), "hipHostMalloc hb") &&
              hip_ok(ctx, b->h_active.alloc((size_t)std::max(n_scans, 1)), "hipHostMalloc active") &&
              hip_ok(ctx, b->d_active.alloc((size_t)std::max(n_scans, 1)), "hipMalloc active") &&
              fill_now(ctx, b->d_counts, std::max(n_scans, 1) * sizeof(int), "hipMemset counts") &&
              fill_now(ctx, b->d_redo_count, 4 * sizeof(unsigned int), "hipMemset redo");
    if (!ok) { free_batch(b); return LOCGPU_ERR_OOM; }
    *out = b;
    return LOCGPU_OK;
}

extern "C" {

static int make_batch(locgpu_ctx* ctx, const void* const* srcs, const size_t* counts, size_t stride_bytes, int n_scans, locgpu_batch** out,
                      int first = 0, int n_total = -1) {
    if (!ctx || !out) return LOCGPU_ERR_INVALID;
    *out = nullptr;
    if (n_scans < 0 || (n_scans > 0 && (!srcs || !counts)) || stride_bytes < 12) return fail(ctx, LOCGPU_ERR_INVALID, "batch_create: bad arguments");
    size_t max_n = 0;
    for (int s = 0; s < n_scans; ++s) max_n = std::max(max_n, counts[s]);
    for (int s = 0; s < n_scans; ++s)
        if (!srcs[s] && counts[s]) return fail(ctx, LOCGPU_ERR_INVALID, "batch_create: NULL scan pointer");
    locgpu_batch* b = nullptr;
    int rc = alloc_batch(ctx, n_scans, max_n, &b, first, n_total);
    if (rc != LOCGPU_OK) return rc;
    if (n_scans > 0) {
        rc = upload_start(b, srcs, counts, stride_bytes);
        if (rc == LOCGPU_OK) rc = upload_join_batch(b);
        if (rc == LOCGPU_OK && !hip_ok(ctx, upload_wait_landed(b), "batch_create: H2D")) rc = LOCGPU_ERR_NO_DEVICE;
    }
    if (rc != LOCGPU_OK) { free_batch(b); return rc; }
    *out = b;
    return LOCGPU_OK;
}

int locgpu_batch_create(locgpu_ctx* ctx, const void* const* srcs, const size_t* counts, size_t stride_bytes, int n_scans, locgpu_batch** out) {
    return make_batch(ctx, srcs, counts, stride_bytes, n_scans, out);
}

int locgpu_batch_create_empty(locgpu_ctx* ctx, int n_scans, size_t max_points_per_scan, locgpu_batch** out) {
    return alloc_batch(ctx, n_scans, max_points_per_scan, out);
}

int locgpu_batch_upload_async(locgpu_batch* b, const void* const* srcs, const size_t* counts, size_t stride_bytes) {
    if (!b) return LOCGPU_ERR_INVALID;
    if (b->shared_src) return fail(b->ctx, LOCGPU_ERR_INVALID, "batch upload: a shared-source batch takes its cloud when it is created");
    LOCGPU_HIP(b->ctx, hipSetDevice(b->ctx->device));
    return upload_start(b, srcs, counts, stride_bytes);
}

int locgpu_batch_upload_wait(locgpu_batch* b) {
    if (!b) return LOCGPU_ERR_INVALID;
    return upload_join_batch(b);
}

int locgpu_batch_create_sharded(locgpu_ctx* ctx, const void* const* srcs, const size_t* counts, size_t stride_bytes, int n_local, int first_scan,
                                int n_total, locgpu_batch** out) {
    if (!ctx) return LOCGPU_ERR_INVALID;
    if (n_total <= 0) return fail(ctx, LOCGPU_ERR_INVALID, "batch_create_sharded: n_total must be positive");
    if (!ctx->comm && !(first_scan == 0 && n_local == n_total))
        return fail(ctx, LOCGPU_ERR_INVALID, "batch_create_sharded: this rank holds only part of the batch and locgpu_comm_init has not been called");
    const int rc = make_batch(ctx, srcs, counts, stride_bytes, n_local, out, first_scan, n_total);
    if (rc != LOCGPU_OK) return rc;
    locgpu_batch* b = *out;
    if (!hip_ok(ctx, b->ev_ready.ensure(), "batch_create_sharded: hipEventCreate") || !hip_ok(ctx, b->ev_reduced.ensure(), "batch_create_sharded: hipEventCreate")) {
        free_batch(b);
        *out = nullptr;
        return LOCGPU_ERR_OOM;
    }
    return LOCGPU_OK;
}

void locgpu_batch_destroy(locgpu_batch* b) {
    if (!b) return;
    (void)hipSetDevice(b->ctx->device);
    (void)hipStreamSynchronize(b->stream);
    if (b->sharded && b->ctx->comm_stream) (void)hipStreamSynchronize(b->ctx->comm_stream);
    free_batch(b);
}

}

namespace locgpu {

static int check_batch(locgpu_ctx* ctx, const locgpu_batch* b, bool args_ok, const AlignSpec& spec, const char* who) {
    if (!b || b->ctx != ctx || !args_ok) return fail(ctx, LOCGPU_ERR_INVALID, std::string(who) + ": bad arguments");
    if (b->sharded && spec.prm.method == LOCGPU_P2PLANE_MAP)
        return fail(ctx, LOCGPU_ERR_INVALID, "icp: LOCGPU_P2PLANE_MAP is not available on a sharded batch");
    return LOCGPU_OK;
}

int check_icp(locgpu_ctx* ctx, const locgpu_icp_opts* o, AlignSpec& spec) {
    if (!ctx) return LOCGPU_ERR_INVALID;
    if (!o) return fail(ctx, LOCGPU_ERR_INVALID, "icp: opts is NULL");
    { const int jrc = target_join(ctx); if (jrc != LOCGPU_OK) return jrc; }
    if (!ctx->d_tree) return fail(ctx, LOCGPU_ERR_NO_TARGET, "icp: SetInputTarget has not been called");
    if ((o->method < LOCGPU_P2P || o->method > LOCGPU_P2PLANE) && o->method != LOCGPU_P2PLANE_MAP) return fail(ctx, LOCGPU_ERR_INVALID, "icp: unknown method");
    if (o->search_mode != LOCGPU_SEARCH_TREE_FAITHFUL && o->search_mode != LOCGPU_SEARCH_GRID_EXACT)
        return fail(ctx, LOCGPU_ERR_INVALID, "icp: unknown search mode");
    if (o->search_mode == LOCGPU_SEARCH_GRID_EXACT) {
        const int rc = ensure_grid(ctx);
        if (rc != LOCGPU_OK) return rc;
    }
    GnParams& prm = spec.prm;
    prm.method = o->method;
    prm.max_iteration = o->max_iteration;
    prm.min_effective_pts = o->min_effective_pts;
    prm.eps = o->eps;
    prm.max_nn_distance = o->max_nn_distance;
    prm.max_plane_distance = o->max_plane_distance;
    prm.max_line_distance = o->max_line_distance;
    if (o->method == LOCGPU_P2PLANE_MAP) {
        const int rc = ensure_map_planes(ctx);
        if (rc != LOCGPU_OK) return rc;
    }
    spec.grid = o->search_mode == LOCGPU_SEARCH_GRID_EXACT;
    spec.alpha = (o->approximate && !spec.grid) ? o->ann_alpha : 1.0f;
    return LOCGPU_OK;
}

static int single_reserve(locgpu_ctx* ctx, size_t n, locgpu_batch** out) {
    if (n == 0) return fail(ctx, LOCGPU_ERR_INVALID, "source cloud is empty");
    locgpu_batch* b = ctx->single;
    if (!b || (size_t)b->max_n < n || !b->h_src) {
        if (b) { free_batch(b); ctx->single = nullptr; }
        const size_t cap = with_headroom(n);
        const int rc = alloc_batch(ctx, 1, cap, &ctx->single);
        if (rc != LOCGPU_OK) return rc;
        b = ctx->single;
        b->slot = 0;
        b->stream = ctx->stream;
        b->pinned = true;
        if (!hip_ok(ctx, b->h_src.alloc(cap), "hipHostMalloc src")) { free_batch(b); ctx->single = nullptr; return LOCGPU_ERR_OOM; }
    }
    *out = b;
    return LOCGPU_OK;
}

static int single_batch(locgpu_ctx* ctx, const void* src, size_t n, size_t stride_bytes, locgpu_batch** out) {
    if (n == 0) return fail(ctx, LOCGPU_ERR_INVALID, "source cloud is empty");
    if (!src || stride_bytes < 12) return fail(ctx, LOCGPU_ERR_INVALID, "source cloud: NULL pointer or stride < 12");
    locgpu_batch* b = nullptr;
    const int rc = single_reserve(ctx, n, &b);
    if (rc != LOCGPU_OK) return rc;
    pack_points((const char*)src, stride_bytes, n, b->h_src);
    b->d_src_ext = nullptr;
    b->counts[0] = (int)n;
    LOCGPU_HIP(ctx, hipMemcpyAsync(b->d_src, b->h_src, n * sizeof(float4), hipMemcpyHostToDevice, b->stream));
    LOCGPU_HIP(ctx, hipMemcpyAsync(b->d_counts, b->counts.data(), sizeof(int), hipMemcpyHostToDevice, b->stream));
    *out = b;
    return LOCGPU_OK;
}

static int single_batch_dev(locgpu_ctx* ctx, const float4* d_src, size_t n, locgpu_batch** out) {
    locgpu_batch* b = nullptr;
    const int rc = single_reserve(ctx, n, &b);
    if (rc != LOCGPU_OK) return rc;
    b->counts[0] = (int)n;
    b->d_src_ext = ctx->use_graph ? nullptr : d_src;
    if (!b->d_src_ext) LOCGPU_HIP(ctx, hipMemcpyAsync(b->d_src, d_src, n * sizeof(float4), hipMemcpyDeviceToDevice, b->stream));
    LOCGPU_HIP(ctx, hipMemcpyAsync(b->d_counts, b->counts.data(), sizeof(int), hipMemcpyHostToDevice, b->stream));
    *out = b;
    return LOCGPU_OK;
}

static int align_single(locgpu_ctx* ctx, const AlignSpec& spec, const char* who, bool args_ok, const void* src, size_t n, size_t stride_bytes,
                        const locgpu_cloud* cloud, const double init_pose[7], double out_pose[7], locgpu_align_stats* stats) {
    if (!args_ok) return fail(ctx, LOCGPU_ERR_INVALID, std::string(who) + ": bad arguments");
    locgpu_batch* b = nullptr;
    int rc;
    if (cloud) {
        const hipError_t ce = cloud_input_ready(ctx, cloud);
        if (ce == hipErrorInvalidDevice) return fail(ctx, LOCGPU_ERR_INVALID, std::string(who) + ": the cloud belongs to a context on another GPU");
        if (!hip_ok(ctx, ce, (std::string(who) + ": ordering behind the cloud's context").c_str())) return LOCGPU_ERR_NO_DEVICE;
        rc = single_batch_dev(ctx, cloud->d, cloud->n, &b);
    } else {
        rc = single_batch(ctx, src, n, stride_bytes, &b);
    }
    return rc != LOCGPU_OK ? rc : run_align(ctx, b, init_pose, spec, out_pose, stats);
}

}

extern "C" {

int locgpu_icp_align_batch(locgpu_ctx* ctx, locgpu_batch* b, const double* init_poses, const locgpu_icp_opts* opts, double* out_poses,
                           locgpu_align_stats* stats) {
    AlignSpec spec;
    int rc = check_icp(ctx, opts, spec);
    if (rc == LOCGPU_OK) rc = check_batch(ctx, b, init_poses && out_poses, spec, "icp_align_batch");
    return rc != LOCGPU_OK ? rc : run_align(ctx, b, init_poses, spec, out_poses, stats);
}

int locgpu_icp_align_batch_begin(locgpu_ctx* ctx, locgpu_batch* b, const double* init_poses, const locgpu_icp_opts* opts) {
    AlignSpec spec;
    int rc = check_icp(ctx, opts, spec);
    if (rc == LOCGPU_OK) rc = check_batch(ctx, b, init_poses != nullptr, spec, "icp_align_batch_begin");
    return rc != LOCGPU_OK ? rc : align_begin(ctx, b, init_poses, spec);
}

int locgpu_align_batch_end(locgpu_ctx* ctx, locgpu_batch* b, double* out_poses, locgpu_align_stats* stats) {
    if (!ctx) return LOCGPU_ERR_INVALID;
    if (!b || b->ctx != ctx || !out_poses) return fail(ctx, LOCGPU_ERR_INVALID, "align_batch_end: bad arguments");
    return align_finish(ctx, b, out_poses, stats);
}

int locgpu_icp_align(locgpu_ctx* ctx, const void* src, size_t n, size_t stride_bytes, const double init_pose[7], const locgpu_icp_opts* opts,
                     double out_pose[7], locgpu_align_stats* stats) {
    AlignSpec spec;
    const int rc = check_icp(ctx, opts, spec);
    return rc != LOCGPU_OK ? rc : align_single(ctx, spec, "icp_align", src && init_pose && out_pose, src, n, stride_bytes, nullptr, init_pose, out_pose, stats);
}

int locgpu_icp_hb_batch(locgpu_ctx* ctx, locgpu_batch* b, const double* poses, const locgpu_icp_opts* opts, double* hb) {
    AlignSpec spec;
    int rc = check_icp(ctx, opts, spec);
    if (rc == LOCGPU_OK) rc = check_batch(ctx, b, poses && hb, spec, "icp_hb_batch");
    return rc != LOCGPU_OK ? rc : eval_hb_batch(ctx, b, poses, spec, hb, "icp_hb_batch");
}

int locgpu_debug_batch_nn(locgpu_ctx* ctx, locgpu_batch* b, int k, int32_t* out) {
    if (!ctx || !b || b->ctx != ctx || !out || k < 1 || k > 5) return fail(ctx, LOCGPU_ERR_INVALID, "debug_batch_nn: bad arguments");
    { const int jrc = target_join(ctx); if (jrc != LOCGPU_OK) return jrc; }
    if (!ctx->d_tree) return fail(ctx, LOCGPU_ERR_NO_TARGET, "debug_batch_nn: no ICP target");
    LOCGPU_HIP(ctx, hipSetDevice(ctx->device));
    const size_t nq = (size_t)b->n_scans * b->max_n;
    DevBuf<int32_t> d_out;
    LOCGPU_HIP(ctx, d_out.alloc(nq * k));
    launch_nn_to_index(ctx->d_tree, ctx->tree_slots, b->d_nn, b->pitch, b->d_counts, b->max_n, nq, k, d_out, b->stream);
    const hipError_t e = hipMemcpyAsync(out, d_out, nq * k * sizeof(int32_t), hipMemcpyDeviceToHost, b->stream);
    const hipError_t e2 = hipStreamSynchronize(b->stream);
    LOCGPU_HIP(ctx, e);
    LOCGPU_HIP(ctx, e2);
    return LOCGPU_OK;
}

int locgpu_icp_hb(locgpu_ctx* ctx, const void* src, size_t n, size_t stride_bytes, const double pose[7], const locgpu_icp_opts* opts, double H[36],
                  double B[6], int64_t* effective_num, int* ok) {
    AlignSpec spec;
    int rc = check_icp(ctx, opts, spec);
    if (rc != LOCGPU_OK) return rc;
    if (!src || !pose || !H || !B) return fail(ctx, LOCGPU_ERR_INVALID, "icp_hb: bad arguments");
    locgpu_batch* b = nullptr;
    rc = single_batch(ctx, src, n, stride_bytes, &b);
    if (rc != LOCGPU_OK) return rc;
    double hb[44];
    rc = eval_hb_batch(ctx, b, pose, spec, hb, "icp_hb");
    if (rc != LOCGPU_OK) return rc;
    std::memcpy(H, hb, 36 * sizeof(double));
    std::memcpy(B, hb + 36, 6 * sizeof(double));
    if (effective_num) *effective_num = (int64_t)hb[42];
    if (ok) *ok = hb[43] != 0.0;
    return LOCGPU_OK;
}

int locgpu_icp_build_map_planes(locgpu_ctx* ctx) {
    if (!ctx) return LOCGPU_ERR_INVALID;
    { const int jrc = target_join(ctx); if (jrc != LOCGPU_OK) return jrc; }
    if (!ctx->d_tree) return fail(ctx, LOCGPU_ERR_NO_TARGET, "icp_build_map_planes: SetInputTarget has not been called");
    return ensure_map_planes(ctx);
}

int locgpu_icp_map_planes_info(const locgpu_ctx* ctx, int64_t out[3]) {
    if (!ctx || !out) return LOCGPU_ERR_INVALID;
    { const int jrc = target_join(const_cast<locgpu_ctx*>(ctx)); if (jrc != LOCGPU_OK) return jrc; }
    out[0] = out[1] = out[2] = 0;
    if (!ctx->d_tree) return LOCGPU_ERR_NO_TARGET;
    if (!ctx->planes_ready) return LOCGPU_OK;
    out[0] = (int64_t)ctx->planes_rows;
    out[1] = (int64_t)ctx->planes_valid;
    out[2] = (int64_t)((ctx->tree_slots / 2 + 2) * 4 * sizeof(double));
    return LOCGPU_OK;
}

int locgpu_icp_map_planes_dump(locgpu_ctx* ctx, double* n4, uint8_t* valid, size_t cap, size_t* n_out) {
    if (!ctx) return LOCGPU_ERR_INVALID;
    int rc = locgpu_icp_build_map_planes(ctx);
    if (rc != LOCGPU_OK) return rc;
    const size_t n = ctx->num_points;
    if (n_out) *n_out = n;
    if (!n4 && !valid && cap == 0 && n_out) return LOCGPU_OK;
    if (!n4 || !valid || cap < n) return fail(ctx, LOCGPU_ERR_INVALID, "icp_map_planes_dump: NULL output or capacity below the number of target points");
    DevBuf<double> d_n4;
    DevBuf<unsigned char> d_valid;
    hipStream_t s = ctx->stream;
    bool ok = hip_ok(ctx, d_n4.alloc(std::max<size_t>(n, 1) * 4), "hipMalloc") && hip_ok(ctx, d_valid.alloc(std::max<size_t>(n, 1)), "hipMalloc");
    if (!ok) rc = LOCGPU_ERR_OOM;
    ok = ok && hip_ok(ctx, hipMemsetAsync(d_n4, 0, n * 4 * sizeof(double), s), "hipMemset") && hip_ok(ctx, hipMemsetAsync(d_valid, 0, n, s), "hipMemset");
    if (ok && ctx->num_leaves > 0) launch_map_plane_dump(ctx->d_tree, ctx->d_leaf_slots, ctx->num_leaves, ctx->d_planes, n, d_n4, d_valid, s);
    ok = ok && hip_ok(ctx, hipGetLastError(), "map_planes_dump launch") && hip_ok(ctx, hipMemcpyAsync(n4, d_n4, n * 4 * sizeof(double), hipMemcpyDeviceToHost, s), "D2H") &&
         hip_ok(ctx, hipMemcpyAsync(valid, d_valid, n, hipMemcpyDeviceToHost, s), "D2H");
    if (!hip_ok(ctx, hipStreamSynchronize(s), "sync")) ok = false;
    return ok ? LOCGPU_OK : (rc != LOCGPU_OK ? rc : LOCGPU_ERR_NO_DEVICE);
}

int locgpu_gn_update(const double hb[44], int method, int min_effective_pts, double eps, double pose[7], double dx[6], int* applied, int* stop) {
    if (!hb || !pose || !dx) return LOCGPU_ERR_INVALID;
    for (int i = 0; i < 6; ++i) dx[i] = 0.0;
    if (applied) *applied = 0;
    if (stop) *stop = 0;
    const double det = lu6_det_solve(hb, hb + 36, dx);
    const bool ok = ((long long)hb[42] >= min_effective_pts) && !(det == 0.0);
    if (!ok) { for (int i = 0; i < 6; ++i) dx[i] = 0.0; return LOCGPU_OK; }
    if (method == LOCGPU_P2P)
        for (int i = 0; i < 6; ++i) dx[i] = dx[i] / 16;
    se3_apply_update(pose, pose + 4, dx);
    double n2 = 0.0;
    for (int i = 0; i < 6; ++i) n2 += dx[i] * dx[i];
    if (applied) *applied = 1;
    if (stop) *stop = std::sqrt(n2) < eps;
    return LOCGPU_OK;
}

static int write_output_cloud(locgpu_ctx* ctx, locgpu_batch* b, const float4* d_points, size_t n, const double pose[7], void* out, size_t out_stride) {
    double R[9];
    quat_to_R(pose, R);
    M12f m;
    for (int r = 0; r < 3; ++r) {
        for (int c = 0; c < 3; ++c) m.v[4 * r + c] = (float)R[3 * r + c];
        m.v[4 * r + 3] = (float)pose[4 + r];
    }
    float* d_xyz = reinterpret_cast<float*>(b->d_nn.get());
    float* h_xyz = reinterpret_cast<float*>(b->h_src.get());
    launch_transform_cloud(d_points, n, m, d_xyz, b->stream);
    LOCGPU_HIP(ctx, hipGetLastError());
    constexpr int kMaxPieces = 8;
    const size_t piece = std::max<size_t>(32 * 1024, (n + kMaxPieces - 1) / kMaxPieces);
    const int pieces = (int)((n + piece - 1) / piece);
    for (int p = 0; p < pieces; ++p) {
        LOCGPU_HIP(ctx, b->xyz_ev[p].ensure());
        const size_t lo = (size_t)p * piece, len = std::min(piece, n - lo);
        LOCGPU_HIP(ctx, hipMemcpyAsync(h_xyz + 3 * lo, d_xyz + 3 * lo, len * 3 * sizeof(float), hipMemcpyDeviceToHost, b->stream));
        LOCGPU_HIP(ctx, hipEventRecord(b->xyz_ev[p], b->stream));
    }
    char* ob = (char*)out;
    std::atomic<int> failed{0};
    auto scatter = [&, ob, h_xyz](int first) {
        for (int p = first; p < pieces; p += 2) {
            if (hipEventSynchronize(b->xyz_ev[p]) != hipSuccess) { failed = 1; return; }
            const size_t lo = (size_t)p * piece, hi = std::min(n, lo + piece);
            for (size_t i = lo; i < hi; ++i) std::memcpy(ob + i * out_stride, h_xyz + 3 * i, 12);
        }
    };
    if (ctx->worker) ctx->worker->wait();
    const bool two = pieces > 1 && ctx->worker;
    if (two) ctx->worker->run([&] { (void)hipSetDevice(ctx->device); scatter(1); });
    scatter(0);
    if (two) ctx->worker->wait(); else if (pieces > 1) scatter(1);
    if (failed) return fail(ctx, LOCGPU_ERR_NO_DEVICE, "output cloud: copy back");
    return LOCGPU_OK;
}

static void scan_match_fields(locgpu_ctx* ctx, const void* src, size_t n, size_t src_stride, void* out, size_t out_stride, locgpu_out_cloud_fn out_fn,
                              void* user, void** dst) {
    *dst = out;
    if (out_stride & LOCGPU_OUT_FIELDS_DONE) {
        if (!out_fn) return;
        if (!ctx->worker) ctx->worker = new locgpu::HostWorker();
        ctx->worker->run([=] { *dst = out_fn(user, n); });
        return;
    }
    if ((!out && !out_fn) || (!out_fn && out == src) || n == 0) return;
    if (!ctx->worker) ctx->worker = new locgpu::HostWorker();
    ctx->worker->run([=] {
        void* o = out_fn ? out_fn(user, n) : out;
        *dst = o;
        if (!o || o == src) return;
        if (src_stride == out_stride) { std::memcpy(o, src, n * src_stride); return; }
        const size_t w = std::min(src_stride, out_stride);
        const char* sb = (const char*)src;
        char* ob = (char*)o;
        for (size_t i = 0; i < n; ++i) std::memcpy(ob + i * out_stride, sb + i * src_stride, w);
    });
}
static int scan_match_output(locgpu_ctx* ctx, locgpu_batch* b, size_t n, int rc, const double pose[7], void** dst, size_t out_stride) {
    if (ctx->worker) ctx->worker->wait();
    if (rc != LOCGPU_OK || !*dst) return rc;
    return write_output_cloud(ctx, b, b->d_src, n, pose, *dst, out_stride & ~LOCGPU_OUT_FIELDS_DONE);
}

static int scan_match(locgpu_ctx* ctx, const AlignSpec& spec, const char* who, const void* src, size_t n, size_t stride_bytes, const double init_pose[7],
                      double result_pose[7], locgpu_align_stats* stats, void* out_cloud, size_t out_stride_bytes, locgpu_out_cloud_fn out_fn, void* out_user) {
    if (!src || !init_pose || !result_pose || ((out_cloud || out_fn) && (out_stride_bytes & ~LOCGPU_OUT_FIELDS_DONE) < 12)) return fail(ctx, LOCGPU_ERR_INVALID, std::string(who) + ": bad arguments");
    locgpu_batch* b = nullptr;
    int rc = single_batch(ctx, src, n, stride_bytes, &b);
    if (rc != LOCGPU_OK) return rc;
// ... 568 lines not shown
```

Baseline: 13470 scans/s.

## Emit plane-run leader flags from KNN search and consume them in plane accumulation

```diff
diff --git a/include/locgpu.h b/include/locgpu.h
--- a/include/locgpu.h
+++ b/include/locgpu.h
@@ -231,6 +231,7 @@
 
 LOCGPU_API int locgpu_search_stats_read(locgpu_ctx* ctx, uint64_t out[4], int reset);
 LOCGPU_API int locgpu_debug_batch_nn(locgpu_ctx* ctx, locgpu_batch* batch, int k, int32_t* out);
+LOCGPU_API int locgpu_debug_batch_run_flags(locgpu_ctx* ctx, locgpu_batch* batch, uint64_t* out, int* written);
 LOCGPU_API int locgpu_debug_batch_slot(const locgpu_batch* batch);
 
 typedef struct locgpu_cloud locgpu_cloud;
diff --git a/loc_lib_amd/api.py b/loc_lib_amd/api.py
--- a/loc_lib_amd/api.py
+++ b/loc_lib_amd/api.py
@@ -20,7 +20,7 @@
     "locgpu_transform_cloud", "locgpu_batch_create", "locgpu_batch_destroy", "locgpu_icp_align_batch", "locgpu_ndt_align_batch",
     "locgpu_icp_hb_batch", "locgpu_gn_update", "locgpu_ndt_set_target", "locgpu_ndt_target_info", "locgpu_ndt_dump",
     "locgpu_ndt_align", "locgpu_profile_enable", "locgpu_profile_read", "locgpu_visit_count_enable", "locgpu_visit_count_read",
-    "locgpu_search_stats_read", "locgpu_debug_batch_nn", "locgpu_debug_batch_slot", "locgpu_graph_enable",
+    "locgpu_search_stats_read", "locgpu_debug_batch_nn", "locgpu_debug_batch_run_flags", "locgpu_debug_batch_slot", "locgpu_graph_enable",
     "locgpu_cloud_create", "locgpu_cloud_destroy", "locgpu_cloud_upload", "locgpu_cloud_info", "locgpu_cloud_download", "locgpu_cloud_copy",
     "locgpu_cloud_remove_nan", "locgpu_cloud_voxel_filter", "locgpu_cloud_crop_box", "locgpu_cloud_transform", "locgpu_cloud_append",
     "locgpu_icp_set_target_cloud", "locgpu_icp_set_target_cloud_async", "locgpu_ndt_set_target_cloud", "locgpu_icp_align_cloud", "locgpu_ndt_align_cloud",
@@ -137,7 +137,7 @@
             "locgpu_ndt_dump": (i32, [vp, vp, vp, vp, sz, vp]), "locgpu_ndt_align": (i32, [vp, vp, sz, sz, vp, vp, vp]),
             "locgpu_profile_enable": (i32, [vp, i32]), "locgpu_profile_read": (i32, [vp, vp, i32]),
             "locgpu_visit_count_enable": (i32, [vp, i32]), "locgpu_visit_count_read": (i32, [vp, vp, i32]),
-            "locgpu_search_stats_read": (i32, [vp, vp, i32]), "locgpu_debug_batch_nn": (i32, [vp, vp, i32, vp]), "locgpu_debug_batch_slot": (i32, [vp]), "locgpu_graph_enable": (i32, [vp, i32]),
+            "locgpu_search_stats_read": (i32, [vp, vp, i32]), "locgpu_debug_batch_nn": (i32, [vp, vp, i32, vp]), "locgpu_debug_batch_run_flags": (i32, [vp, vp, vp, vp]), "locgpu_debug_batch_slot": (i32, [vp]), "locgpu_graph_enable": (i32, [vp, i32]),
             "locgpu_cloud_create": (i32, [vp, vp]), "locgpu_cloud_destroy": (None, [vp]),
             "locgpu_cloud_upload": (i32, [vp, vp, sz, sz, sz, i32]), "locgpu_cloud_info": (i32, [vp, vp, vp]),
             "locgpu_cloud_download": (i32, [vp, vp, sz, sz, sz]), "locgpu_cloud_copy": (i32, [vp, vp]),
@@ -668,6 +668,12 @@
         self._check(lib().locgpu_debug_batch_nn(self._h, batch._h, int(k), out.ctypes.data))
         return out
 
+    def debug_batch_run_flags(self, batch):
+        out = np.zeros((batch.n_local, (batch.max_points + 63) // 64), dtype=np.uint64)
+        written = ctypes.c_int(0)
+        self._check(lib().locgpu_debug_batch_run_flags(self._h, batch._h, out.ctypes.data, ctypes.byref(written)))
+        return out, bool(written.value)
+
     def search_stats_read(self, reset=True):
         out = np.zeros(4, dtype=np.uint64)
         self._check(lib().locgpu_search_stats_read(self._h, out.ctypes.data, int(reset)))
diff --git a/loc_lib_amd/csrc/context.hpp b/loc_lib_amd/csrc/context.hpp
--- a/loc_lib_amd/csrc/context.hpp
+++ b/loc_lib_amd/csrc/context.hpp
@@ -132,6 +132,8 @@
     bool rings_valid = false;
     locgpu::DevBuf<locgpu::PoseState> d_state;
     locgpu::DevBuf<uint32_t> d_nn;
+    locgpu::DevBuf<unsigned long long> d_run_flags;
+    bool run_flags_written = false;
     bool shared_src = false;
     locgpu::DevBuf<int> d_src_of;
     int cap_scans = 0, split_scans = 0;
diff --git a/loc_lib_amd/csrc/gn_driver.hip b/loc_lib_amd/csrc/gn_driver.hip
--- a/loc_lib_amd/csrc/gn_driver.hip
+++ b/loc_lib_amd/csrc/gn_driver.hip
@@ -29,6 +29,11 @@
                   skip_nonfinite ? 1 : 0, nullptr, b->d_redo_list, b->d_redo_count, b->d_redo_list2, b->d_redo_count + 1, ctx->d_search_stats};
     if (!ctx->tree_bounded) sa.redo_list = nullptr;
     return sa;
+}
+
+static bool plane_run_flags() {
+    static const bool on = env_int("LOCGPU_PLANE_RUNFLAGS", 1) != 0;
+    return on;
 }
 
 void init_state(PoseState& ps, const double pose[7]) {
@@ -103,7 +108,10 @@
             }
             sa.touched = ctx->touched_words ? ctx->d_touched.get() : nullptr;
         }
-        const bool ok_search = (grid_mode && !sa.visit_totals) ? launch_icp_search_grid(ctx->grid, sa, *w.grid, s) : launch_icp_search(sa, s);
+        if (prm.method == LOCGPU_P2PLANE && plane_run_flags()) sa.run_flags = b->d_run_flags;
+        bool wrote_flags = false;
+        const bool ok_search = (grid_mode && !sa.visit_totals) ? launch_icp_search_grid(ctx->grid, sa, *w.grid, s) : launch_icp_search(sa, s, &wrote_flags);
+        b->run_flags_written = wrote_flags;
         if (!ok_search) { fail(ctx, LOCGPU_ERR_DEPTH, std::string(w.who) + ": unsupported k/depth"); return -1; }
         if (sa.touched) launch_count_touched(sa.touched, (ctx->tree_slots + 2 + 31) / 32, sa.visit_totals, s);
         ev.mark(s, true);
@@ -112,6 +120,7 @@
         aa.active = w.active; aa.n_active = w.n_active;
         aa.src_of = w.src_of;
         aa.split_scans = w.split_scans;
+        if (wrote_flags && prm.method == LOCGPU_P2PLANE) aa.run_flags = b->d_run_flags;
         n_partial_blocks = launch_icp_accum(prm.method, aa, s);
     } else {
         ev.mark(s, true);
diff --git a/loc_lib_amd/csrc/icp_fit.hip b/loc_lib_amd/csrc/icp_fit.hip
--- a/loc_lib_amd/csrc/icp_fit.hip
+++ b/loc_lib_amd/csrc/icp_fit.hip
@@ -103,14 +103,6 @@
     J[1] = nR[2] * q.x - nR[0] * q.z;
     J[2] = nR[0] * q.y - nR[1] * q.x;
     J[3] = n3.x; J[4] = n3.y; J[5] = n3.z;
-}
-
-__device__ __forceinline__ void sort5(uint32_t (&s)[5]) {
-    auto cx = [&](int a, int b) {
-        const uint32_t lo = min(s[a], s[b]), hi = max(s[a], s[b]);
-        s[a] = lo; s[b] = hi;
-    };
-    cx(0, 1); cx(3, 4); cx(2, 4); cx(2, 3); cx(1, 4); cx(0, 3); cx(0, 2); cx(1, 3); cx(1, 2);
 }
 
 template <int FIT>
@@ -311,13 +303,136 @@
     ra.store(s_slice, partials + ((size_t)scan * gridDim.x + blockIdx.x) * kAccW);
 }
 
-template <int FIT, bool DEDUP>
+__device__ __forceinline__ void run_flag_ranks(const unsigned long long* __restrict__ words, int left, int kPlanePts, int wave, int lane,
+                                               int (&rank)[kDedupPP], bool (&leader)[kDedupPP], int& n_lead) {
+    static_assert(4 * kDedupPP <= 16, "a word per lane of a 16-lane row");
+    const int k = lane & 15;
+    const int valid = k < 4 * kPlanePts ? left - 64 * k : 0;
+    unsigned long long word = 0ull;
+    if (valid > 0) {
+        word = words[k];
+        if (valid < 64) word &= (1ull << valid) - 1ull;
+    }
+    const int count = __popcll(word);
+    int upto = count;
+#pragma unroll
+    for (int d = 1; d < 16; d <<= 1) {
+        const int t = __shfl_up(upto, d, 16);
+        if (k >= d) upto += t;
+    }
+    n_lead = __builtin_amdgcn_readlane(upto, 15);
+#pragma unroll
+    for (int h = 0; h < kDedupPP; ++h) {
+        const int from = 4 * h + wave;
+        const uint32_t lo = (uint32_t)__builtin_amdgcn_readlane((int)(uint32_t)word, from), hi = (uint32_t)__builtin_amdgcn_readlane((int)(uint32_t)(word >> 32), from);
+        const int before = __builtin_amdgcn_readlane(upto - count, from);
+        const int mine = h < kPlanePts ? left - 64 * from : 0;
+        const int below = (int)__builtin_amdgcn_mbcnt_hi(hi, __builtin_amdgcn_mbcnt_lo(lo, 0u));
+        const bool lead = (((lane < 32 ? lo : hi) >> (lane & 31)) & 1u) != 0u;
+        leader[h] = lead;
+        rank[h] = lane < mine ? before + below + (lead ? 1 : 0) : 0;
+    }
+}
+
+template <int FIT>
+__device__ __forceinline__ void plane_accum_flagged(const uint2* __restrict__ tree, const float4* __restrict__ src,
+                                                                 const int* __restrict__ counts, const PoseState* __restrict__ st,
+                                                                 const uint32_t* __restrict__ nn, size_t nn_pitch, int max_n,
+                                                                 double max_plane_distance, double* __restrict__ partials, int kPlanePts,
+                                                                 const int* __restrict__ active, const int* __restrict__ src_of,
+                                                                 const unsigned long long* __restrict__ run_flags) {
+    __shared__ double s_plane[kDedupPts][4];
+    __shared__ double s_slice[kBlock / 32][32];
+    __shared__ uint16_t s_lead[kDedupPts];
+    __shared__ uint16_t s_rank[kDedupPP][kBlock];
+    double (&s_row)[8][kAccPad] = *reinterpret_cast<double (*)[8][kAccPad]>(&s_plane[0][0]);
+    const int scan = active ? active[blockIdx.y] : (int)blockIdx.y;
+    if (st[scan].done) return;
+    const int lane = threadIdx.x & 63;
+    const int wave = __builtin_amdgcn_readfirstlane(threadIdx.x >> 6);
+    const size_t region = (size_t)scan * max_n;
+    const int first = blockIdx.x * kPlanePts * kBlock;
+    const int left = counts[scan] - first;
+    const unsigned long long* words = run_flags + (size_t)scan * ((max_n + 63) >> 6) + (first >> 6);
+    RowAccum ra;
+    ra.init();
+    int tid = threadIdx.x;
+    asm volatile("" : "+v"(tid));
+    int rank[kDedupPP], n_lead;
+    bool leader[kDedupPP];
+    run_flag_ranks(words, left, kPlanePts, wave, lane, rank, leader, n_lead);
+    n_lead = __builtin_amdgcn_readfirstlane(n_lead);
+#pragma unroll
+    for (int h = 0; h < kDedupPP; ++h) {
+        if (leader[h]) s_lead[rank[h] - 1] = (uint16_t)(h * kBlock + tid);
+        s_rank[h][tid] = (uint16_t)rank[h];
+    }
+    __syncthreads();
+#pragma unroll 1
+    for (int base = 0; base < n_lead; base += kBlock) {
+        if (base + wave * 64 < n_lead) {
+            const int j = base + tid;
+            if (j < n_lead) {
+                const uint16_t pt = s_lead[j];
+                const size_t gi = region + first + pt;
+                uint32_t slot[5];
+#pragma unroll
+                for (int k = 0; k < 5; ++k) slot[k] = __builtin_nontemporal_load(&nn[(size_t)k * nn_pitch + gi]);
+                if (slot[4] != kInvalidSlot) {
+                    sort5(slot);
+                    double n4[4];
+                    if (fit_plane<FIT>(tree, slot, n4)) s_lead[j] = pt | kLeadFits;
+#pragma unroll
+                    for (int c = 0; c < 4; ++c) s_plane[j][c] = n4[c];
+                }
+            }
+        }
+    }
+    __syncthreads();
+    tid = threadIdx.x;
+    asm volatile("" : "+v"(tid));
+    ra.index(tid);
+    double n4[kDedupPP][4];
+    float4 p[kDedupPP];
+    bool fits[kDedupPP];
+#pragma unroll
+    for (int h = 0; h < kDedupPP; ++h) {
+        rank[h] = s_rank[h][tid];
+        fits[h] = false;
+        if (rank[h] > 0) {
+            fits[h] = (s_lead[rank[h] - 1] & kLeadFits) != 0;
+#pragma unroll
+            for (int c = 0; c < 4; ++c) n4[h][c] = s_plane[rank[h] - 1][c];
+            p[h] = src[src_index(src_of, scan, max_n, first + h * kBlock + tid)];
+        }
+    }
+    __syncthreads();
+#pragma unroll
+    for (int h = 0; h < kDedupPP; ++h) {
+        if (h < kPlanePts) {
+            double J[1][6] = {{0.0, 0.0, 0.0, 0.0, 0.0, 0.0}};
+            double neg_e[1] = {0.0};
+            double fitted = 0.0;
+            if (fits[h]) {
+                fitted = 1.0;
+                plane_point_row(n4[h], p[h], st[scan], max_plane_distance, J[0], neg_e[0]);
+            }
+            ra.add<1>(s_row, J, neg_e, fitted);
+        }
+    }
+    ra.store(s_slice, partials + ((size_t)scan * gridDim.x + blockIdx.x) * kAccW);
+}
+
+template <int FIT, int RUNS>
 __global__ __launch_bounds__(kBlock) __attribute__((amdgpu_waves_per_eu(4, 4))) void icp_plane_accum_kernel(const uint2* __restrict__ tree, const float4* __restrict__ src,
                                                                  const int* __restrict__ counts, const PoseState* __restrict__ st,
                                                                  const uint32_t* __restrict__ nn, size_t nn_pitch, int max_n,
                                                                  double max_plane_distance, double* __restrict__ partials, int kPlanePts,
-                                                                 const int* __restrict__ active, const int* __restrict__ src_of) {
-    if constexpr (DEDUP)
+                                                                 const int* __restrict__ active, const int* __restrict__ src_of,
+                                                                 const unsigned long long* __restrict__ run_flags) {
+    if constexpr (RUNS == 2)
+        plane_accum_flagged<FIT>(tree, src, counts, st, nn, nn_pitch, max_n, max_plane_distance, partials, kPlanePts, active, src_of, run_flags);
+    else if constexpr (RUNS == 1)
         plane_accum_per_run<FIT>(tree, src, counts, st, nn, nn_pitch, max_n, max_plane_distance, partials, kPlanePts, active, src_of);
     else
         plane_accum_per_point<FIT>(tree, src, counts, st, nn, nn_pitch, max_n, max_plane_distance, partials, kPlanePts, active, src_of);
@@ -706,9 +821,11 @@
     const dim3 grid((blocks + pts - 1) / pts, a.active ? a.n_active : a.n_scans);
     if (method == LOCGPU_P2PLANE) {
         const bool secular = plane_fit_mode() == 1;
-        auto kernel = plane_dedup() && pts <= kDedupPP ? (secular ? icp_plane_accum_kernel<1, true> : icp_plane_accum_kernel<0, true>)
-                                    : (secular ? icp_plane_accum_kernel<1, false> : icp_plane_accum_kernel<0, false>);
-        hipLaunchKernelGGL(kernel, grid, dim3(kBlock), 0, s, a.tree, a.src, a.counts, a.st, a.nn, a.nn_pitch, a.max_n, a.gate, a.partials, pts, a.active, a.src_of);
+        const bool runs = plane_dedup() && pts <= kDedupPP;
+        auto kernel = !runs ? (secular ? icp_plane_accum_kernel<1, 0> : icp_plane_accum_kernel<0, 0>)
+                      : !a.run_flags ? (secular ? icp_plane_accum_kernel<1, 1> : icp_plane_accum_kernel<0, 1>)
+                                     : (secular ? icp_plane_accum_kernel<1, 2> : icp_plane_accum_kernel<0, 2>);
+        hipLaunchKernelGGL(kernel, grid, dim3(kBlock), 0, s, a.tree, a.src, a.counts, a.st, a.nn, a.nn_pitch, a.max_n, a.gate, a.partials, pts, a.active, a.src_of, a.run_flags);
     } else if (method == LOCGPU_P2PLANE_MAP)
         hipLaunchKernelGGL(icp_mapplane_accum_kernel, grid, dim3(kBlock), 0, s, reinterpret_cast<const double4*>(a.planes), a.src, a.counts, a.st, a.nn, a.max_n, a.gate, a.partials, pts, a.active, a.src_of);
     else if (method == LOCGPU_P2LINE)
diff --git a/loc_lib_amd/csrc/icp_kernels.hpp b/loc_lib_amd/csrc/icp_kernels.hpp
--- a/loc_lib_amd/csrc/icp_kernels.hpp
+++ b/loc_lib_amd/csrc/icp_kernels.hpp
@@ -52,6 +52,14 @@
         for (int w = 1; w < kBlock / 64; ++w) s += s_part[w][threadIdx.x];
         dst[threadIdx.x] = s;
     }
+}
+
+__device__ __forceinline__ void sort5(uint32_t (&s)[5]) {
+    auto cx = [&](int a, int b) {
+        const uint32_t lo = min(s[a], s[b]), hi = max(s[a], s[b]);
+        s[a] = lo; s[b] = hi;
+    };
+    cx(0, 1); cx(3, 4); cx(2, 4); cx(2, 3); cx(1, 4); cx(0, 3); cx(0, 2); cx(1, 3); cx(1, 2);
 }
 
 __device__ __forceinline__ void wave_append(uint32_t* __restrict__ list, unsigned int* __restrict__ count, bool pred, uint32_t value) {
diff --git a/loc_lib_amd/csrc/icp_search.hip b/loc_lib_amd/csrc/icp_search.hip
--- a/loc_lib_amd/csrc/icp_search.hip
+++ b/loc_lib_amd/csrc/icp_search.hip
@@ -108,7 +108,8 @@
                                                              unsigned int tree_bytes, uint32_t dummy, int skip_nonfinite, uint32_t* __restrict__ redo_list,
                                                              unsigned int* __restrict__ redo_count, uint32_t* __restrict__ deep_list,
                                                              unsigned int* __restrict__ deep_count, unsigned long long* __restrict__ search_stats,
-                                                             const int* __restrict__ active, const int* __restrict__ src_of) {
+                                                             const int* __restrict__ active, const int* __restrict__ src_of,
+                                                             unsigned long long* __restrict__ run_flags) {
     extern __shared__ uint2 s_dyn[];
     constexpr int ROWB = LANES * 8;
     static_assert(DF * ROWB >= 64 * 2 * 8, "exact stack columns do not fit");
@@ -139,6 +140,20 @@
     if (!deep && !slow) {
 #pragma unroll
         for (int j = 0; j < K; ++j) __builtin_nontemporal_store(w.id[j], &nn[(size_t)j * nn_pitch + gi]);
+    }
+    if constexpr (K == 5 && LANES == 64) {
+        if (run_flags) {
+            uint32_t set5[5];
+#pragma unroll
+            for (int j = 0; j < 5; ++j) set5[j] = w.id[j];
+            sort5(set5);
+            bool lead = w.id[4] == kInvalidSlot;
+#pragma unroll
+            for (int j = 0; j < 5; ++j) lead |= (uint32_t)__shfl_up((int)set5[j], 1, 64) != set5[j];
+            const unsigned long long unknown = __ballot(deep || slow);
+            const unsigned long long word = (__ballot(lead) | unknown | (unknown << 1) | 1ull) & __ballot(true);
+            if (tid == 0) run_flags[(size_t)scan * gridDim.x + blockIdx.x] = word;
+        }
     }
     wave_append(deep_list, deep_count, deep, (uint32_t)gi);
     if (LANES == 16) {
@@ -360,7 +375,7 @@
 }
 
 template <int K, int D, int DF, int WIN>
-static void launch_walk(const SearchArgs& a, hipStream_t s) {
+static bool launch_walk(const SearchArgs& a, hipStream_t s) {
     const bool stamp = stamp_build();
     const uint32_t dummy = (uint32_t)(a.tree_bytes / 8);
     const unsigned int rsrc_bytes = (unsigned int)a.tree_bytes + 16u;
@@ -368,8 +383,8 @@
     if (!stamp && (size_t)((a.max_n + 63) / 64) * n_launch <= 2048) {
         dim3 g1((a.max_n + 15) / 16, n_launch);
         hipLaunchKernelGGL((icp_search_walk_kernel<K, D + 2, 16>), g1, dim3(64), (D + 2) * 16 * 8, s, a.tree, a.src, a.counts, a.st, a.nn, a.nn_pitch, a.max_n,
-                           a.alpha_eff, 0, rsrc_bytes, dummy, a.skip_nonfinite, a.redo_list, a.redo_count, a.redo_list2, a.redo_count2, a.search_stats, a.active, a.src_of);
-        return;
+                           a.alpha_eff, 0, rsrc_bytes, dummy, a.skip_nonfinite, a.redo_list, a.redo_count, a.redo_list2, a.redo_count2, a.search_stats, a.active, a.src_of, nullptr);
+        return false;
     }
     const int stored = WIN ? kWindowStored : DF - 2;
     const int Tw = a.depth > stored ? a.depth - stored : 0;
@@ -379,15 +394,17 @@
     if (lds_knob) lds_bytes = (unsigned)std::max(env_int("LOCGPU_K1_LDS_BYTES", 0), DF * 64 * 8);
     if (stamp)
         hipLaunchKernelGGL((icp_search_walk_kernel<K, DF, 64, true, WIN>), g2, dim3(64), DF * 64 * 8, s, a.tree, a.src, a.counts, a.st, a.nn, a.nn_pitch, a.max_n,
-                           a.alpha_eff, Tw, rsrc_bytes, dummy, a.skip_nonfinite, a.redo_list, a.redo_count, a.redo_list2, a.redo_count2, a.search_stats, a.active, a.src_of);
+                           a.alpha_eff, Tw, rsrc_bytes, dummy, a.skip_nonfinite, a.redo_list, a.redo_count, a.redo_list2, a.redo_count2, a.search_stats, a.active, a.src_of, a.run_flags);
     else
         hipLaunchKernelGGL((icp_search_walk_kernel<K, DF, 64, false, WIN>), g2, dim3(64), lds_bytes, s, a.tree, a.src, a.counts, a.st, a.nn, a.nn_pitch, a.max_n,
-                           a.alpha_eff, Tw, rsrc_bytes, dummy, a.skip_nonfinite, a.redo_list, a.redo_count, a.redo_list2, a.redo_count2, a.search_stats, a.active, a.src_of);
+                           a.alpha_eff, Tw, rsrc_bytes, dummy, a.skip_nonfinite, a.redo_list, a.redo_count, a.redo_list2, a.redo_count2, a.search_stats, a.active, a.src_of, a.run_flags);
     launch_walk_list<K, D>(a, a.redo_list2, a.redo_count2, s);
     launch_redo<K, D>(a, s);
-}
-
-bool launch_icp_search(const SearchArgs& a, hipStream_t s) {
+    return K == 5 && a.run_flags != nullptr;
+}
+
+bool launch_icp_search(const SearchArgs& a, hipStream_t s, bool* wrote_run_flags) {
+    if (wrote_run_flags) *wrote_run_flags = false;
     const bool exact_only = a.visit_totals != nullptr || !a.redo_list || !a.redo_list2;
     return with_k<false>(a.k, [&](auto Kc) {
         return with_depth(a.depth, [&](auto Dc) {
@@ -395,7 +412,8 @@
             if (exact_only) return a.visit_totals ? launch_exact<K, D, true>(a, s) : launch_exact<K, D, false>(a, s);
             all_walk_shapes([&](auto DF, auto WIN) {
                 if (DF() != fast_stack_depth()) return true;
-                launch_walk<K, D, DF(), WIN()>(a, s);
+                const bool wrote = launch_walk<K, D, DF(), WIN()>(a, s);
+                if (wrote_run_flags) *wrote_run_flags = wrote;
                 return false;
             });
         });
diff --git a/loc_lib_amd/csrc/launch.hpp b/loc_lib_amd/csrc/launch.hpp
--- a/loc_lib_amd/csrc/launch.hpp
+++ b/loc_lib_amd/csrc/launch.hpp
@@ -31,6 +31,7 @@
     int n_active = 0;
     const int* src_of = nullptr;
     uint32_t* touched = nullptr;
+    unsigned long long* run_flags = nullptr;
 };
 
 struct AccumArgs {
@@ -48,9 +49,10 @@
     const int* src_of = nullptr;
     int split_scans = 0;
     const double* planes = nullptr;
+    const unsigned long long* run_flags = nullptr;
 };
 
-bool launch_icp_search(const SearchArgs& a, hipStream_t s);
+bool launch_icp_search(const SearchArgs& a, hipStream_t s, bool* wrote_run_flags = nullptr);
 bool launch_icp_search_redo(const SearchArgs& a, hipStream_t s);
 bool launch_icp_search_list(const SearchArgs& a, const uint32_t* list, const unsigned int* n_list, hipStream_t s);
 bool launch_knn_query(const uint2* tree, int depth, const float* q, size_t nq, int k, float alpha_eff, int32_t* out, uint32_t* visits,
diff --git a/loc_lib_amd/csrc/locgpu_api.hip b/loc_lib_amd/csrc/locgpu_api.hip
--- a/loc_lib_amd/csrc/locgpu_api.hip
+++ b/loc_lib_amd/csrc/locgpu_api.hip
@@ -235,6 +235,7 @@
               hip_ok(ctx, b->d_state.alloc(n_total), "hipMalloc state") &&
               (!sharded || hip_ok(ctx, b->d_acc.alloc((size_t)kFirstChunk * n_total * kAccW), "hipMalloc acc")) &&
               hip_ok(ctx, b->d_nn.alloc(5 * std::max<size_t>(b->pitch, 1)), "hipMalloc nn") &&
+              hip_ok(ctx, b->d_run_flags.alloc(std::max<size_t>((size_t)n_scans * ((max_n + 63) / 64), 1)), "hipMalloc run flags") &&
               hip_ok(ctx, b->d_partials.alloc((size_t)std::max(n_scans, 1) * b->blocks_per_scan * kAccW), "hipMalloc partials") &&
               hip_ok(ctx, b->d_hb.alloc((size_t)n_total * 44), "hipMalloc hb") &&
               hip_ok(ctx, b->d_redo_list.alloc((stamp_build() ? 2 : 1) * std::max<size_t>(b->pitch, 1)), "hipMalloc redo") &&
@@ -473,6 +474,18 @@
     const hipError_t e2 = hipStreamSynchronize(b->stream);
     LOCGPU_HIP(ctx, e);
     LOCGPU_HIP(ctx, e2);
+    return LOCGPU_OK;
+}
+
+int locgpu_debug_batch_run_flags(locgpu_ctx* ctx, locgpu_batch* b, uint64_t* out, int* written) {
+    if (!ctx || !b || b->ctx != ctx || !out || !written) return fail(ctx, LOCGPU_ERR_INVALID, "debug_batch_run_flags: bad arguments");
+    LOCGPU_HIP(ctx, hipSetDevice(ctx->device));
+    const size_t words = (size_t)b->n_scans * (((size_t)b->max_n + 63) / 64);
+    const hipError_t e = hipMemcpyAsync(out, b->d_run_flags, words * sizeof(uint64_t), hipMemcpyDeviceToHost, b->stream);
+    const hipError_t e2 = hipStreamSynchronize(b->stream);
+    LOCGPU_HIP(ctx, e);
+    LOCGPU_HIP(ctx, e2);
+    *written = b->run_flags_written ? 1 : 0;
     return LOCGPU_OK;
 }
 
```

Result: faster. 13730 scans/s, median of 6 (+1.9%).
